# Banus/pano360

Hardware: AMD Instinct MI355X
Metric: blended megapixels/sec (multiband) (higher is better)
Workload: dtype f32; 1 GPU; cfg3: 32 synthetic 3840x2160 frames per image set, spherical warp + multiband blend L=5, native resolution (MAX_RESOLUTION uncapped); frames=32

## Files before the change

### include/pano360.h

```cpp
#ifndef PANO360_H
#define PANO360_H

#include <stddef.h>
#include <stdint.h>

#ifdef __cplusplus
extern "C" {
#endif

#define PANO_OK 0
#define PANO_EINVAL (-1)
#define PANO_EHIP (-2)
#define PANO_ELIMIT (-3)
#define PANO_ESOLVE (-4)

#define PANO_MAX_TAPS 129
#define PANO_MAX_LEVELS 8
#define PANO_TAP_LEAD 7
#define PANO_TAP_PAD 40
#ifndef PANO_INTERIOR_BLOCK
#define PANO_INTERIOR_BLOCK 4
#endif

typedef struct pano_patch {
    float *planes;
    uint8_t *mask;
    float *blurred;
    float *scratch;
    int32_t y0, x0, h, w;
    int32_t vy0, vx0, vh, vw;
    int32_t ay0, ax0, ah, aw;
    int32_t vpitch, apitch;
    int32_t index;
    int32_t tiles_off;
} pano_patch;

typedef struct pano_layout {
    int64_t planes_floats;
    int64_t blurred_floats;
    int64_t scratch_floats;
    int32_t n_records, n_tiles;
    int32_t max_vw, max_vh, max_aw, max_ah;
    int32_t missing;
} pano_layout;

typedef struct pano_camera {
    double proj[9];
    const uint8_t *frame;
    const double *hat_x;
    const double *hat_y;
    int32_t sh, sw;
    int32_t y0, x0, h, w;
} pano_camera;

typedef struct pano_pair {
    double minv[9];
    int32_t i, j;
} pano_pair;

typedef struct pano_sift_keypoint {
    float x, y;
    float size;
    float angle;
    float response;
    int32_t octave;
    int32_t r, c;
} pano_sift_keypoint;


const char *pano_version(void);
const char *pano_last_error(void);
int pano_device_count(void);
int pano_pitch(int w);
int pano_interior_block(void);

typedef struct pano_ctx pano_ctx;
#define PANO_OPT_BLUR_KERNEL 0
#define PANO_OPT_OWN_PRUNE 1
#define PANO_OPT_BLUR_SEGMENTS 2
#define PANO_OPT_BLUR_LEAN 3
#define PANO_OPT_STITCH_STREAMS 4
#define PANO_OPT_STITCH_ASYNC 5
#define PANO_OPT_BLUR_SEG_LEN 6
#define PANO_OPT_SIFT_GRAPH 7
#define PANO_OPT_LEVEL_CLASSES 8
#define PANO_OPT_COUNT 9
#define PANO_BLUR_MFMA 0
#define PANO_BLUR_VALU 1
int pano_ctx_create(int device, void *stream, pano_ctx **out);
int pano_ctx_destroy(pano_ctx *ctx);
int pano_ctx_set_stream(pano_ctx *ctx, void *stream);
int pano_ctx_set_option(pano_ctx *ctx, int option, int value);
int pano_ctx_get_option(const pano_ctx *ctx, int option, int *value);

int pano_timing_enable(pano_ctx *ctx, int on);
int pano_kernel_count(void);
const char *pano_kernel_name(int kid);
int pano_timing_read(pano_ctx *ctx, int kid, double *total_ms, int *launches);

int pano_add_weights(pano_ctx *ctx, const uint8_t *frame, int h, int w,
                     const float *lut255, const double *hat_x, const double *hat_y,
                     float *rgba);

int pano_warp_spherical(pano_ctx *ctx, const uint8_t *frame, int sh, int sw,
                        const double *proj, const double *sin_t, const double *cos_t,
                        const double *tan_p, const float *lut255, const double *hat_x,
                        const double *hat_y, int gx0, int gy0, int pw, int ph,
                        float *planes, uint8_t *mask, float *map_x, float *map_y);

int pano_warp_windows(pano_ctx *ctx, const pano_camera *cams, const pano_patch *patches,
                      int n, int max_vw, int max_vh, const double *sin_t,
                      const double *cos_t, const double *tan_p, const float *lut,
                      int lut_stride, const uint8_t *need);

int pano_ownership(pano_ctx *ctx, const pano_patch *patches, int n, int H, int W,
                   int16_t *owner, uint8_t *valid);

int pano_ownership_cameras(pano_ctx *ctx, const pano_camera *cams, int n, int H, int W,
                           int xs0, int xs1, const double *sin_t, const double *cos_t,
                           const double *tan_p, int16_t *owner, uint8_t *valid);

int pano_owned_regions(pano_ctx *ctx, const int16_t *owner, int H, int W, int xs0, int xs1,
                       int n, int min_gap, int max_spans, uint8_t *marks,
                       int32_t *regions);

int pano_ownership_regions(pano_ctx *ctx, const pano_camera *cams, int n, int H, int W,
                           int xs0, int xs1, const double *sin_t, const double *cos_t,
                           const double *tan_p, int16_t *owner, uint8_t *valid,
                           int min_gap, int max_spans, uint8_t *marks, int32_t *regions);

int pano_blur_tile_grid(const pano_ctx *ctx);
int pano_blur_tiles(pano_ctx *ctx, const pano_patch *patches, int n, int max_aw,
                    int max_ah, int W, int radius, const uint8_t *interior,
                    uint8_t *tile_flags, uint8_t *warp_need);
int pano_multiband_blur_prepare(pano_ctx *ctx, const pano_patch *patches, int n,
                                int max_aw, int max_ah, int W, const uint8_t *interior,
                                uint8_t *tile_flags);
int pano_multiband_blur(pano_ctx *ctx, const pano_patch *patches, int n, int max_aw,
                        int max_vh, int max_ah, const int16_t *owner, int W,
                        const float *taps, const int *ntaps, int n_blur,
                        const uint8_t *interior, uint8_t *tile_flags);

int pano_interior_map(pano_ctx *ctx, const int16_t *owner, int H, int W, int xs0, int xs1,
                      int radius, int16_t *block_owner, uint8_t *interior);
int pano_interior_classes(pano_ctx *ctx, const int16_t *owner, int H, int W, int xs0, int xs1,
                          const int *radii, int n_radii, int16_t *block_owner, uint8_t *interior,
                          uint8_t *classes);

int pano_layout_windows(int tile_grid, const int32_t *regions, int n, int max_spans,
                        const int32_t *rects, const uint8_t *have, int radius,
                        int xs0, int xs1, int n_blur, pano_patch *records, int cap,
                        pano_layout *out);
int pano_layout_place(pano_patch *records, int n_records, void *planes, void *blurred,
                      void *scratch);

int pano_multiband_compose(pano_ctx *ctx, const pano_patch *patches, int n, int H, int W,
                           int xs0, int xs1, int n_levels, const int16_t *owner,
                           const uint8_t *valid, const uint8_t *interior,
                           const uint8_t *classes, const pano_camera *cams,
                           const double *sin_t, const double *cos_t, const double *tan_p,
                           const float *lut, int lut_stride, uint8_t *mosaic,
                           float *mosaic_f32);

int pano_blend_cameras(pano_ctx *ctx, const pano_camera *cams, int n, int H, int W,
                       int xs0, int xs1, int linear, const double *sin_t,
                       const double *cos_t, const double *tan_p, const float *lut,
                       int lut_stride, uint8_t *mosaic, uint8_t *valid);

int pano_overlap_blocks(int h, int w);
int pano_overlap_stats(pano_ctx *ctx, const pano_camera *cams, const pano_pair *pairs,
                       int n_pairs, int h, int w, int bw0, const float *lut255,
                       double *partials, double *stats);

int pano_linear_blend(pano_ctx *ctx, const pano_patch *patches, int n, int H, int W,
                      uint8_t *mosaic);

int pano_no_blend(pano_ctx *ctx, const pano_patch *patches, int n, int H, int W,
                  uint8_t *mosaic);

int pano_crop_rect(pano_ctx *ctx, const uint8_t *valid, int H, int W, int32_t *heights,
                   int64_t *result);

int pano_blur_plane(pano_ctx *ctx, const float *src, float *dst, float *tmp, int h, int w,
                    int pitch, const float *taps, int ntaps);

int pano_pyr_down(pano_ctx *ctx, const float *src, int h, int w, float *dst);

int pano_gray_u8(pano_ctx *ctx, const uint8_t *bgr, int h, int w, float *out);
int pano_scale_step(pano_ctx *ctx, const float *src, int h, int w, const float *taps, int ntaps,
                    float *dst, float *dog);
int pano_scale_space(pano_ctx *ctx, const uint8_t *frame, int h, int w, int n_octaves,
                     int n_layers, const float *taps, const int *ntaps, float *const *gauss,
                     float *const *dog, float *work);
int pano_resize_up2(pano_ctx *ctx, const float *src, int h, int w, float *dst);
int pano_decimate2(pano_ctx *ctx, const float *src, int h, int w, float *dst);
int pano_subtract(pano_ctx *ctx, const float *a, const float *b, size_t n, float *out);

int pano_pyr_down_image(pano_ctx *ctx, const void *src, int h, int w, int c, int is_f64,
                        void *dst);
int pano_pyr_up_image(pano_ctx *ctx, const void *src, int sh, int sw, int c, int is_f64,
                      const void *other, int mode, void *dst, int oh, int ow);
int pano_u8_to_f32(pano_ctx *ctx, const uint8_t *src, size_t n, float *dst);
int pano_laplacian_mix(pano_ctx *ctx, const float *la, const float *lb, const void *gm, size_t n,
                       int is_f64, void *out);
int pano_clip_u8(pano_ctx *ctx, const void *src, size_t n, int is_f64, uint8_t *dst);

#define PANO_POISSON_CHUNK 32
int pano_poisson_blend(pano_ctx *ctx, const uint8_t *src, uint8_t *tgt, const uint8_t *mask,
                       int h, int w, int c, double rtol, int max_iters, double *solution,
                       int32_t *iters, double *resid);

#define PANO_SEAM_U8 0
#define PANO_SEAM_I16 1
#define PANO_SEAM_I32 2
#define PANO_SEAM_F32 3
#define PANO_SEAM_F64 4
#define PANO_SEAM_RESIDENT_CELLS 81408
#define PANO_SEAM_BATCH 64
int pano_seam_levels(pano_ctx *ctx, const void *img1, const void *img2, int dtype, int h, int w,
                     int c, int shrink, int16_t *level, int32_t *bad);
int pano_seam_flood(pano_ctx *ctx, const int16_t *level, int rows, int cols, int border,
                    int path, int8_t *labels, int32_t *stats);
int pano_seam_mask(pano_ctx *ctx, const int8_t *labels, int rows, int cols,
                   const int32_t *xtab, const int32_t *ytab, uint8_t *mask, int h, int w);
int pano_alpha_blend(pano_ctx *ctx, const void *img1, const void *img2, int dtype,
                     const void *mask, int mask_f64, int64_t mask_sy, int64_t mask_sx,
                     int64_t mask_sc, int h, int w, int c, uint8_t *out);

int pano_resize_u8(pano_ctx *ctx, const uint8_t *src, int sh, int sw, int c,
                   const int32_t *xtab, const int32_t *ytab, uint8_t *dst, int oh, int ow);

int pano_sift_extrema(pano_ctx *ctx, const float *dog, int rows, int cols, int octave,
                      int n_layers, float contrast_thr, float edge_thr, float sigma,
                      pano_sift_keypoint *cands, int *count, int max_cands);
int pano_sift_orient(pano_ctx *ctx, const float *const *gauss, const int *dims,
                     int n_layers, const pano_sift_keypoint *cands, const int *n_cands,
                     int max_cands, pano_sift_keypoint *kpts, int *count, int max_kpts);
int pano_sift_describe(pano_ctx *ctx, const float *const *gauss, const int *dims,
                       int first_octave, const pano_sift_keypoint *kpts, int n,
                       const int *n_dev, float *desc);
size_t pano_sift_sort_work_bytes(int n);
int pano_sift_sort_unique(pano_ctx *ctx, const pano_sift_keypoint *kpts, int n, const int *n_dev,
                          int first_octave, void *work, pano_sift_keypoint *out, int *n_out);

typedef struct pano_sift_args {
    const uint8_t *frame;
    uint8_t *frame_copy;
    int32_t h, w, n_octaves, n_layers;
    const float *taps;
    const int32_t *ntaps;
    float *const *gauss;
    float *const *dog;
    float *work;
    int32_t detect;
    float contrast_thr, edge_thr, sigma;
    int32_t first_octave, max_keypoints;
    const float *const *gauss_dev;
    const int32_t *dims_dev;
    pano_sift_keypoint *cands, *kpts;
    int32_t *counts;
    void *sort_work;
    float *desc;
} pano_sift_args;
int pano_sift_detect(pano_ctx *ctx, const pano_sift_args *args);
int pano_sift_detect_replaying(const pano_ctx *ctx);

size_t pano_knn2_work_bytes(int nq, int nt, int d);
int pano_knn2(pano_ctx *ctx, const float *query, int nq, const float *train, int nt, int d,
              float scale, void *work, int32_t *idx, float *dist, int *rescans);

int pano_match_pack(pano_ctx *ctx, const int32_t *idx, const float *dist, int nq, double ratio,
                    const float *kp_query, const float *kp_train, int nt, float *pts,
                    int32_t *match, int32_t *count);

size_t pano_hom_ransac_work_bytes(int n_pairs, int max_iters);
int pano_hom_ransac(pano_ctx *ctx, const float *pts, const int32_t *offsets, const int32_t *counts,
                    int n_pairs, int max_iters, float thresh, uint64_t seed, void *work,
                    double *hom, uint8_t *mask, int32_t *n_inliers, int32_t *hyp_inliers);

size_t pano_ba_work_bytes(int n_pairs);
int pano_ba_residuals(pano_ctx *ctx, const double *rows, const int32_t *pairs, int n_pairs,
                      const double *hom, double *ssq);
int pano_ba_normal(pano_ctx *ctx, const double *rows, const int32_t *pairs, int n_pairs,
                   const int32_t *slot, int n_active, const double *jtab, const double *hom_r,
                   double lambda, void *work, double *jtj, double *jtr);

#define PANO_JPEG_FIELDS 32
#define PANO_JPEG_CHUNK 1024
#define PANO_JPEG_SUBSEQ 1024
#define PANO_JPEG_HUFF_BYTES 1424
enum {
    PANO_JD_W, PANO_JD_H, PANO_JD_NC, PANO_JD_HMAX, PANO_JD_VMAX, PANO_JD_MCUX, PANO_JD_MCUY,
    PANO_JD_RI,
    PANO_JD_NINT,
    PANO_JD_BPM,
    PANO_JD_ORIENT, PANO_JD_DATA_OFF, PANO_JD_DATA_LEN, PANO_JD_TAB_OFF,
    PANO_JD_CHUNK0,
    PANO_JD_INT0,
    PANO_JD_SUB0,
    PANO_JD_BLK0, PANO_JD_PIX0,
    PANO_JD_DST_OFF,
    PANO_JD_PLANE0, PANO_JD_PLANE1, PANO_JD_PLANE2,
    PANO_JD_PITCH0, PANO_JD_PITCH1, PANO_JD_PITCH2,
    PANO_JD_OUT_OFF,
    PANO_JD_COMP_U,
    PANO_JD_SAMP,
    PANO_JD_TABSEL
};
enum {
    PANO_JB_N, PANO_JB_CHUNKS, PANO_JB_INTS, PANO_JB_SUBS, PANO_JB_BLOCKS, PANO_JB_PIXELS,
    PANO_JB_OUT_BYTES, PANO_JB_W_KEPT, PANO_JB_W_RST, PANO_JB_W_KEPTX, PANO_JB_W_RSTX,
    PANO_JB_W_DSTLEN, PANO_JB_W_ISTART, PANO_JB_W_IEND, PANO_JB_W_INSUB, PANO_JB_W_ISUBX,
    PANO_JB_W_STATE0, PANO_JB_W_STATE1, PANO_JB_W_CNTX, PANO_JB_W_FLAG, PANO_JB_W_COEF,
    PANO_JB_WORK_BYTES, PANO_JB_PACKED_BYTES
};
int pano_jpeg_decode(pano_ctx *ctx, const int64_t *desc, int n, const uint8_t *packed,
                     int64_t packed_bytes, void *work, int64_t work_bytes, uint8_t *out,
                     int64_t out_bytes);

#define PANO_JPEG_MAX_SIDE 65500
#define PANO_JPEG_BGR 1
size_t pano_jpeg_encode_work_bytes(int h, int w, int subsampling);
int pano_jpeg_encode(pano_ctx *ctx, const uint8_t *img, int h, int w, int64_t pitch, int flags,
                     int subsampling, const uint8_t *qt, void *work, int64_t work_bytes,
                     const uint8_t **stream, int64_t *stream_bytes);

#define PANO_EGROW 1
typedef struct pano_stitch_args {
    const pano_camera *cams;
    const int32_t *rects;
    const uint8_t *have;
    const double *sin_t, *cos_t, *tan_p;
    const float *lut;
    const float *taps;
    const int32_t *ntaps;
    int16_t *owner;
    uint8_t *valid;
    uint8_t *marks;
    int32_t *regions;
    int32_t *regions_host;
    int16_t *block_owner;
    uint8_t *interior;
    pano_patch *records_host;
    pano_patch *table;
    float *planes, *blurred, *scratch;
    uint8_t *tile_flags, *need;
    uint8_t *mosaic;
    float *mosaic_f32;
    int64_t planes_floats, blurred_floats, scratch_floats;
    int32_t n, H, W, xs0, xs1, own0, own1;
    int32_t lut_stride, n_levels, radius, shortcut, warp_need, max_spans, min_gap;
    int32_t cap_records, cap_tiles;
    int32_t used_need;
    int32_t trust_layout;
    uint8_t *classes;
    pano_layout layout;
} pano_stitch_args;
int pano_stitch_multiband(pano_ctx *ctx, pano_stitch_args *args, int resume);
int pano_stitch_verify(pano_ctx *ctx);
int pano_stitch_counts(const pano_ctx *ctx, int *device_layouts, int *fallbacks);

#ifdef __cplusplus
}
#endif
#endif
```

### pano360_amd/_lib.py

```python
import ctypes as C
import os
import subprocess

_HERE = os.path.dirname(os.path.abspath(__file__))
LIB_PATH = os.environ.get("PANO_LIB") or os.path.join(_HERE, "libpano360_hip.so")

MAX_TAPS = 129
MAX_LEVELS = 8
TAP_LEAD = 7
TAP_PAD = 40
OPT_BLUR_KERNEL, OPT_OWN_PRUNE, OPT_BLUR_SEGMENTS, OPT_BLUR_LEAN, OPT_STITCH_STREAMS = 0, 1, 2, 3, 4
OPT_STITCH_ASYNC = 5
OPT_BLUR_SEG_LEN = 6
OPT_SIFT_GRAPH = 7
OPT_LEVEL_CLASSES = 8
BLUR_MFMA, BLUR_VALU = 0, 1


class PanoError(RuntimeError):
    """A C-ABI call returned a negative status."""


class Patch(C.Structure):
    _fields_ = [("planes", C.c_void_p), ("mask", C.c_void_p),
                ("blurred", C.c_void_p), ("scratch", C.c_void_p),
                ("y0", C.c_int32), ("x0", C.c_int32), ("h", C.c_int32), ("w", C.c_int32),
                ("vy0", C.c_int32), ("vx0", C.c_int32), ("vh", C.c_int32), ("vw", C.c_int32),
                ("ay0", C.c_int32), ("ax0", C.c_int32), ("ah", C.c_int32), ("aw", C.c_int32),
                ("vpitch", C.c_int32), ("apitch", C.c_int32),
                ("index", C.c_int32), ("tiles_off", C.c_int32)]


class Layout(C.Structure):
    _fields_ = [("planes_floats", C.c_int64), ("blurred_floats", C.c_int64),
                ("scratch_floats", C.c_int64), ("n_records", C.c_int32), ("n_tiles", C.c_int32),
                ("max_vw", C.c_int32), ("max_vh", C.c_int32), ("max_aw", C.c_int32),
                ("max_ah", C.c_int32), ("missing", C.c_int32)]


class SiftArgs(C.Structure):
    _fields_ = [("frame", C.c_void_p), ("frame_copy", C.c_void_p),
                ("h", C.c_int32), ("w", C.c_int32), ("n_octaves", C.c_int32), ("n_layers", C.c_int32),
                ("taps", C.c_void_p), ("ntaps", C.c_void_p), ("gauss", C.c_void_p),
                ("dog", C.c_void_p), ("work", C.c_void_p), ("detect", C.c_int32),
                ("contrast_thr", C.c_float), ("edge_thr", C.c_float), ("sigma", C.c_float),
                ("first_octave", C.c_int32), ("max_keypoints", C.c_int32),
                ("gauss_dev", C.c_void_p), ("dims_dev", C.c_void_p), ("cands", C.c_void_p),
                ("kpts", C.c_void_p), ("counts", C.c_void_p), ("sort_work", C.c_void_p),
                ("desc", C.c_void_p)]


class StitchArgs(C.Structure):
    _fields_ = ([(k, C.c_void_p) for k in (
        "cams", "rects", "have", "sin_t", "cos_t", "tan_p", "lut", "taps", "ntaps", "owner",
        "valid", "marks", "regions", "regions_host", "block_owner", "interior", "records_host",
        "table", "planes", "blurred", "scratch", "tile_flags", "need", "mosaic", "mosaic_f32")]
        + [(k, C.c_int64) for k in ("planes_floats", "blurred_floats", "scratch_floats")]
        + [(k, C.c_int32) for k in (
            "n", "H", "W", "xs0", "xs1", "own0", "own1", "lut_stride", "n_levels", "radius",
            "shortcut", "warp_need", "max_spans", "min_gap", "cap_records", "cap_tiles",
            "used_need", "trust_layout")]
        + [("classes", C.c_void_p), ("layout", Layout)])


EINVAL = -1
ESOLVE = -4
SEAM_DTYPES = {"uint8": 0, "int16": 1, "int32": 2, "float32": 3, "float64": 4}
SEAM_RESIDENT_CELLS = 81408
EGROW = 1


class Pair(C.Structure):
    _fields_ = [("minv", C.c_double * 9), ("i", C.c_int32), ("j", C.c_int32)]


class SiftKeypoint(C.Structure):
    _fields_ = [("x", C.c_float), ("y", C.c_float), ("size", C.c_float), ("angle", C.c_float),
                ("response", C.c_float), ("octave", C.c_int32), ("r", C.c_int32), ("c", C.c_int32)]


class Camera(C.Structure):
    _fields_ = [("proj", C.c_double * 9), ("frame", C.c_void_p),
                ("hat_x", C.c_void_p), ("hat_y", C.c_void_p),
                ("sh", C.c_int32), ("sw", C.c_int32),
                ("y0", C.c_int32), ("x0", C.c_int32), ("h", C.c_int32), ("w", C.c_int32)]


_vp, _i = C.c_void_p, C.c_int
_SIGNATURES = {
    "pano_version": (C.c_char_p, []),
    "pano_last_error": (C.c_char_p, []),
    "pano_device_count": (_i, []),
    "pano_pitch": (_i, [_i]),
    "pano_interior_block": (_i, []),
    "pano_ctx_create": (_i, [_i, _vp, C.POINTER(C.c_void_p)]),
    "pano_ctx_destroy": (_i, [_vp]),
    "pano_ctx_set_stream": (_i, [_vp, _vp]),
    "pano_ctx_set_option": (_i, [_vp, _i, _i]),
    "pano_ctx_get_option": (_i, [_vp, _i, C.POINTER(C.c_int)]),
    "pano_timing_enable": (_i, [_vp, _i]),
    "pano_kernel_count": (_i, []),
    "pano_kernel_name": (C.c_char_p, [_i]),
    "pano_timing_read": (_i, [_vp, _i, C.POINTER(C.c_double), C.POINTER(C.c_int)]),
    "pano_add_weights": (_i, [_vp, _vp, _i, _i, _vp, _vp, _vp, _vp]),
    "pano_warp_spherical": (_i, [_vp, _vp, _i, _i, _vp, _vp, _vp, _vp, _vp, _vp, _vp, _i, _i, _i,
                                 _i, _vp, _vp, _vp, _vp]),
    "pano_warp_windows": (_i, [_vp, _vp, _vp, _i, _i, _i, _vp, _vp, _vp, _vp, _i, _vp]),
    "pano_blur_tiles": (_i, [_vp, _vp, _i, _i, _i, _i, _i, _vp, _vp, _vp]),
    "pano_ownership": (_i, [_vp, _vp, _i, _i, _i, _vp, _vp]),
    "pano_ownership_cameras": (_i, [_vp, _vp, _i, _i, _i, _i, _i, _vp, _vp, _vp, _vp, _vp]),
    "pano_owned_regions": (_i, [_vp, _vp, _i, _i, _i, _i, _i, _i, _i, _vp, _vp]),
    "pano_ownership_regions": (_i, [_vp, _vp, _i, _i, _i, _i, _i, _vp, _vp, _vp, _vp, _vp,
                                    _i, _i, _vp, _vp]),
    "pano_multiband_blur": (_i, [_vp, _vp, _i, _i, _i, _i, _vp, _i, _vp, C.POINTER(C.c_int), _i,
                                 _vp, _vp]),
    "pano_multiband_blur_prepare": (_i, [_vp, _vp, _i, _i, _i, _i, _vp, _vp]),
    "pano_layout_windows": (_i, [_i, _vp, _i, _i, _vp, _vp, _i, _i, _i, _i, _vp, _i, _vp]),
    "pano_layout_place": (_i, [_vp, _i, _vp, _vp, _vp]),
    "pano_interior_map": (_i, [_vp, _vp, _i, _i, _i, _i, _i, _vp, _vp]),
    "pano_interior_classes": (_i, [_vp, _vp, _i, _i, _i, _i, _vp, _i, _vp, _vp, _vp]),
    "pano_multiband_compose": (_i, [_vp, _vp, _i, _i, _i, _i, _i, _i, _vp, _vp, _vp, _vp, _vp, _vp,
                                    _vp, _vp, _vp, _i, _vp, _vp]),
    "pano_blend_cameras": (_i, [_vp, _vp, _i, _i, _i, _i, _i, _i, _vp, _vp, _vp, _vp, _i, _vp,
                                _vp]),
    "pano_blur_tile_grid": (_i, [_vp]),
    "pano_overlap_blocks": (_i, [_i, _i]),
    "pano_overlap_stats": (_i, [_vp, _vp, _vp, _i, _i, _i, _i, _vp, _vp, _vp]),
    "pano_linear_blend": (_i, [_vp, _vp, _i, _i, _i, _vp]),
    "pano_no_blend": (_i, [_vp, _vp, _i, _i, _i, _vp]),
    "pano_crop_rect": (_i, [_vp, _vp, _i, _i, _vp, _vp]),
    "pano_blur_plane": (_i, [_vp, _vp, _vp, _vp, _i, _i, _i, _vp, _i]),
    "pano_pyr_down": (_i, [_vp, _vp, _i, _i, _vp]),
    "pano_gray_u8": (_i, [_vp, _vp, _i, _i, _vp]),
    "pano_scale_step": (_i, [_vp, _vp, _i, _i, _vp, _i, _vp, _vp]),
    "pano_scale_space": (_i, [_vp, _vp, _i, _i, _i, _i, _vp, _vp, _vp, _vp, _vp]),
    "pano_resize_up2": (_i, [_vp, _vp, _i, _i, _vp]),
    "pano_decimate2": (_i, [_vp, _vp, _i, _i, _vp]),
    "pano_subtract": (_i, [_vp, _vp, _vp, C.c_size_t, _vp]),
    "pano_pyr_down_image": (_i, [_vp, _vp, _i, _i, _i, _i, _vp]),
    "pano_pyr_up_image": (_i, [_vp, _vp, _i, _i, _i, _i, _vp, _i, _vp, _i, _i]),
    "pano_u8_to_f32": (_i, [_vp, _vp, C.c_size_t, _vp]),
    "pano_laplacian_mix": (_i, [_vp, _vp, _vp, _vp, C.c_size_t, _i, _vp]),
    "pano_clip_u8": (_i, [_vp, _vp, C.c_size_t, _i, _vp]),
    "pano_poisson_blend": (_i, [_vp, _vp, _vp, _vp, _i, _i, _i, C.c_double, _i, _vp, _vp, _vp]),
    "pano_seam_levels": (_i, [_vp, _vp, _vp, _i, _i, _i, _i, _i, _vp, _vp]),
    "pano_seam_flood": (_i, [_vp, _vp, _i, _i, _i, _i, _vp, _vp]),
    "pano_seam_mask": (_i, [_vp, _vp, _i, _i, _vp, _vp, _vp, _i, _i]),
    "pano_alpha_blend": (_i, [_vp, _vp, _vp, _i, _vp, _i, C.c_int64, C.c_int64, C.c_int64, _i, _i,
                              _i, _vp]),
    "pano_resize_u8": (_i, [_vp, _vp, _i, _i, _i, _vp, _vp, _vp, _i, _i]),
    "pano_sift_extrema": (_i, [_vp, _vp, _i, _i, _i, _i, C.c_float, C.c_float, C.c_float, _vp,
                               _vp, _i]),
    "pano_sift_orient": (_i, [_vp, _vp, _vp, _i, _vp, _vp, _i, _vp, _vp, _i]),
    "pano_sift_describe": (_i, [_vp, _vp, _vp, _i, _vp, _i, _vp, _vp]),
    "pano_sift_sort_work_bytes": (C.c_size_t, [_i]),
    "pano_sift_sort_unique": (_i, [_vp, _vp, _i, _vp, _i, _vp, _vp, _vp]),
    "pano_knn2_work_bytes": (C.c_size_t, [_i, _i, _i]),
    "pano_knn2": (_i, [_vp, _vp, _i, _vp, _i, _i, C.c_float, _vp, _vp, _vp, _vp]),
    "pano_hom_ransac_work_bytes": (C.c_size_t, [_i, _i]),
    "pano_hom_ransac": (_i, [_vp, _vp, _vp, _vp, _i, _i, C.c_float, C.c_uint64, _vp, _vp, _vp, _vp,
                             _vp]),
    "pano_match_pack": (_i, [_vp, _vp, _vp, _i, C.c_double, _vp, _vp, _i, _vp, _vp, _vp]),
    "pano_ba_work_bytes": (C.c_size_t, [_i]),
    "pano_ba_residuals": (_i, [_vp, _vp, _vp, _i, _vp, _vp]),
    "pano_ba_normal": (_i, [_vp, _vp, _vp, _i, _vp, _i, _vp, _vp, C.c_double, _vp, _vp, _vp]),
    "pano_jpeg_decode": (_i, [_vp, _vp, _i, _vp, C.c_int64, _vp, C.c_int64, _vp, C.c_int64]),
    "pano_jpeg_encode_work_bytes": (C.c_size_t, [_i, _i, _i]),
    "pano_jpeg_encode": (_i, [_vp, _vp, _i, _i, C.c_int64, _i, _i, _vp, _vp, C.c_int64,
                             C.POINTER(C.c_void_p), C.POINTER(C.c_int64)]),
    "pano_sift_detect": (_i, [_vp, _vp]),
    "pano_sift_detect_replaying": (_i, [_vp]),
    "pano_stitch_multiband": (_i, [_vp, _vp, _i]),
    "pano_stitch_counts": (_i, [_vp, _vp, _vp]),
    "pano_stitch_verify": (_i, [_vp]),
}
EXPORTS = tuple(_SIGNATURES)


def sources_digest():
    import hashlib
    src = os.path.join(_HERE, "csrc")
    files = sorted(os.path.join(src, f) for f in os.listdir(src)
                   if f.endswith((".hip", ".h", ".inc")) or f == "Makefile")
    files.append(os.path.join(os.path.dirname(_HERE), "include", "pano360.h"))
    h = hashlib.sha256()
    for path in files:
        if not os.path.exists(path):
            continue
        h.update(os.path.basename(path).encode() + b"\0")
        with open(path, "rb") as fid:
            h.update(fid.read())
    return h.hexdigest()


BUILD_RECORD = os.path.join(_HERE, "csrc", ".build_stamp")


def build(force=False):
    import json
    src = os.path.join(_HERE, "csrc")
    digest = sources_digest()
    have = None
    try:
        with open(BUILD_RECORD) as fid:
            have = json.load(fid).get("sources_sha256")
    except (OSError, ValueError):
        pass
    full = force or have != digest or not os.path.exists(LIB_PATH)
    before = os.path.getmtime(LIB_PATH) if os.path.exists(LIB_PATH) else None
    cmd = ["make", "-C", src, "-s", "-j4"] + (["-B"] if full else [])
    subprocess.check_call(cmd)
    after = os.path.getmtime(LIB_PATH)
    mode = "full" if full else ("incremental" if after != before else "up to date")
    with open(BUILD_RECORD, "w") as fid:
        json.dump({"sources_sha256": digest, "mode": mode}, fid)
    return LIB_PATH


_lib = None


def lib():
    global _lib
    if _lib is None:
        if not os.path.exists(LIB_PATH):
            raise PanoError(
                f"{LIB_PATH} is missing: build it with "
                "`python -c 'import __graft_entry__ as g; g.build()'` "
                "(there is no CPU fallback)")
        import torch
        handle = C.CDLL(LIB_PATH)
        for name, (res, args) in _SIGNATURES.items():
            fn = getattr(handle, name)
            fn.restype, fn.argtypes = res, args
        _lib = handle
    return _lib


def check(status, what):
    if status != 0:
        msg = lib().pano_last_error().decode("utf-8", "replace")
        raise PanoError(f"{what} failed ({status}): {msg}")
```

### pano360_amd/csrc/api.hip

```cpp
#include <stdarg.h>
#include <stdio.h>
#include <stdlib.h>
#include <string.h>

#include <vector>

#include "common.h"
#include "layout.h"

static thread_local char g_error[512] = "";

void pano_set_error(const char *fmt, ...) {
    va_list ap;
    va_start(ap, fmt);
    vsnprintf(g_error, sizeof(g_error), fmt, ap);
    va_end(ap);
}

extern "C" const char *pano_version(void) { return "pano360_hip 0.1 (gfx950)"; }

extern "C" const char *pano_last_error(void) { return g_error; }

extern "C" int pano_device_count(void) {
    int n = 0;
    if (hipGetDeviceCount(&n) != hipSuccess) {
        (void)hipGetLastError();
        return 0;
    }
    return n;
}

extern "C" int pano_pitch(int w) { return pano_pitch_of(w); }

extern "C" int pano_interior_block(void) { return PANO_INTERIOR_BLOCK; }

extern "C" int pano_ctx_create(int device, void *stream, pano_ctx **out) {
    PANO_REQUIRE(out, "pano_ctx_create: null output");
    *out = nullptr;
    PANO_REQUIRE(device >= 0 && device < pano_device_count(), "pano_ctx_create: no device %d",
                 device);
    PANO_HIP(hipSetDevice(device));
    if (int rc = pano_blur_mfma_opt_in()) return rc;
    if (int rc = pano_blur_valu_opt_in()) return rc;
    pano_ctx *ctx = new pano_ctx();
    ctx->device = device;
    ctx->stream = (hipStream_t)stream;
    ctx->opt[PANO_OPT_BLUR_KERNEL] = PANO_BLUR_MFMA;
    ctx->opt[PANO_OPT_OWN_PRUNE] = 1;
    ctx->opt[PANO_OPT_BLUR_SEGMENTS] = 1;
    ctx->opt[PANO_OPT_BLUR_LEAN] = 1;
    ctx->opt[PANO_OPT_STITCH_STREAMS] = 1;
    ctx->opt[PANO_OPT_STITCH_ASYNC] = 0;
    ctx->opt[PANO_OPT_BLUR_SEG_LEN] = 0;
    ctx->opt[PANO_OPT_SIFT_GRAPH] = 1;
    ctx->opt[PANO_OPT_LEVEL_CLASSES] = 0;
    *out = ctx;
    return PANO_OK;
}

int pano_ctx_enter(pano_ctx *ctx) {
    if (!ctx->in_stitch) ctx->geom_valid = false;
    PANO_HIP(hipSetDevice(ctx->device));
    return PANO_OK;
}

static void timing_clear(pano_ctx *ctx) {
    for (int k = 0; k < PK_COUNT; ++k) {
        for (hipEvent_t e : ctx->t_begin[k]) (void)hipEventDestroy(e);
        for (hipEvent_t e : ctx->t_end[k]) (void)hipEventDestroy(e);
        ctx->t_begin[k].clear();
        ctx->t_end[k].clear();
    }
}

static void tap_set_free(PanoTapSet &ts) {
    if (ts.taps) (void)hipFree(ts.taps);
    if (ts.tables) (void)hipFree(ts.tables);
    if (ts.ready) (void)hipEventDestroy(ts.ready);
    free(ts.host);
    ts.taps = nullptr;
    ts.tables = nullptr;
    ts.ready = nullptr;
    ts.host = nullptr;
}

extern "C" int pano_ctx_destroy(pano_ctx *ctx) {
    if (!ctx) return PANO_OK;
    PANO_HIP(hipSetDevice(ctx->device));
    if (hipStreamSynchronize(ctx->stream) != hipSuccess) {
        (void)hipGetLastError();
        (void)hipDeviceSynchronize();
    }
    timing_clear(ctx);
    for (PanoTapSet &ts : ctx->tap_sets) tap_set_free(ts);
    if (ctx->item_buf) (void)hipFree(ctx->item_buf);
    if (ctx->item_counter) (void)hipFree(ctx->item_counter);
    if (ctx->sift_raw) (void)hipFree(ctx->sift_raw);
    if (ctx->enc_dev) (void)hipFree(ctx->enc_dev);
    if (ctx->enc_out) (void)hipFree(ctx->enc_out);
    if (ctx->enc_host) (void)hipHostFree(ctx->enc_host);
    if (ctx->poisson_dev) (void)hipFree(ctx->poisson_dev);
    if (ctx->poisson_host) (void)hipHostFree(ctx->poisson_host);
    if (ctx->seam_dev) (void)hipFree(ctx->seam_dev);
    if (ctx->seam_host) (void)hipHostFree(ctx->seam_host);
    pano_sift_graphs_free(ctx);
    if (ctx->lay_sum_host) (void)hipHostFree(ctx->lay_sum_host);
    if (ctx->lay_rects_dev) (void)hipFree(ctx->lay_rects_dev);
    if (ctx->lay_have_dev) (void)hipFree(ctx->lay_have_dev);
    if (ctx->side) {
        (void)hipStreamSynchronize(ctx->side);
        (void)hipStreamDestroy(ctx->side);
    }
    if (ctx->ev_fork) (void)hipEventDestroy(ctx->ev_fork);
    if (ctx->ev_join) (void)hipEventDestroy(ctx->ev_join);
    if (ctx->ev_regions) (void)hipEventDestroy(ctx->ev_regions);
    if (ctx->ev_upload) (void)hipEventDestroy(ctx->ev_upload);
    if (ctx->ev_copy) (void)hipEventDestroy(ctx->ev_copy);
    delete ctx;
    return PANO_OK;
}

int pano_ctx_side_stream(pano_ctx *ctx) {
    if (!ctx->ev_regions) PANO_HIP(hipEventCreateWithFlags(&ctx->ev_regions, hipEventDisableTiming));
    if (!ctx->ev_upload) PANO_HIP(hipEventCreateWithFlags(&ctx->ev_upload, hipEventDisableTiming));
    if (!ctx->ev_fork) PANO_HIP(hipEventCreateWithFlags(&ctx->ev_fork, hipEventDisableTiming));
    if (!ctx->ev_join) PANO_HIP(hipEventCreateWithFlags(&ctx->ev_join, hipEventDisableTiming));
    if (!ctx->ev_copy) PANO_HIP(hipEventCreateWithFlags(&ctx->ev_copy, hipEventDisableTiming));
    if (!ctx->side) PANO_HIP(hipStreamCreateWithFlags(&ctx->side, hipStreamNonBlocking));
    return PANO_OK;
}

extern "C" int pano_ctx_set_stream(pano_ctx *ctx, void *stream) {
    PANO_REQUIRE(ctx, "pano_ctx_set_stream: null context");
    if ((hipStream_t)stream != ctx->stream) ctx->geom_valid = false;
    ctx->stream = (hipStream_t)stream;
    return PANO_OK;
}

extern "C" int pano_ctx_set_option(pano_ctx *ctx, int option, int value) {
    PANO_REQUIRE(ctx, "pano_ctx_set_option: null context");
    PANO_REQUIRE(option >= 0 && option < PANO_OPT_COUNT, "pano_ctx_set_option: option %d", option);
    if (option == PANO_OPT_BLUR_KERNEL)
        PANO_REQUIRE(value == PANO_BLUR_MFMA || value == PANO_BLUR_VALU,
                     "pano_ctx_set_option: blur kernel %d", value);
    else if (option == PANO_OPT_STITCH_ASYNC)
        PANO_REQUIRE(value >= 0 && value <= 2, "pano_ctx_set_option: option %d takes 0, 1 or 2", option);
    else if (option == PANO_OPT_OWN_PRUNE)
        PANO_REQUIRE(value >= 0 && value <= 3, "pano_ctx_set_option: option %d takes 0 .. 3", option);
    else if (option == PANO_OPT_BLUR_SEG_LEN)
        PANO_REQUIRE(value == -1 || value == 0 || (value >= 4 && value <= 2047),
                     "pano_ctx_set_option: option %d takes -1, 0 or 4 .. 2047", option);
    else
        PANO_REQUIRE(value == 0 || value == 1, "pano_ctx_set_option: option %d takes 0 or 1", option);
    const bool changed = ctx->opt[option] != value;
    ctx->opt[option] = value;
    ctx->prepared_table = ctx->flags_table = ctx->list_table = nullptr;
    ctx->geom_valid = false;
    if (changed && option == PANO_OPT_BLUR_KERNEL)
        ctx->lay_prev_valid = ctx->lay_prev_verified = false;
    return PANO_OK;
}

extern "C" int pano_ctx_get_option(const pano_ctx *ctx, int option, int *value) {
    PANO_REQUIRE(ctx && value, "pano_ctx_get_option: null pointer");
    PANO_REQUIRE(option >= 0 && option < PANO_OPT_COUNT, "pano_ctx_get_option: option %d", option);
    *value = ctx->opt[option];
    return PANO_OK;
}

static uint64_t tap_hash(const float *taps, const int *ntaps, int n, size_t floats) {
    uint64_t h = 1469598103934665603ull;
    auto eat = [&](const void *p, size_t bytes) {
        const unsigned char *b = (const unsigned char *)p;
        for (size_t i = 0; i < bytes; ++i) h = (h ^ b[i]) * 1099511628211ull;
    };
    eat(&n, sizeof(n));
    eat(ntaps, n * sizeof(int));
    eat(taps, floats * sizeof(float));
    return h;
}

#define PANO_TAP_SETS_MAX 64
int pano_ctx_tap_set(pano_ctx *ctx, const float *taps, const int *ntaps, int n, size_t table_bytes,
                     PanoTapSet **out, bool *fresh) {
    size_t floats = 0;
    for (int k = 0; k < n; ++k) floats += (size_t)ntaps[k] + PANO_TAP_PAD;
    const uint64_t key = tap_hash(taps, ntaps, n, floats);
    *fresh = false;
    for (PanoTapSet &ts : ctx->tap_sets)
        if (ts.key == key && ts.n == n && !memcmp(ts.ntaps, ntaps, n * sizeof(int)) &&
            ts.floats == floats && !memcmp(ts.host, taps, floats * sizeof(float))) {
            ts.used = ++ctx->tick;
            if (ctx->stream != ts.built_on) PANO_HIP(hipStreamWaitEvent(ctx->stream, ts.ready, 0));
            if (table_bytes && !ts.tables) {
                PANO_HIP(hipMalloc((void **)&ts.tables, table_bytes));
                *fresh = true;
            }
            *out = &ts;
            return PANO_OK;
        }
    if (ctx->tap_sets.size() >= PANO_TAP_SETS_MAX) {
        size_t old = 0;
        for (size_t i = 1; i < ctx->tap_sets.size(); ++i)
            if (ctx->tap_sets[i].used < ctx->tap_sets[old].used) old = i;
        PANO_HIP(hipDeviceSynchronize());
        tap_set_free(ctx->tap_sets[old]);
        ctx->tap_sets.erase(ctx->tap_sets.begin() + old);
    }
    PanoTapSet ts = {};
    ts.key = key;
    ts.n = n;
    memcpy(ts.ntaps, ntaps, n * sizeof(int));
    ts.floats = floats;
    ts.host = (float *)malloc(floats * sizeof(float));
    PANO_REQUIRE(ts.host, "pano_ctx_tap_set: out of host memory");
    memcpy(ts.host, taps, floats * sizeof(float));
    PANO_HIP(hipMalloc((void **)&ts.taps, floats * sizeof(float)));
    PANO_HIP(hipMemcpyAsync(ts.taps, taps, floats * sizeof(float), hipMemcpyHostToDevice,
                            ctx->stream));
    PANO_HIP(hipEventCreateWithFlags(&ts.ready, hipEventDisableTiming));
    PANO_HIP(hipEventRecord(ts.ready, ctx->stream));
    ts.built_on = ctx->stream;
    if (table_bytes) {
        PANO_HIP(hipMalloc((void **)&ts.tables, table_bytes));
        *fresh = true;
    }
    ts.used = ++ctx->tick;
    ctx->tap_sets.push_back(ts);
    *out = &ctx->tap_sets.back();
    return PANO_OK;
}

int pano_ctx_tap_set_built(pano_ctx *ctx, PanoTapSet *set) {
    PANO_HIP(hipEventRecord(set->ready, ctx->stream));
    set->built_on = ctx->stream;
    return PANO_OK;
}

static const char *const g_kernel_names[] = {
    "add_weights_kernel", "warp_spherical_kernel", "ownership_kernel", "blur_rows_kernel",
    "blur_cols_kernel",   "multiband_compose_kernel", "linear_blend_kernel",
    "no_blend_kernel",    "crop_heights_kernel", "crop_rows_kernel", "pyr_down_kernel",
    "ownership_cameras_kernel", "owned_boxes_kernel", "warp_windows_kernel",
    "blend_cameras_kernel", "owned_spans_kernel",
    "block_owner_kernel", "tile_flags_kernel", "overlap_stats_kernel",
    "blur_mfma_kernel", "sift_extrema_kernel", "sift_orient_kernel", "sift_describe_kernel",
    "scale_step_kernel", "knn2_kernel", "blur_lean_kernel", "blur_lean5_kernel",
    "ransac_score_kernel", "ransac_finish_kernel", "match_pack_kernel",
    "ba_residual_kernel", "ba_pair_kernel", "ba_assemble_kernel",
    "jpeg_destuff_kernel", "jpeg_scan_kernel", "jpeg_intervals_kernel", "jpeg_huff_sync_kernel",
    "jpeg_huff_write_kernel", "jpeg_dc_kernel", "jpeg_idct_kernel", "jpeg_pixels_kernel",
    "jpeg_enc_blocks_kernel", "jpeg_enc_count_kernel", "jpeg_enc_scan_kernel", "jpeg_enc_emit_kernel",
    "jpeg_enc_stuff_kernel"};
static_assert(sizeof(g_kernel_names) / sizeof(g_kernel_names[0]) == PK_COUNT,
              "one name per PanoKernelId, in enum order");

void pano_timing_edge(pano_ctx *ctx, int kid, hipStream_t stream, bool begin) {
    hipEvent_t ev;
    if (hipEventCreate(&ev) != hipSuccess) return;
    (void)hipEventRecord(ev, stream);
    (begin ? ctx->t_begin : ctx->t_end)[kid].push_back(ev);
}

extern "C" int pano_timing_enable(pano_ctx *ctx, int on) {
    PANO_REQUIRE(ctx, "pano_timing_enable: null context");
    timing_clear(ctx);
    ctx->timing_on = on != 0;
    return PANO_OK;
}

extern "C" int pano_kernel_count(void) { return PK_COUNT; }

extern "C" const char *pano_kernel_name(int kid) {
    return kid >= 0 && kid < PK_COUNT ? g_kernel_names[kid] : "";
}

extern "C" int pano_timing_read(pano_ctx *ctx, int kid, double *total_ms, int *launches) {
    PANO_REQUIRE(ctx && kid >= 0 && kid < PK_COUNT && total_ms && launches,
                 "pano_timing_read: bad argument");
    double sum = 0.0;
    const size_t nb = ctx->t_begin[kid].size(), ne = ctx->t_end[kid].size();
    const size_t n = ne < nb ? ne : nb;
    for (size_t i = 0; i < n; ++i) {
        PANO_HIP(hipEventSynchronize(ctx->t_end[kid][i]));
        float ms = 0.f;
        PANO_HIP(hipEventElapsedTime(&ms, ctx->t_begin[kid][i], ctx->t_end[kid][i]));
        sum += ms;
    }
    *total_ms = sum;
    *launches = (int)n;
    return PANO_OK;
}

extern "C" int pano_layout_windows(int tile_grid, const int32_t *regions, int n, int max_spans,
                                   const int32_t *rects, const uint8_t *have, int radius,
                                   int xs0, int xs1, int n_blur, pano_patch *records, int cap,
                                   pano_layout *out) {
    PANO_REQUIRE(regions && rects && records && out, "pano_layout_windows: null pointer");
    PANO_REQUIRE(tile_grid == 0 || tile_grid == 32, "pano_layout_windows: tile grid %d", tile_grid);
    PANO_REQUIRE(n >= 0 && max_spans >= 1 && radius >= 0 && n_blur >= 0 && cap >= 0,
                 "pano_layout_windows: bad argument");
    const bool grid32 = tile_grid == 32;
    const int stride = 5 + 2 * max_spans;
    pano_layout lay = {};
    lay.missing = 0;
    long planes = 0, blurred = 0, scratch = 0, tiles = 0;
    int k = 0;
    for (int i = 0; i < n; ++i) {
        const int32_t *rg = regions + (size_t)i * stride;
        const int spans = rg[4] < max_spans ? rg[4] : max_spans;
        for (int sp = 0; sp < spans; ++sp) {
            pano_patch rec;
            LayoutSizes sz;
            if (!layout_record(rg, sp, rects + 4 * i, i, radius, xs0, xs1, n_blur, grid32, rec, sz))
                continue;
            PANO_REQUIRE(k < cap, "pano_layout_windows: more than %d records", cap);
            if (have && !have[i]) ++lay.missing;
            pano_patch &r = records[k++];
            r = rec;
            PANO_REQUIRE(layout_record_fits(r),
                         "pano_layout_windows: a plane of record %d exceeds 2 GiB", k - 1);
            r.planes = (float *)(uintptr_t)planes;
            r.blurred = (float *)(uintptr_t)(blurred + sz.lead);
            r.scratch = (float *)(uintptr_t)scratch;
            PANO_REQUIRE(tiles < (1l << 31), "pano_layout_windows: tile count overflow");
            r.tiles_off = (int)tiles;
            planes += sz.planes;
            blurred += sz.blurred;
            scratch += sz.scratch;
            tiles += sz.tiles;
            lay.max_vw = r.vw > lay.max_vw ? r.vw : lay.max_vw;
            lay.max_vh = r.vh > lay.max_vh ? r.vh : lay.max_vh;
            lay.max_aw = r.aw > lay.max_aw ? r.aw : lay.max_aw;
            lay.max_ah = r.ah > lay.max_ah ? r.ah : lay.max_ah;
        }
    }
    lay.n_records = k;
    lay.n_tiles = (int)tiles;
    lay.planes_floats = planes;
    lay.blurred_floats = blurred + 32;
    lay.scratch_floats = scratch;
    *out = lay;
    return PANO_OK;
}

extern "C" int pano_layout_place(pano_patch *records, int n_records, void *planes, void *blurred,
                                 void *scratch) {
    PANO_REQUIRE(records || n_records == 0, "pano_layout_place: null pointer");
    uintptr_t bbase = (uintptr_t)blurred;
    bbase += (uintptr_t)(-(intptr_t)bbase) % 128;
    for (int k = 0; k < n_records; ++k) {
        pano_patch &r = records[k];
        r.planes = (float *)planes + (uintptr_t)r.planes;
        r.blurred = blurred ? (float *)bbase + (uintptr_t)r.blurred : nullptr;
        r.scratch = scratch ? (float *)scratch + (uintptr_t)r.scratch : nullptr;
    }
    return PANO_OK;
}
```

### pano360_amd/csrc/blend.hip

```cpp
#include <stdlib.h>

#include "geom.h"

__global__ __launch_bounds__(256) void ownership_kernel(
    const pano_patch *__restrict__ patches, int n, int H, int W,
    int16_t *__restrict__ owner, uint8_t *__restrict__ valid) {
    const int x = blockIdx.x * 64 + threadIdx.x, y = blockIdx.y * 4 + threadIdx.y;
    if (x >= W || y >= H) return;
    float best = 0.0f;
    int who = -1;
    bool any = false;
    for (int i = 0; i < n; ++i) {
        const pano_patch p = patches[i];
        const int px = x - p.x0, py = y - p.y0;
        if ((unsigned)px >= (unsigned)p.w || (unsigned)py >= (unsigned)p.h) continue;
        const float a = p.planes[3 * (size_t)p.vh * p.vpitch + (size_t)py * p.vpitch + px];
        if (a > best) {
            best = a;
            who = i;
        }
        any |= p.mask[(size_t)py * p.w + px] == 0;
    }
    owner[(size_t)y * W + x] = (int16_t)who;
    valid[(size_t)y * W + x] = any ? 1 : 0;
// ... 384 lines not shown
        }
        __syncthreads();
        const int tid = wave * 64 + lane;
        const bool keep = tid < listed && alpha_bound(cams + sh.list[tid], s_rng).hi >= 0.0f;
        const unsigned long long bal = __ballot(keep);
        if (lane == 0) s_kept[wave] = __popcll(bal);
        __syncthreads();
        int off = 0;
        for (int w = 0; w < wave; ++w) off += s_kept[w];
        off += __popcll(bal & ((1ull << lane) - 1ull));
        if (keep) s_keep[off] = sh.list[tid];
        ncand = s_kept[0] + s_kept[1] + s_kept[2] + s_kept[3];
        list = s_keep;
        __syncthreads();
    }

    const int x = bx0 + threadIdx.x, y = by0 + threadIdx.y;
    if (x >= xs1 || y >= H) return;
    const double s = sin_t[x], c = cos_t[x], t = tan_p[y];
    float acc[3] = {0.0f, 0.0f, 0.0f}, wsum = 0.0f;
    uint8_t last[3] = {0, 0, 0};
    bool any = false;
    for (int kk = 0; kk < ncand; ++kk) {
        const int k = LINEAR ? kk : ncand - 1 - kk;
        const int i = listed < 0 ? k : __builtin_amdgcn_readfirstlane(list[k]);
        const pano_camera *cam = cams + i;
        const int px = x - cam->x0, py = y - cam->y0;
        if ((unsigned)px >= (unsigned)cam->w || (unsigned)py >= (unsigned)cam->h) continue;
        float fx, fy;
        const int sw = cam->sw, sh_ = cam->sh;
        if (map_pixel(cam->proj, s, c, t, sw, sh_, fx, fy)) continue;
        any = true;
        const Taps tp = make_taps_unmasked(fx, fy, sw, sh_);
        const TapBytes tb = load_taps(cam->frame, sw, tp);
        float rgb[3];
        const float *__restrict__ gl = lut + (size_t)i * 256;
#pragma unroll
        for (int ch = 0; ch < 3; ++ch)
            rgb[ch] = PERCAM ? lerp4(lut_at(gl, tb.v[0][ch]), lut_at(gl, tb.v[1][ch]), lut_at(gl, tb.v[2][ch]),
                                     lut_at(gl, tb.v[3][ch]), tp)
                             : lerp4(lut_at(s_lut, tb.v[0][ch]), lut_at(s_lut, tb.v[1][ch]), lut_at(s_lut, tb.v[2][ch]),
                                     lut_at(s_lut, tb.v[3][ch]), tp);
        if (LINEAR) {
            const float a = alpha_at(cam->hat_x, cam->hat_y, tp);
#pragma unroll
            for (int ch = 0; ch < 3; ++ch) acc[ch] = acc[ch] + rgb[ch] * a;
            wsum = wsum + a;
        } else {
#pragma unroll
            for (int ch = 0; ch < 3; ++ch) last[ch] = (uint8_t)(int)(255.0f * rgb[ch]);
            break;
        }
    }
    const size_t g = ((size_t)y * W + x) * 3;
    if (LINEAR) {
        const float ws = wsum == 0.0f ? 1.0f : wsum;
#pragma unroll
        for (int ch = 0; ch < 3; ++ch)
            mosaic[g + ch] = (uint8_t)(int)(255.0f * __fdiv_rn(acc[ch], ws));
    } else {
        mosaic[g] = last[0];
        mosaic[g + 1] = last[1];
        mosaic[g + 2] = last[2];
    }
    if (valid) valid[(size_t)y * W + x] = any ? 1 : 0;
}

typedef short own8 __attribute__((ext_vector_type(8), aligned(2)));

__device__ __forceinline__ void owned_box_pixel(int o, int x, int y, bool up, bool down, bool left,
                                                bool right, int W, int32_t *__restrict__ boxes,
                                                int stride, uint8_t *__restrict__ marks) {
    if (o < 0) return;
    if (up && marks) marks[(size_t)o * W + x] = 1;
    if (!left && !right) return;
    if (left && up) {
        atomicMin(&boxes[(size_t)stride * o + 0], y);
        atomicMin(&boxes[(size_t)stride * o + 2], x);
    }
    if (left && down) atomicMax(&boxes[(size_t)stride * o + 1], y);
    if (right && up) atomicMax(&boxes[(size_t)stride * o + 3], x);
}

__global__ __launch_bounds__(256) void owned_boxes_kernel(const int16_t *__restrict__ owner,
                                                          int H, int W, int xs0, int xs1,
                                                          int32_t *__restrict__ boxes, int stride,
                                                          uint8_t *__restrict__ marks) {
    const int x8 = xs0 + (blockIdx.x * 64 + threadIdx.x) * 8, y = blockIdx.y * 4 + threadIdx.y;
    if (x8 >= xs1 || y >= H) return;
    const int16_t *row = owner + (size_t)y * W;
    const bool top = y == 0, bottom = y == H - 1;
    if (x8 + 8 <= xs1) {
        const own8 cur = *(const own8 *)(row + x8);
        const own8 upv = top ? cur : *(const own8 *)(row - W + x8);
        const own8 dnv = bottom ? cur : *(const own8 *)(row + W + x8);
        const int before = x8 == xs0 ? -32768 : row[x8 - 1];
        const int after = x8 + 8 == xs1 ? -32768 : row[x8 + 8];
#pragma unroll
        for (int j = 0; j < 8; ++j) {
            const int o = cur[j];
            const int l = j == 0 ? before : cur[j - 1], r = j == 7 ? after : cur[j + 1];
            owned_box_pixel(o, x8 + j, y, top || upv[j] != o, bottom || dnv[j] != o, l != o, r != o,
                            W, boxes, stride, marks);
        }
        return;
    }
    for (int x = x8; x < xs1; ++x) {
        const int o = row[x];
        owned_box_pixel(o, x, y, top || row[x - W] != o, bottom || row[x + W] != o,
                        x == xs0 || row[x - 1] != o, x == xs1 - 1 || row[x + 1] != o, W, boxes,
                        stride, marks);
    }
}

__device__ __forceinline__ uint8_t quant255(float v) { return (uint8_t)(int)(255.0f * v); }

#define IB PANO_INTERIOR_BLOCK

__global__ __launch_bounds__(256) void block_owner_kernel(const int16_t *__restrict__ owner,
                                                          int H, int W, int xs0, int xs1,
                                                          int H8, int W8, int blo, int bhi,
                                                          int16_t *__restrict__ bown) {
    const int bx = blo + blockIdx.x * 64 + threadIdx.x, by = blockIdx.y * 4 + threadIdx.y;
    if (bx >= bhi || by >= H8) return;
    const int x0 = bx * IB, y0 = by * IB;
    int o = -2;
    if (x0 >= xs0 && (x0 + IB < W ? x0 + IB : W) <= xs1) {
        o = owner[(size_t)y0 * W + x0];
        const bool whole = x0 + IB <= W && (W & 1) == 0;
        if (x0 + IB <= W && y0 + IB <= H) {
            static_assert(IB == 4, "one 8-byte load per block row");
            typedef uint64_t u64_any __attribute__((aligned(2)));
            const uint64_t o16 = (uint16_t)o;
            const uint64_t all = o16 | o16 << 16 | o16 << 32 | o16 << 48;
            uint64_t diff = 0;
#pragma unroll
            for (int dy = 0; dy < IB; ++dy)
                diff |= *(const u64_any *)(owner + (size_t)(y0 + dy) * W + x0) ^ all;
            if (diff) o = -2;
        } else
        for (int dy = 0; dy < IB && o != -2; ++dy) {
            const int y = y0 + dy;
            if (y >= H) break;
            if (whole) {
                const uint32_t *q = (const uint32_t *)(owner + (size_t)y * W + x0);
                const uint32_t both = ((uint32_t)(uint16_t)o << 16) | (uint16_t)o;
                uint32_t diff = 0;
#pragma unroll
                for (int k = 0; k < IB / 2; ++k) diff |= q[k] ^ both;
                if (diff) o = -2;
            } else {
                for (int dx = 0; dx < IB; ++dx) {
                    const int x = x0 + dx;
                    if (x >= W) break;
                    if (owner[(size_t)y * W + x] != o) {
                        o = -2;
                        break;
                    }
                }
            }
        }
    }
    bown[(size_t)by * W8 + bx] = (int16_t)o;
}

#define IT_W 64
#define IT_H 16
#define IT_REACH_MAX 20
__device__ __forceinline__ bool agree(int a, int b) { return a == b || a == -3 || b == -3; }

struct LevelReaches {
    int n;
    int reach[PANO_MAX_LEVELS];
};

__global__ __launch_bounds__(256) void interior_tile_kernel(const int16_t *__restrict__ bown,
                                                            int H8, int W8, int reach, int blo,
                                                            int bhi, int ilo, int ihi,
                                                            uint8_t *__restrict__ interior,
                                                            LevelReaches lv,
                                                            uint8_t *__restrict__ classes) {
    __shared__ int16_t s_own[(IT_H + 2 * IT_REACH_MAX) * (IT_W + 2 * IT_REACH_MAX)];
    __shared__ int16_t s_col[IT_H * (IT_W + 2 * IT_REACH_MAX)];
    __shared__ unsigned long long s_vmask[IT_W + 2 * IT_REACH_MAX];
    const int tid = threadIdx.x, lane = tid & 63, wave = tid >> 6;
    const int bx0 = ilo + blockIdx.x * IT_W, by0 = blockIdx.y * IT_H;
    const int tw = IT_W + 2 * reach, th = IT_H + 2 * reach;
    for (int ty = wave; ty < th; ty += 4) {
        const int y = by0 - reach + ty;
        const bool row_in = y >= 0 && y < H8;
        for (int tx = lane; tx < tw; tx += 64) {
            const int x = bx0 - reach + tx;
            s_own[ty * tw + tx] = (row_in && x >= 0 && x < W8)
                                      ? (x >= blo && x < bhi ? bown[(size_t)y * W8 + x] : (int16_t)-2)
                                      : (int16_t)-3;
        }
    }
    __syncthreads();
    for (int tx = tid; tx < tw; tx += 256) {
        unsigned long long m = 0;
        int prev = s_own[tx];
#pragma unroll 8
        for (int ty = 0; ty + 1 < th; ++ty) {
            const int cur = s_own[(ty + 1) * tw + tx];
            m |= (unsigned long long)agree(prev, cur) << ty;
            prev = cur;
        }
        s_vmask[tx] = m;
    }
    __syncthreads();
    int cls[IT_H / 4];
#pragma unroll
    for (int r = 0; r < IT_H / 4; ++r) cls[r] = 0;
    const int nlv = classes ? lv.n : 1;
    for (int q = 0; q < nlv; ++q) {
        const int rq = classes ? lv.reach[q] : reach, off = reach - rq;
        const unsigned long long full = (1ull << (2 * rq)) - 1ull;
        for (int ry = wave; ry < IT_H; ry += 4)
            for (int tx = lane; tx < tw; tx += 64) {
                const int o = s_own[(ry + reach) * tw + tx];
                const bool same = ((s_vmask[tx] >> (ry + off)) & full) == full;
                s_col[ry * tw + tx] = (int16_t)(o >= 0 && !same ? -2 : o);
            }
        __syncthreads();
#pragma unroll
        for (int r = 0; r < IT_H / 4; ++r) {
            const int ry = wave + 4 * r;
            const int16_t *row = s_col + ry * tw;
            const int a0 = row[lane], a1 = row[min(lane + 1, tw - 1)];
            const int b0 = row[min(lane + 64, tw - 1)], b1 = row[min(lane + 65, tw - 1)];
            const unsigned long long lo = __ballot(lane + 1 < tw && agree(a0, a1));
            const unsigned long long hi = __ballot(lane + 65 < tw && agree(b0, b1));
            const int sh = lane + off;
            const unsigned long long win = sh == 0 ? lo
                                           : sh < 64 ? (lo >> sh) | (hi << (64 - sh))
                                                     : hi >> (sh - 64);
            const int o = row[lane + reach];
            if (o >= 0 && (win & full) == full && cls[r] == q) cls[r] = q + 1;
        }
        __syncthreads();
    }
#pragma unroll
    for (int r = 0; r < IT_H / 4; ++r) {
        const int y = by0 + wave + 4 * r, x = bx0 + lane;
        if (y >= H8 || x >= ihi) continue;
        interior[(size_t)y * W8 + x] = cls[r] == nlv ? 1 : 0;
        if (classes) classes[(size_t)y * W8 + x] = (uint8_t)cls[r];
    }
}

struct InteriorArgs {
    const uint8_t *interior;
    int W8;
    const pano_camera *cams;
    const double *sin_t, *cos_t, *tan_p;
    const float *lut;
    const uint8_t *classes;
};

enum { LUT_LDS = 0, LUT_GLOBAL = 1 };

template <int LUT>
__device__ __forceinline__ void shade_interior(const pano_camera *cam, const float *__restrict__ table,
                                               const InteriorArgs &ia, int x, int y, int W,
                                               uint8_t *__restrict__ mosaic,
                                               float *__restrict__ mosaic_f32) {
    if (!cam->frame) return;
    const int sw = cam->sw, sh = cam->sh;
    float fx, fy;
    map_pixel(cam->proj, table_f64(ia.sin_t, x), table_f64(ia.cos_t, x), table_f64(ia.tan_p, y), sw, sh, fx, fy);
    Taps tp = tap_base(fx, fy);
    TapBytes tb;
    if (__ballot(!taps_interior(tp, sw, sh)) == 0ull) {
        tb = load_taps_interior(cam->frame, sw, tp);
    } else {
        tp.x1 = min(tp.x1, sw - 1);
        tp.y1 = min(tp.y1, sh - 1);
        tb = load_taps(cam->frame, sw, tp);
    }
    const size_t g = ((size_t)y * W + x) * 3;
#pragma unroll
    for (int c = 0; c < 3; ++c) {
        float v = lerp4(lut_at(table, tb.v[0][c]), lut_at(table, tb.v[1][c]),
                        lut_at(table, tb.v[2][c]), lut_at(table, tb.v[3][c]), tp);
        v = v < 0.0f ? 0.0f : (v > 1.0f ? 1.0f : v);
        if (mosaic_f32) mosaic_f32[g + c] = v;
        mosaic[g + c] = (uint8_t)(int)(255.0f * v);
    }
}

template <int LUT>
__device__ __forceinline__ void shade_interior_of(int own, const float *__restrict__ table, int stride,
                                                  const InteriorArgs &ia, int x, int y, int W,
                                                  uint8_t *__restrict__ mosaic,
                                                  float *__restrict__ mosaic_f32) {
    const int own_u = __builtin_amdgcn_readfirstlane(own);
    if (__ballot(own != own_u) == 0)
        shade_interior<LUT>(ia.cams + own_u, table + (size_t)own_u * stride, ia, x, y, W, mosaic, mosaic_f32);
    else
        shade_interior<LUT>(ia.cams + own, table + (size_t)own * stride, ia, x, y, W, mosaic, mosaic_f32);
}

#define COMPOSE_MASKS 4
template <int L, bool PERCAM, bool CLS>
__global__ __launch_bounds__(256) void multiband_compose_kernel(
    const pano_patch *__restrict__ patches, int n, int H, int W, int xs0, int xs1,
    const int16_t *__restrict__ owner, const uint8_t *__restrict__ valid,
    uint8_t *__restrict__ mosaic, float *__restrict__ mosaic_f32, InteriorArgs ia) {
    __shared__ float s_lut[256];
    if (ia.interior && !PERCAM) {
        s_lut[threadIdx.y * 64 + threadIdx.x] = ia.lut[threadIdx.y * 64 + threadIdx.x];
        __syncthreads();
    }
    const int x = xs0 + blockIdx.x * 64 + threadIdx.x, y = blockIdx.y * 4 + threadIdx.y;
    const bool inside = x < xs1 && y < H;
    const bool is_interior = inside && ia.interior && ia.interior[(size_t)(y / IB) * ia.W8 + x / IB];
    unsigned long long cand[COMPOSE_MASKS] = {};
    const bool masked = n <= 64 * COMPOSE_MASKS && __ballot(inside && !is_interior) != 0;
    if (masked) {
        const int wx0 = xs0 + blockIdx.x * 64, wx1 = min(wx0 + 64, xs1);
#pragma unroll
        for (int m = 0; m < COMPOSE_MASKS; ++m) {
            const int i = 64 * m + (int)threadIdx.x;
            bool hit = false;
            if (i < n) {
                const pano_patch *q = patches + i;
                const int ax = q->x0 + q->ax0, ay = q->y0 + q->ay0;
                hit = ax < wx1 && ax + q->aw > wx0 && ay <= y && y < ay + q->ah;
            }
            cand[m] = __ballot(hit);
        }
    }
    if (!inside) return;
    if (is_interior) {
        const int own = owner[(size_t)y * W + x];
        if (PERCAM)
            shade_interior_of<LUT_GLOBAL>(own, ia.lut, 256, ia, x, y, W, mosaic, mosaic_f32);
        else
            shade_interior_of<LUT_LDS>(own, s_lut, 0, ia, x, y, W, mosaic, mosaic_f32);
        return;
    }
    float layer[L][3], wsum[L];
#pragma unroll
    for (int k = 0; k < L; ++k) layer[k][0] = layer[k][1] = layer[k][2] = wsum[k] = 0.0f;
    const int j = CLS && L > 1 ? (int)ia.classes[(size_t)(y / IB) * ia.W8 + x / IB] : 0;
    const int own_px = CLS && j > 0 ? (int)owner[(size_t)y * W + x] : -1;
    float base[3] = {0.0f, 0.0f, 0.0f};

    int m = 0;
    unsigned long long bits = masked ? cand[0] : 0ull;
    for (int i = 0;; ++i) {
        if (masked) {
            while (bits == 0ull && ++m < COMPOSE_MASKS) bits = cand[m];
            if (bits == 0ull) break;
            i = 64 * m + __ffsll((long long)bits) - 1;
            bits &= bits - 1ull;
        } else if (i >= n) {
            break;
        }
        const pano_patch p = patches[i];
        const int ax = x - p.x0 - p.ax0, ay = y - p.y0 - p.ay0;
        if ((unsigned)ax >= (unsigned)p.aw || (unsigned)ay >= (unsigned)p.ah) continue;
        const size_t vplane = (size_t)p.vh * p.vpitch;
        const size_t vo = (size_t)(ay + p.ay0 - p.vy0) * p.vpitch + (ax + p.ax0 - p.vx0);
        const size_t aplane = (size_t)p.ah * p.apitch, ao = (size_t)ay * p.apitch + ax;
        float hi[3], ha = 0.0f;
        if (!CLS || j == 0) {
#pragma unroll
            for (int c = 0; c < 3; ++c) hi[c] = p.planes[c * vplane + vo];
        } else {
            const float *b = p.blurred + (size_t)(j - 1) * 4 * aplane + ao;
#pragma unroll
            for (int c = 0; c < 3; ++c) hi[c] = b[c * aplane];
            if (p.index == own_px) {
#pragma unroll
                for (int c = 0; c < 3; ++c) base[c] = p.planes[c * vplane + vo] - hi[c];
            }
        }
        if (L == 1) ha = owner[(size_t)y * W + x] == p.index ? 1.0f : 0.0f;
#pragma unroll
        for (int k = 0; k < L; ++k) {
            if (CLS && k < j) continue;
            float rgb[3], a;
            if (k < L - 1) {
                const float *b = p.blurred + (size_t)k * 4 * aplane + ao;
                a = b[3 * aplane];
#pragma unroll
                for (int c = 0; c < 3; ++c) {
                    const float g = b[c * aplane];
                    rgb[c] = hi[c] - g;
                    hi[c] = g;
                }
                ha = a;
            } else {
                a = ha;
#pragma unroll
                for (int c = 0; c < 3; ++c) rgb[c] = hi[c];
            }
#pragma unroll
            for (int c = 0; c < 3; ++c) layer[k][c] = layer[k][c] + rgb[c] * a;
            wsum[k] = wsum[k] + a;
        }
    }
    const bool ok = valid[(size_t)y * W + x] != 0;
    float out[3] = {CLS && ok ? base[0] : 0.0f, CLS && ok ? base[1] : 0.0f, CLS && ok ? base[2] : 0.0f};
#pragma unroll
    for (int k = 0; k < L; ++k) {
        if (CLS && k < j) continue;
        const float ws = wsum[k] == 0.0f ? 1.0f : wsum[k];
#pragma unroll
        for (int c = 0; c < 3; ++c)
            out[c] = out[c] + __fdiv_rn(ok ? layer[k][c] : 0.0f, ws);
    }
    const size_t g = ((size_t)y * W + x) * 3;
#pragma unroll
    for (int c = 0; c < 3; ++c) {
        float v = out[c];
        v = v < 0.0f ? 0.0f : (v > 1.0f ? 1.0f : v);
        if (mosaic_f32) mosaic_f32[g + c] = v;
        mosaic[g + c] = quant255(v);
    }
}

__global__ __launch_bounds__(256) void linear_blend_kernel(
    const pano_patch *__restrict__ patches, int n, int H, int W,
    uint8_t *__restrict__ mosaic) {
    const int x = blockIdx.x * 64 + threadIdx.x, y = blockIdx.y * 4 + threadIdx.y;
    if (x >= W || y >= H) return;
    float acc[3] = {0.0f, 0.0f, 0.0f}, wsum = 0.0f;
    for (int i = 0; i < n; ++i) {
        const pano_patch p = patches[i];
        const int px = x - p.x0, py = y - p.y0;
        if ((unsigned)px >= (unsigned)p.w || (unsigned)py >= (unsigned)p.h) continue;
        const size_t plane = (size_t)p.vh * p.vpitch, o = (size_t)py * p.vpitch + px;
        const bool m = p.mask[(size_t)py * p.w + px] != 0;
        const float a = p.planes[3 * plane + o];
#pragma unroll
        for (int c = 0; c < 3; ++c) {
            const float t = m ? 0.0f : p.planes[c * plane + o];
            acc[c] = acc[c] + t * a;
        }
        wsum = wsum + a;
    }
    const float ws = wsum == 0.0f ? 1.0f : wsum;
    const size_t g = ((size_t)y * W + x) * 3;
#pragma unroll
    for (int c = 0; c < 3; ++c) mosaic[g + c] = quant255(__fdiv_rn(acc[c], ws));
}

__global__ __launch_bounds__(256) void no_blend_kernel(
    const pano_patch *__restrict__ patches, int n, int H, int W,
    uint8_t *__restrict__ mosaic) {
    const int x = blockIdx.x * 64 + threadIdx.x, y = blockIdx.y * 4 + threadIdx.y;
    if (x >= W || y >= H) return;
    uint8_t out[3] = {0, 0, 0};
    for (int i = 0; i < n; ++i) {
        const pano_patch p = patches[i];
        const int px = x - p.x0, py = y - p.y0;
        if ((unsigned)px >= (unsigned)p.w || (unsigned)py >= (unsigned)p.h) continue;
        if (p.mask[(size_t)py * p.w + px]) continue;
        const size_t plane = (size_t)p.vh * p.vpitch, o = (size_t)py * p.vpitch + px;
#pragma unroll
        for (int c = 0; c < 3; ++c) out[c] = quant255(p.planes[c * plane + o]);
    }
    const size_t g = ((size_t)y * W + x) * 3;
    mosaic[g] = out[0];
    mosaic[g + 1] = out[1];
    mosaic[g + 2] = out[2];
}

static int check_table(const void *table, int n, int H, int W, const char *who) {
    PANO_REQUIRE(table, "%s: null table", who);
    PANO_REQUIRE(n >= 0 && n <= 32767, "%s: %d patches (int16 owner map holds 32767)", who, n);
    PANO_REQUIRE(H > 0 && W > 0, "%s: bad mosaic shape %dx%d", who, H, W);
    return PANO_OK;
}

#define MOSAIC_GRID dim3 block(64, 4), grid(ceil_div(W, 64), ceil_div(H, 4))

extern "C" int pano_ownership(pano_ctx *ctx, const pano_patch *patches, int n, int H, int W,
                              int16_t *owner, uint8_t *valid) {
    PANO_ENTER(ctx, "pano_ownership");
    if (int rc = check_table(patches, n, H, W, "pano_ownership")) return rc;
    PANO_REQUIRE(owner && valid, "pano_ownership: null output");
    MOSAIC_GRID;
    PANO_TIMED(PK_OWNERSHIP, (hipStream_t)stream,
               hipLaunchKernelGGL(ownership_kernel, grid, block, 0, (hipStream_t)stream,
                                  patches, n, H, W, owner, valid));
    PANO_LAUNCH_CHECK("ownership_kernel");
    return PANO_OK;
}

extern "C" int pano_ownership_cameras(pano_ctx *ctx, const pano_camera *cams, int n, int H, int W,
                                      int xs0, int xs1, const double *sin_t, const double *cos_t,
                                      const double *tan_p, int16_t *owner, uint8_t *valid) {
    PANO_ENTER(ctx, "pano_ownership_cameras");
    if (int rc = check_table(cams, n, H, W, "pano_ownership_cameras")) return rc;
    PANO_REQUIRE(sin_t && cos_t && tan_p && owner && valid, "pano_ownership_cameras: null pointer");
    PANO_REQUIRE(xs0 >= 0 && xs1 <= W && xs0 <= xs1, "pano_ownership_cameras: bad strip [%d, %d)", xs0, xs1);
    if (xs0 == xs1) return PANO_OK;
    const int prune = ctx->opt[PANO_OPT_OWN_PRUNE];
    dim3 block(64, 4), grid(ceil_div(xs1 - xs0, 64), ceil_div(H, (prune & 2) ? OWN_TILE_ROWS : OW_TH_TALL));
    PANO_TIMED(PK_OWNERSHIP_CAMS, (hipStream_t)stream,
               hipLaunchKernelGGL((prune & 2) ? ownership_cameras_l1_kernel : ownership_cameras_kernel,
                                  grid, block, (prune & 2) ? 0 : own_shared_bytes(n),
                                  (hipStream_t)stream, cams, n, H, W, xs0, xs1, sin_t, cos_t,
                                  tan_p, owner, valid, prune & 1, (int32_t *)nullptr, 0,
                                  (uint8_t *)nullptr));
    PANO_LAUNCH_CHECK("ownership_cameras_kernel");
    return PANO_OK;
}

extern "C" int pano_blend_cameras(pano_ctx *ctx, const pano_camera *cams, int n, int H, int W,
                                  int xs0, int xs1, int linear, const double *sin_t,
                                  const double *cos_t, const double *tan_p, const float *lut,
                                  int lut_stride, uint8_t *mosaic, uint8_t *valid) {
    PANO_ENTER(ctx, "pano_blend_cameras");
    if (int rc = check_table(cams, n, H, W, "pano_blend_cameras")) return rc;
    PANO_REQUIRE(sin_t && cos_t && tan_p && lut && mosaic, "pano_blend_cameras: null pointer");
    PANO_REQUIRE(lut_stride == 0 || lut_stride == 256,
                 "pano_blend_cameras: lut_stride %d (0 = shared table, 256 = per camera)", lut_stride);
    PANO_REQUIRE(xs0 >= 0 && xs1 <= W && xs0 <= xs1, "pano_blend_cameras: bad strip [%d, %d)", xs0, xs1);
    if (xs0 == xs1) return PANO_OK;
    dim3 block(64, 4), grid(ceil_div(xs1 - xs0, 64), ceil_div(H, 4));
    hipStream_t s = (hipStream_t)stream;
#define BLEND(LIN, PC)                                                                        \
    PANO_TIMED(PK_BLEND_CAMERAS, s,                                                           \
               hipLaunchKernelGGL((blend_cameras_kernel<LIN, PC>), grid, block, 0, s, cams, n, \
                                  H, W, xs0, xs1, sin_t, cos_t, tan_p, lut, mosaic, valid))
    if (linear && lut_stride) BLEND(true, true);
    else if (linear) BLEND(true, false);
    else if (lut_stride) BLEND(false, true);
    else BLEND(false, false);
#undef BLEND
    PANO_LAUNCH_CHECK("blend_cameras_kernel");
    return PANO_OK;
}

#define SPAN_WORDS 1024
__global__ __launch_bounds__(256) void owned_spans_kernel(const uint8_t *__restrict__ marks,
                                                          int W, int xs0, int xs1, int min_gap,
                                                          int max_spans, int stride,
                                                          int32_t *__restrict__ regions) {
    __shared__ unsigned long long s_bits[SPAN_WORDS];
    const int lane = threadIdx.x & 63, wave = threadIdx.x >> 6;
    const uint8_t *row = marks + (size_t)blockIdx.x * W;
    int32_t *out = regions + (size_t)blockIdx.x * stride + 5;
    int cnt = 0, last = 0;
    const int32_t *box = regions + (size_t)blockIdx.x * stride;
    xs0 = max(xs0, box[2]);
    xs1 = min(xs1, box[3] + 1);
    for (int chunk0 = xs0; chunk0 < xs1; chunk0 += 64 * SPAN_WORDS) {
        const int words = min(SPAN_WORDS, (xs1 - chunk0 + 63) >> 6);
        for (int w = wave; w < words; w += 4) {
            const int x = chunk0 + 64 * w + lane;
            const unsigned long long bal = __ballot(x < xs1 && row[x] != 0);
            if (lane == 0) s_bits[w] = bal;
        }
        __syncthreads();
        if (wave == 0) {
            for (int w = 0; w < words; ++w) {
                const int base = chunk0 + 64 * w;
                unsigned long long bal = s_bits[w];
                while (bal) {
                    const int s = __ffsll((long long)bal) - 1;
                    const unsigned long long rest = ~(bal >> s);
                    const int len = rest ? __ffsll((long long)rest) - 1 : 64 - s;
                    const int xa = base + s, xb = xa + len - 1;
                    if (cnt && (xa - last - 1 < min_gap || cnt == max_spans)) {
                        if (lane == 0) out[2 * (cnt - 1) + 1] = xb;
                    } else {
                        if (lane == 0) {
                            out[2 * cnt] = xa;
                            out[2 * cnt + 1] = xb;
                        }
                        ++cnt;
                    }
                    last = xb;
                    bal = s + len >= 64 ? 0ull : bal & ~((1ull << (s + len)) - 1ull);
                }
            }
        }
        __syncthreads();
    }
    if (threadIdx.x == 0) regions[(size_t)blockIdx.x * stride + 4] = cnt;
}

__global__ __launch_bounds__(256) void init_regions_kernel(int32_t *regions, int n, int stride,
                                                           uint8_t *marks, size_t mark_bytes) {
    const size_t i = (size_t)blockIdx.x * 256 + threadIdx.x;
    if (i < (size_t)n) {
        int32_t *r = regions + i * stride;
        r[0] = 0x7fffffff;
        r[1] = -1;
        r[2] = 0x7fffffff;
        r[3] = -1;
        r[4] = 0;
    }
    const size_t words = mark_bytes / 16, step = (size_t)gridDim.x * 256;
    uint4 *m16 = (uint4 *)marks;
    for (size_t k = i; k < words; k += step) m16[k] = make_uint4(0u, 0u, 0u, 0u);
    if (i < mark_bytes - words * 16) marks[words * 16 + i] = 0;
}

static int launch_init_regions(hipStream_t s, int32_t *regions, int n, int stride, uint8_t *marks,
                               int W) {
    size_t bytes = (size_t)n * W;
    if ((uintptr_t)marks & 15) {
        PANO_HIP(hipMemsetAsync(marks, 0, bytes, s));
        bytes = 0;
    }
    const size_t want = bytes / 16 / 256 + 1;
    const int blocks = (int)(want < 2048 ? (want > (size_t)ceil_div(n, 256) ? want : ceil_div(n, 256))
                                         : 2048);
    hipLaunchKernelGGL(init_regions_kernel, dim3(blocks), dim3(256), 0, s, regions, n, stride, marks,
                       bytes);
    PANO_LAUNCH_CHECK("init_regions_kernel");
    return PANO_OK;
}

extern "C" int pano_owned_regions(pano_ctx *ctx, const int16_t *owner, int H, int W, int xs0,
                                  int xs1, int n, int min_gap, int max_spans, uint8_t *marks,
                                  int32_t *regions) {
    PANO_ENTER(ctx, "pano_owned_regions");
    PANO_REQUIRE(owner && marks && regions, "pano_owned_regions: null pointer");
    PANO_REQUIRE(H > 0 && W > 0 && n >= 0 && n <= 32767 && max_spans >= 1 && min_gap >= 0,
                 "pano_owned_regions: bad argument");
    PANO_REQUIRE(xs0 >= 0 && xs1 <= W && xs0 <= xs1, "pano_owned_regions: bad strip [%d, %d)", xs0, xs1);
    if (n == 0) return PANO_OK;
    hipStream_t s = (hipStream_t)stream;
    const int stride = 5 + 2 * max_spans;
    if (int rc = launch_init_regions(s, regions, n, stride, marks, W)) return rc;
    if (xs0 == xs1) return PANO_OK;
    dim3 block(64, 4), grid(ceil_div(xs1 - xs0, 512), ceil_div(H, 4));
    PANO_TIMED(PK_OWNED_BOXES, s,
               hipLaunchKernelGGL(owned_boxes_kernel, grid, block, 0, s, owner, H, W, xs0, xs1,
                                  regions, stride, marks));
    PANO_LAUNCH_CHECK("owned_boxes_kernel");
    PANO_TIMED(PK_OWNED_SPANS, s,
               hipLaunchKernelGGL(owned_spans_kernel, dim3(n), dim3(256), 0, s, marks, W, xs0, xs1,
                                  min_gap, max_spans, stride, regions));
    PANO_LAUNCH_CHECK("owned_spans_kernel");
    return PANO_OK;
}

extern "C" int pano_ownership_regions(pano_ctx *ctx, const pano_camera *cams, int n, int H, int W,
                                      int xs0, int xs1, const double *sin_t, const double *cos_t,
                                      const double *tan_p, int16_t *owner, uint8_t *valid,
                                      int min_gap, int max_spans, uint8_t *marks,
                                      int32_t *regions) {
    PANO_ENTER(ctx, "pano_ownership_regions");
    if (int rc = check_table(cams, n, H, W, "pano_ownership_regions")) return rc;
    PANO_REQUIRE(sin_t && cos_t && tan_p && owner && valid && marks && regions,
                 "pano_ownership_regions: null pointer");
    PANO_REQUIRE(xs0 >= 0 && xs1 <= W && xs0 <= xs1, "pano_ownership_regions: bad strip [%d, %d)", xs0, xs1);
    PANO_REQUIRE(max_spans >= 1 && min_gap >= 0, "pano_ownership_regions: bad argument");
    if (n == 0) return PANO_OK;
    hipStream_t s = (hipStream_t)stream;
    const int stride = 5 + 2 * max_spans;
    if (int rc = launch_init_regions(s, regions, n, stride, marks, W)) return rc;
    if (xs0 == xs1) return PANO_OK;
    const int prune = ctx->opt[PANO_OPT_OWN_PRUNE];
    dim3 block(64, 4), grid(ceil_div(xs1 - xs0, 64), ceil_div(H, (prune & 2) ? OWN_TILE_ROWS : OW_TH_TALL));
    PANO_TIMED(PK_OWNERSHIP_CAMS, s,
               hipLaunchKernelGGL((prune & 2) ? ownership_cameras_l1_kernel : ownership_cameras_kernel,
                                  grid, block, (prune & 2) ? 0 : own_shared_bytes(n), s, cams, n, H, W, xs0,
                                  xs1, sin_t, cos_t, tan_p, owner, valid, prune & 1, regions, stride,
                                  marks));
    PANO_LAUNCH_CHECK("ownership_cameras_kernel");
    PANO_TIMED(PK_OWNED_SPANS, s,
               hipLaunchKernelGGL(owned_spans_kernel, dim3(n), dim3(256), 0, s, marks, W, xs0, xs1,
                                  min_gap, max_spans, stride, regions));
    PANO_LAUNCH_CHECK("owned_spans_kernel");
    return PANO_OK;
}

static int interior_map_launch(pano_ctx *ctx, const int16_t *owner, int H, int W, int xs0, int xs1,
                               const int *radii, int n_radii, int16_t *block_owner,
                               uint8_t *interior, uint8_t *classes, const char *who) {
    void *const stream = (void *)ctx->stream;
    PANO_REQUIRE(owner && block_owner && interior && radii, "%s: null pointer", who);
    PANO_REQUIRE(H > 0 && W > 0 && n_radii >= 1 && n_radii < PANO_MAX_LEVELS, "%s: bad argument", who);
    PANO_REQUIRE(xs0 >= 0 && xs1 <= W && xs0 <= xs1, "%s: bad strip [%d, %d)", who, xs0, xs1);
    LevelReaches lv = {};
    lv.n = n_radii;
    for (int k = 0; k < n_radii; ++k) {
        PANO_REQUIRE(radii[k] >= 0 && (k == 0 || radii[k] >= radii[k - 1]),
                     "%s: radii must ascend (level %d: %d)", who, k, radii[k]);
        lv.reach[k] = ceil_div(radii[k] + IB - 1, IB);
    }
    const int radius = radii[n_radii - 1];
    const int H8 = ceil_div(H, IB), W8 = ceil_div(W, IB), reach = lv.reach[n_radii - 1];
    if (xs0 == xs1) return PANO_OK;
    const int ilo = xs0 / IB, ihi = ceil_div(xs1, IB);
    const int blo = ilo - reach > 0 ? ilo - reach : 0, bhi = ihi + reach < W8 ? ihi + reach : W8;
    dim3 block(64, 4), grid(ceil_div(bhi - blo, 64), ceil_div(H8, 4));
    hipStream_t s = (hipStream_t)stream;
    PANO_TIMED(PK_INTERIOR, s,
               hipLaunchKernelGGL(block_owner_kernel, grid, block, 0, s, owner, H, W, xs0, xs1,
                                  H8, W8, blo, bhi, block_owner));
    PANO_LAUNCH_CHECK("block_owner_kernel");
    PANO_REQUIRE(reach <= IT_REACH_MAX, "%s: radius %d reaches %d blocks (at most %d)", who, radius,
                 reach, IT_REACH_MAX);
    hipLaunchKernelGGL(interior_tile_kernel, dim3(ceil_div(ihi - ilo, IT_W), ceil_div(H8, IT_H)),
                       dim3(256), 0, s, block_owner, H8, W8, reach, blo, bhi, ilo, ihi, interior, lv,
                       classes);
    PANO_LAUNCH_CHECK("interior_tile_kernel");
    return PANO_OK;
}

extern "C" int pano_interior_map(pano_ctx *ctx, const int16_t *owner, int H, int W, int xs0,
                                 int xs1, int radius, int16_t *block_owner, uint8_t *interior) {
    PANO_ENTER(ctx, "pano_interior_map");
    return interior_map_launch(ctx, owner, H, W, xs0, xs1, &radius, 1, block_owner, interior, nullptr,
                               "pano_interior_map");
}

extern "C" int pano_interior_classes(pano_ctx *ctx, const int16_t *owner, int H, int W, int xs0,
                                     int xs1, const int *radii, int n_radii, int16_t *block_owner,
                                     uint8_t *interior, uint8_t *classes) {
    PANO_ENTER(ctx, "pano_interior_classes");
    PANO_REQUIRE(classes, "pano_interior_classes: null pointer");
    return interior_map_launch(ctx, owner, H, W, xs0, xs1, radii, n_radii, block_owner, interior,
                               classes, "pano_interior_classes");
}

extern "C" int pano_multiband_compose(pano_ctx *ctx, const pano_patch *patches, int n, int H,
                                      int W, int xs0, int xs1, int n_levels, const int16_t *owner,
                                      const uint8_t *valid, const uint8_t *interior,
                                      const uint8_t *classes, const pano_camera *cams,
                                      const double *sin_t,
                                      const double *cos_t, const double *tan_p, const float *lut,
                                      int lut_stride, uint8_t *mosaic, float *mosaic_f32) {
    PANO_ENTER(ctx, "pano_multiband_compose");
    if (int rc = check_table(patches, n, H, W, "pano_multiband_compose")) return rc;
    PANO_REQUIRE(H > 0 && W > 0, "pano_multiband_compose: bad mosaic shape %dx%d", H, W);
    PANO_REQUIRE(owner && mosaic && valid, "pano_multiband_compose: null pointer");
    PANO_REQUIRE(n_levels >= 1 && n_levels <= PANO_MAX_LEVELS,
                 "pano_multiband_compose: n_levels %d outside [1, %d]", n_levels, PANO_MAX_LEVELS);
    PANO_REQUIRE(xs0 >= 0 && xs1 <= W && xs0 <= xs1,
                 "pano_multiband_compose: bad strip [%d, %d)", xs0, xs1);
    PANO_REQUIRE(!interior || (cams && sin_t && cos_t && tan_p && lut),
                 "pano_multiband_compose: the interior map needs cameras, tables and LUT");
    PANO_REQUIRE(lut_stride == 0 || lut_stride == 256,
                 "pano_multiband_compose: lut_stride %d (0 = shared table, 256 = per camera)",
                 lut_stride);
    if (xs0 == xs1) return PANO_OK;
    PANO_REQUIRE(!classes || interior, "pano_multiband_compose: level classes without the interior map");
    InteriorArgs ia = {interior, ceil_div(W, IB), cams, sin_t, cos_t, tan_p, lut,
                       ctx->opt[PANO_OPT_LEVEL_CLASSES] ? classes : nullptr};
    const bool percam = interior && lut_stride != 0;
    dim3 block(64, 4), grid(ceil_div(xs1 - xs0, 64), ceil_div(H, 4));
    hipStream_t s = (hipStream_t)stream;
#define COMPOSE_AS(L, PC, CL)                                                            \
    PANO_TIMED(PK_COMPOSE, s,                                                           \
               hipLaunchKernelGGL((multiband_compose_kernel<L, PC, CL>), grid, block, 0, s, \
                                  patches, n, H, W, xs0, xs1, owner, valid, mosaic,     \
                                  mosaic_f32, ia))
#define COMPOSE(L)                                                                      \
    case L:                                                                             \
        if (ia.classes && L > 1) {                                                      \
            if (percam) COMPOSE_AS(L, true, true); else COMPOSE_AS(L, false, true);     \
        } else {                                                                        \
            if (percam) COMPOSE_AS(L, true, false); else COMPOSE_AS(L, false, false);   \
        }                                                                               \
        break;
    switch (n_levels) {
        COMPOSE(1) COMPOSE(2) COMPOSE(3) COMPOSE(4) COMPOSE(5) COMPOSE(6) COMPOSE(7) COMPOSE(8)
    }
#undef COMPOSE_AS
#undef COMPOSE
    PANO_LAUNCH_CHECK("multiband_compose_kernel");
    return PANO_OK;
}

extern "C" int pano_linear_blend(pano_ctx *ctx, const pano_patch *patches, int n, int H, int W,
                                 uint8_t *mosaic) {
    PANO_ENTER(ctx, "pano_linear_blend");
    if (int rc = check_table(patches, n, H, W, "pano_linear_blend")) return rc;
    PANO_REQUIRE(mosaic, "pano_linear_blend: null output");
    MOSAIC_GRID;
    PANO_TIMED(PK_LINEAR, (hipStream_t)stream,
               hipLaunchKernelGGL(linear_blend_kernel, grid, block, 0, (hipStream_t)stream,
                                  patches, n, H, W, mosaic));
    PANO_LAUNCH_CHECK("linear_blend_kernel");
    return PANO_OK;
}

extern "C" int pano_no_blend(pano_ctx *ctx, const pano_patch *patches, int n, int H, int W,
                             uint8_t *mosaic) {
    PANO_ENTER(ctx, "pano_no_blend");
    if (int rc = check_table(patches, n, H, W, "pano_no_blend")) return rc;
    PANO_REQUIRE(mosaic, "pano_no_blend: null output");
    MOSAIC_GRID;
    PANO_TIMED(PK_NOBLEND, (hipStream_t)stream,
               hipLaunchKernelGGL(no_blend_kernel, grid, block, 0, (hipStream_t)stream,
                                  patches, n, H, W, mosaic));
    PANO_LAUNCH_CHECK("no_blend_kernel");
    return PANO_OK;
}
```

### pano360_amd/csrc/common.h

```cpp
#pragma once
#include <hip/hip_runtime.h>
#include <stdint.h>

#include <vector>

#include "../../include/pano360.h"

void pano_set_error(const char *fmt, ...);

#define PANO_REQUIRE(cond, ...)          \
    do {                                 \
        if (!(cond)) {                   \
            pano_set_error(__VA_ARGS__); \
            return PANO_EINVAL;          \
        }                                \
    } while (0)

#define PANO_HIP(call)                                                         \
    do {                                                                       \
        hipError_t e_ = (call);                                                \
        if (e_ != hipSuccess) {                                                \
            pano_set_error("%s failed: %s", #call, hipGetErrorString(e_));     \
            return PANO_EHIP;                                                  \
        }                                                                      \
    } while (0)

#define PANO_LAUNCH_CHECK(name)                                                \
    do {                                                                       \
        hipError_t e_ = hipGetLastError();                                     \
        if (e_ != hipSuccess) {                                                \
            pano_set_error("launch of %s failed: %s", name,                    \
                           hipGetErrorString(e_));                             \
            return PANO_EHIP;                                                  \
        }                                                                      \
    } while (0)

enum PanoKernelId {
    PK_ADD_WEIGHTS = 0,
    PK_WARP,
    PK_OWNERSHIP,
    PK_BLUR_ROWS,
    PK_BLUR_COLS,
    PK_COMPOSE,
    PK_LINEAR,
    PK_NOBLEND,
    PK_CROP_HEIGHTS,
    PK_CROP_ROWS,
    PK_PYR_DOWN,
    PK_OWNERSHIP_CAMS,
    PK_OWNED_BOXES,
    PK_WARP_WINDOWS,
    PK_BLEND_CAMERAS,
    PK_OWNED_SPANS,
    PK_INTERIOR,
    PK_TILE_FLAGS,
    PK_OVERLAP,
    PK_BLUR_MFMA,
    PK_SIFT_EXTREMA,
    PK_SIFT_ORIENT,
    PK_SIFT_DESCRIBE,
    PK_SCALE_STEP,
    PK_KNN2,
    PK_BLUR_LEAN,
    PK_BLUR_LEAN5,
    PK_RANSAC_SCORE,
    PK_RANSAC_FINISH,
    PK_MATCH_PACK,
    PK_BA_RESIDUAL,
    PK_BA_PAIRS,
    PK_BA_ASSEMBLE,
    PK_JPEG_DESTUFF,
    PK_JPEG_SCAN,
    PK_JPEG_INTERVALS,
    PK_JPEG_HUFF_SYNC,
    PK_JPEG_HUFF_WRITE,
    PK_JPEG_DC,
    PK_JPEG_IDCT,
    PK_JPEG_PIXELS,
    PK_JPEG_ENC_BLOCKS,
    PK_JPEG_ENC_COUNT,
    PK_JPEG_ENC_SCAN,
    PK_JPEG_ENC_EMIT,
    PK_JPEG_ENC_STUFF,
    PK_COUNT
};
struct PanoTapSet {
    uint64_t key;
    int n, ntaps[PANO_MAX_LEVELS];
    float *taps;
    unsigned char *tables;
    uint64_t used;
    float *host;
    size_t floats;
    hipEvent_t ready;
    hipStream_t built_on;
};

struct LayoutSummary;
struct PanoSiftGraph {
    uint64_t key;
    hipGraphExec_t exec;
    int seen;
    uint64_t used;
};

#define GEOM_BUFS 11
#define STITCH_SIG 13
struct pano_ctx {
    int device;
    hipStream_t stream;
    int opt[PANO_OPT_COUNT];
    bool timing_on;
    std::vector<hipEvent_t> t_begin[PK_COUNT], t_end[PK_COUNT];
    int2 *item_buf;
    int *item_counter;
    int blur_cm;
    int item_cap;
    const pano_patch *prepared_table, *flags_table;
    int prepared_n, flags_n;
    const pano_patch *list_table;
    int list_n;
    std::vector<PanoTapSet> tap_sets;
    uint64_t tick;
    hipEvent_t ev_regions, ev_upload, ev_fork, ev_join, ev_copy;
    hipStream_t side;
    bool upload_pending;
    LayoutSummary *lay_sum_host;
    int32_t *lay_rects_dev;
    uint8_t *lay_have_dev;
    int lay_cap_n;
    std::vector<int32_t> lay_rects_host;
    std::vector<uint8_t> lay_have_host;
    pano_layout lay_prev;
    int lay_prev_sig[STITCH_SIG];
    bool lay_prev_valid;
    bool lay_prev_verified;
    bool trusted_pending;
    int lay_prev_used_need;
    bool geom_valid, in_stitch;
    const void *geom_bufs[GEOM_BUFS];
    int lay_count[2];
    uint32_t *sift_raw;
    size_t sift_raw_cap;
    bool sift_capturing;
    std::vector<PanoSiftGraph> sift_graphs;
    uint8_t *enc_dev, *enc_out, *enc_host;
    size_t enc_dev_cap, enc_out_cap, enc_host_cap;
    uint8_t *poisson_dev, *poisson_host;
    size_t poisson_cap;
    uint8_t *seam_dev, *seam_host;
};

int pano_ctx_enter(pano_ctx *ctx);
void pano_sift_graphs_free(pano_ctx *ctx);
int pano_sift_raw_reserve(pano_ctx *ctx, int rows, int cols);
int pano_zero_i32(hipStream_t s, int *p, int n);
int pano_ctx_side_stream(pano_ctx *ctx);
int pano_ctx_tap_set(pano_ctx *ctx, const float *taps, const int *ntaps, int n, size_t table_bytes,
                     PanoTapSet **out, bool *fresh);
int pano_ctx_tap_set_built(pano_ctx *ctx, PanoTapSet *set);

#define PANO_ENTER(ctx, who)                                       \
    PANO_REQUIRE((ctx) != nullptr, "%s: null context", who);       \
    if (int rc_ = pano_ctx_enter(ctx)) return rc_;                 \
    void *const stream = (void *)(ctx)->stream;                    \
    (void)stream

#define PANO_ENTER_READONLY(ctx, who)                              \
    const bool geom_keep_ = (ctx) != nullptr && (ctx)->geom_valid; \
    PANO_ENTER(ctx, who);                                          \
    (ctx)->geom_valid = geom_keep_

void pano_timing_edge(pano_ctx *ctx, int kid, hipStream_t stream, bool begin);

#define PANO_TIMED(kid, stream, ...)                                        \
    do {                                                                    \
        if (ctx->timing_on) pano_timing_edge(ctx, kid, stream, true);       \
        __VA_ARGS__;                                                        \
        if (ctx->timing_on) pano_timing_edge(ctx, kid, stream, false);      \
    } while (0)

static inline int pano_pitch_of(int w) { return (w + 3) & ~3; }

int pano_launch_blur_mfma(pano_ctx *ctx, const pano_patch *table, int n, int max_aw, int max_ah,
                          const int16_t *owner, int W, const float *taps, const int *ntaps,
                          int n_blur, const uint8_t *interior, uint8_t *tile_flags);
int pano_prepare_blur_mfma(pano_ctx *ctx, const pano_patch *table, int n, int max_aw, int max_ah,
                           int W, const uint8_t *interior, uint8_t *tile_flags);
int pano_tiles_blur_mfma(pano_ctx *ctx, const pano_patch *table, int n, int max_aw, int max_ah,
                         int W, int radius, const uint8_t *interior, uint8_t *tile_flags,
                         uint8_t *warp_need);
int pano_blur_mfma_opt_in(void);
int pano_blur_valu_opt_in(void);
static inline bool pano_blur_uses_mfma(const pano_ctx *ctx) {
    return ctx->opt[PANO_OPT_BLUR_KERNEL] == PANO_BLUR_MFMA;
}
static inline int ceil_div(int a, int b) { return (a + b - 1) / b; }

typedef const __attribute__((address_space(4))) float *kptr_f32;

__device__ __forceinline__ int reflect_edge(int p, int len) {
    if ((unsigned)p < (unsigned)len) return p;
    int per = 2 * len;
    int m = p % per;
    if (m < 0) m += per;
    return m < len ? m : per - 1 - m;
}

__device__ __forceinline__ int reflect_101(int p, int len) {
    if ((unsigned)p < (unsigned)len) return p;
    if (len == 1) return 0;
    int per = 2 * len - 2;
    int m = p % per;
    if (m < 0) m += per;
    return m < len ? m : per - m;
}

__device__ __forceinline__ int cv_round(float v) {
    const float r = rintf(v);
    return fabsf(r) < 2147483648.0f ? (int)r : (int)0x80000000;
}

__device__ __forceinline__ int sat16(int v) {
    return v < -32768 ? -32768 : (v > 32767 ? 32767 : v);
}
```

### pano360_amd/csrc/stitch.hip

```cpp
#include <string.h>

#include "common.h"
#include "layout.h"


#define LAY_THREADS 512
__global__ __launch_bounds__(LAY_THREADS) void layout_windows_kernel(
    const int32_t *__restrict__ regions, const int32_t *__restrict__ rects,
    const uint8_t *__restrict__ have, int n, int max_spans, int radius, int xs0, int xs1,
    int n_blur, int grid32, float *planes, float *blurred, float *scratch, long cap_planes,
    long cap_blurred, long cap_scratch, int cap_tiles, int want_tiles, int b_nr, int b_vw,
    int b_vh, int b_aw, int b_ah, pano_patch *__restrict__ table,
    LayoutSummary *__restrict__ summary, LayoutSummary expect, int check_expect,
    int *__restrict__ sticky) {
    __shared__ long s_planes[LAY_THREADS], s_blurred[LAY_THREADS], s_scratch[LAY_THREADS];
    __shared__ int s_tiles[LAY_THREADS], s_slot[LAY_THREADS];
    __shared__ long s_run[4];
    __shared__ int s_count, s_max[4], s_missing, s_bad;
    const int tid = threadIdx.x, stride = 5 + 2 * max_spans;
    if (tid == 0) {
        s_run[0] = s_run[1] = s_run[2] = s_run[3] = 0;
        s_count = s_missing = s_bad = 0;
        s_max[0] = s_max[1] = s_max[2] = s_max[3] = 0;
    }
    __syncthreads();
    const int total = n * max_spans;
    for (int base = 0; base < total; base += LAY_THREADS) {
        const int c = base + tid, i = c / max_spans, sp = c - i * max_spans;
        pano_patch rec = pano_patch{};
        LayoutSizes sz = LayoutSizes{};
        bool ok = false;
        if (c < total) {
            const int32_t *rg = regions + (size_t)i * stride;
            const int spans = rg[4] < max_spans ? rg[4] : max_spans;
            if (sp < spans)
                ok = layout_record(rg, sp, rects + 4 * i, i, radius, xs0, xs1, n_blur, grid32 != 0,
                                   rec, sz);
        }
        s_slot[tid] = ok ? 1 : 0;
        s_planes[tid] = sz.planes;
        s_blurred[tid] = sz.blurred;
        s_scratch[tid] = sz.scratch;
        s_tiles[tid] = (int)(sz.tiles < (1l << 30) ? sz.tiles : (1l << 30));
        if (ok) {
            atomicMax(&s_max[0], rec.vw);
            atomicMax(&s_max[1], rec.vh);
            atomicMax(&s_max[2], rec.aw);
            atomicMax(&s_max[3], rec.ah);
            if (have && !have[i]) atomicAdd(&s_missing, 1);
            if (!layout_record_fits(rec)) atomicOr(&s_bad, 8);
        }
        __syncthreads();
        if (tid < 64) {
            long pl = s_run[0], bl = s_run[1], sc = s_run[2], tl = s_run[3];
            int k = s_count;
            const int cnt = min(LAY_THREADS, total - base);
            for (int t0 = 0; t0 < cnt; t0 += 64) {
                const int t = t0 + tid;
                const int has = s_slot[t];
                long v[4] = {has ? s_planes[t] : 0, has ? s_blurred[t] : 0, has ? s_scratch[t] : 0,
                             has ? (long)s_tiles[t] : 0};
                int one = has;
                const long own[4] = {v[0], v[1], v[2], v[3]};
#pragma unroll
                for (int off = 1; off < 64; off <<= 1) {
                    const int o1 = __shfl_up(one, off, 64);
                    long o[4];
#pragma unroll
                    for (int q = 0; q < 4; ++q) o[q] = __shfl_up(v[q], off, 64);
                    if (tid >= off) {
                        one += o1;
#pragma unroll
                        for (int q = 0; q < 4; ++q) v[q] += o[q];
                    }
                }
                s_slot[t] = has ? k + one - 1 : -1;
                s_planes[t] = pl + v[0] - own[0];
                s_blurred[t] = bl + v[1] - own[1];
                s_scratch[t] = sc + v[2] - own[2];
                const long toff = tl + v[3] - own[3];
                s_tiles[t] = (int)(toff < (1l << 30) ? toff : (1l << 30));
                k += __shfl(one, 63, 64);
                pl += __shfl(v[0], 63, 64);
                bl += __shfl(v[1], 63, 64);
                sc += __shfl(v[2], 63, 64);
                tl += __shfl(v[3], 63, 64);
            }
            for (int t = cnt + tid; t < LAY_THREADS; t += 64) s_slot[t] = -1;
            if (tid == 0) {
                s_run[0] = pl, s_run[1] = bl, s_run[2] = sc, s_run[3] = tl;
                s_count = k;
            }
        }
        __syncthreads();
        const int k = s_slot[tid];
        if (k >= 0 && k < b_nr) {
            rec.planes = planes + s_planes[tid];
            rec.blurred = blurred ? blurred + s_blurred[tid] + sz.lead : nullptr;
            rec.scratch = scratch ? scratch + s_scratch[tid] : nullptr;
            rec.tiles_off = s_tiles[tid];
            table[k] = rec;
        }
        __syncthreads();
    }
    const int nr = s_count;
    const long need_planes = s_run[0], need_blurred = s_run[1] + 32, need_scratch = s_run[2];
    int why = s_bad;
    if (need_planes > cap_planes || (n_blur > 0 && nr > 0 && (need_blurred > cap_blurred ||
                                                              need_scratch > cap_scratch)) ||
        (want_tiles && s_run[3] > cap_tiles))
        why |= 1;
    if (s_max[0] > b_vw || s_max[1] > b_vh || s_max[2] > b_aw || s_max[3] > b_ah) why |= 2;
    if (nr > b_nr) why |= 4;
    if (s_missing) why |= 16;
    for (int k = (why ? 0 : nr) + tid; k < b_nr; k += LAY_THREADS) table[k] = pano_patch{};
    if (tid == 0) {
        LayoutSummary out;
        out.planes_floats = need_planes;
        out.blurred_floats = need_blurred;
        out.scratch_floats = need_scratch;
        out.n_records = nr;
        out.n_tiles = (int)(s_run[3] < (1l << 30) ? s_run[3] : (1l << 30));
        out.max_vw = s_max[0], out.max_vh = s_max[1], out.max_aw = s_max[2], out.max_ah = s_max[3];
        out.missing = s_missing;
        out.ok = why == 0;
        out.why = why;
        out.pad = 0;
        *summary = out;
        if (check_expect &&
            !(out.ok && out.planes_floats == expect.planes_floats &&
              out.blurred_floats == expect.blurred_floats && out.scratch_floats == expect.scratch_floats &&
              out.n_records == expect.n_records && out.n_tiles == expect.n_tiles &&
              out.max_vw == expect.max_vw && out.max_vh == expect.max_vh && out.max_aw == expect.max_aw &&
              out.max_ah == expect.max_ah && out.missing == 0))
            *(volatile int *)sticky = 1;
    }
}

static int ensure_layout_buffers(pano_ctx *ctx, int n) {
    if (!ctx->lay_sum_host) {
        PANO_HIP(hipHostMalloc((void **)&ctx->lay_sum_host, sizeof(LayoutSummary) + 64, hipHostMallocDefault));
        memset(ctx->lay_sum_host, 0, sizeof(LayoutSummary) + 64);
    }
    if (n > ctx->lay_cap_n) {
        PANO_HIP(hipStreamSynchronize(ctx->stream));
        if (ctx->lay_rects_dev) PANO_HIP(hipFree(ctx->lay_rects_dev));
        if (ctx->lay_have_dev) PANO_HIP(hipFree(ctx->lay_have_dev));
        ctx->lay_rects_dev = nullptr;
        ctx->lay_have_dev = nullptr;
        PANO_HIP(hipMalloc((void **)&ctx->lay_rects_dev, (size_t)n * 4 * sizeof(int32_t)));
        PANO_HIP(hipMalloc((void **)&ctx->lay_have_dev, (size_t)n));
        ctx->lay_cap_n = n;
        ctx->lay_rects_host.clear();
        ctx->lay_have_host.clear();
    }
    return PANO_OK;
}

static LayoutSummary layout_expectation(const pano_layout &v) {
    LayoutSummary e = {};
    e.planes_floats = v.planes_floats, e.blurred_floats = v.blurred_floats;
    e.scratch_floats = v.scratch_floats;
    e.n_records = v.n_records, e.n_tiles = v.n_tiles;
    e.max_vw = v.max_vw, e.max_vh = v.max_vh, e.max_aw = v.max_aw, e.max_ah = v.max_ah;
    return e;
}
static int *layout_sticky(pano_ctx *ctx) {
    return (int *)((unsigned char *)ctx->lay_sum_host + sizeof(LayoutSummary));
}

static void stitch_signature(const pano_stitch_args *a, int tile_grid, int *sig) {
    const int v[STITCH_SIG] = {a->n, a->H, a->W, a->xs0, a->xs1, a->own0, a->own1, a->n_levels,
                               a->radius, a->max_spans, a->shortcut, a->min_gap, tile_grid};
    for (int k = 0; k < STITCH_SIG; ++k) sig[k] = v[k];
}

static int stitch_interior_map(pano_ctx *ctx, const pano_stitch_args *a, int n_blur) {
    if (a->classes && n_blur > 0 && ctx->opt[PANO_OPT_LEVEL_CLASSES]) {
        int radii[PANO_MAX_LEVELS];
        bool ascending = true;
        for (int k = 0; k < n_blur; ++k) {
            radii[k] = a->ntaps[k] / 2;
            if (k && radii[k] < radii[k - 1]) ascending = false;
        }
        if (ascending && radii[n_blur - 1] == a->radius)
            return pano_interior_classes(ctx, a->owner, a->H, a->W, a->own0, a->own1, radii, n_blur,
                                         a->block_owner, a->interior, a->classes);
    }
    return pano_interior_map(ctx, a->owner, a->H, a->W, a->own0, a->own1, a->radius, a->block_owner,
                             a->interior);
}

static bool stitch_has_classes(const pano_ctx *ctx, const pano_stitch_args *a, int n_blur) {
    if (!a->classes || n_blur <= 0 || !ctx->opt[PANO_OPT_LEVEL_CLASSES]) return false;
    for (int k = 0; k < n_blur; ++k)
        if (k && a->ntaps[k] / 2 < a->ntaps[k - 1] / 2) return false;
    return a->ntaps[n_blur - 1] / 2 == a->radius;
}

#define ON_SIDE(ctx, call)                  \
    do {                                    \
        const hipStream_t main_ = (ctx)->stream; \
        (ctx)->stream = (ctx)->side;        \
        const int rc_side_ = (call);        \
        (ctx)->stream = main_;              \
        if (rc_side_) return rc_side_;      \
    } while (0)

static int queue_tail(pano_ctx *ctx, pano_stitch_args *a, const pano_layout &lay, bool device_table,
                      int need_choice, bool two_streams, bool interior, int n_blur, int tile_grid,
                      bool kept = false) {
    const hipStream_t s = ctx->stream;
    const bool use_blur = n_blur > 0 && lay.n_records > 0;
    const int nr = lay.n_records;
    if (!device_table) {
        if (lay.planes_floats > a->planes_floats || (use_blur && lay.blurred_floats > a->blurred_floats) ||
            (use_blur && lay.scratch_floats > a->scratch_floats) ||
            (interior && lay.n_tiles > a->cap_tiles))
            return PANO_EGROW;
        PANO_REQUIRE(lay.planes_floats == 0 || a->planes, "pano_stitch_multiband: no plane arena");
        if (int rc = pano_layout_place(a->records_host, lay.n_records, a->planes, a->blurred, a->scratch))
            return rc;
        if (nr) {
            PANO_HIP(hipMemcpyAsync(a->table, a->records_host, (size_t)nr * sizeof(pano_patch),
                                    hipMemcpyHostToDevice, s));
            PANO_HIP(hipEventRecord(ctx->ev_upload, s));
            ctx->upload_pending = true;
        }
    }
    a->used_need = 0;
    if (kept) {
        a->used_need = need_choice == 1;
        two_streams = false;
    } else if (interior && tile_grid == 32 && nr && a->tile_flags && a->need) {
        bool on = need_choice == 1;
        if (need_choice < 0) {
            double sum = 0.0;
            for (int k = 0; k < nr; ++k) sum += a->records_host[k].aw;
            on = sum / nr >= 768.0;
        }
        if (on) {
            if (two_streams) {
                PANO_HIP(hipEventRecord(ctx->ev_join, ctx->side));
                PANO_HIP(hipStreamWaitEvent(s, ctx->ev_join, 0));
            }
            if (int rc = pano_blur_tiles(ctx, a->table, nr, lay.max_aw, lay.max_ah, a->W, a->radius,
                                         a->interior, a->tile_flags, a->need))
                return rc;
            a->used_need = 1;
        }
    }
    const bool fork2 = two_streams && interior && n_blur && nr &&
                       !a->used_need && tile_grid == 32 && a->tile_flags;
    if (fork2) {
        if (device_table) {
            PANO_HIP(hipEventRecord(ctx->ev_upload, s));
        }
        PANO_HIP(hipStreamWaitEvent(ctx->side, ctx->ev_upload, 0));
        ON_SIDE(ctx, pano_multiband_blur_prepare(ctx, a->table, nr, lay.max_aw, lay.max_ah, a->W,
                                                 a->interior, a->tile_flags));
        PANO_HIP(hipEventRecord(ctx->ev_join, ctx->side));
    } else if (two_streams && interior) {
        PANO_HIP(hipEventRecord(ctx->ev_join, ctx->side));
    }
    if (int rc = pano_warp_windows(ctx, a->cams, a->table, nr, lay.max_vw, lay.max_vh, a->sin_t,
                                   a->cos_t, a->tan_p, a->lut, a->lut_stride,
                                   a->used_need ? a->need : nullptr))
        return rc;
    if (two_streams && interior) PANO_HIP(hipStreamWaitEvent(s, ctx->ev_join, 0));
    if (kept && use_blur) {
        ctx->prepared_table = a->table;
        ctx->prepared_n = nr;
    }
    if (n_blur)
        if (int rc = pano_multiband_blur(ctx, a->table, nr, lay.max_aw, lay.max_vh, lay.max_ah,
                                         a->owner, a->W, a->taps, (const int *)a->ntaps, n_blur,
                                         interior ? a->interior : nullptr,
                                         interior ? a->tile_flags : nullptr))
            return rc;
    return pano_multiband_compose(ctx, a->table, nr, a->H, a->W, a->xs0, a->xs1, a->n_levels,
                                  a->owner, a->valid, interior ? a->interior : nullptr,
                                  interior && stitch_has_classes(ctx, a, n_blur) ? a->classes : nullptr,
                                  interior ? a->cams : nullptr, interior ? a->sin_t : nullptr,
                                  interior ? a->cos_t : nullptr, interior ? a->tan_p : nullptr,
                                  a->lut, a->lut_stride, a->mosaic, a->mosaic_f32);
}

static void geometry_buffers(const pano_stitch_args *a, const void *out[GEOM_BUFS]) {
    const void *v[GEOM_BUFS] = {a->owner, a->valid, a->table, a->interior, a->tile_flags, a->need,
                                a->planes, a->blurred, a->scratch, a->sin_t, a->classes};
    for (int k = 0; k < GEOM_BUFS; ++k) out[k] = v[k];
}
static void geometry_left(pano_ctx *ctx, const pano_stitch_args *a) {
    geometry_buffers(a, ctx->geom_bufs);
    ctx->geom_valid = true;
}

namespace {
struct StitchScope {
    pano_ctx *ctx;
    explicit StitchScope(pano_ctx *c) : ctx(c) { ctx->in_stitch = true; }
    ~StitchScope() { ctx->in_stitch = false; }
};
}

extern "C" int pano_stitch_multiband(pano_ctx *ctx, pano_stitch_args *a, int resume) {
    const bool geom_was_valid = ctx && ctx->geom_valid;
    PANO_ENTER(ctx, "pano_stitch_multiband");
    ctx->geom_valid = false;
    StitchScope scope(ctx);
    PANO_REQUIRE(a, "pano_stitch_multiband: null arguments");
    PANO_REQUIRE(a->cams && a->rects && a->sin_t && a->cos_t && a->tan_p && a->lut && a->owner &&
                     a->valid && a->marks && a->regions && a->regions_host && a->records_host &&
                     a->table && a->mosaic,
                 "pano_stitch_multiband: null pointer");
    PANO_REQUIRE(a->n > 0 && a->n <= 32767 && a->H > 0 && a->W > 0 && a->max_spans >= 1,
                 "pano_stitch_multiband: bad argument");
    PANO_REQUIRE(a->n_levels >= 1 && a->n_levels <= PANO_MAX_LEVELS,
                 "pano_stitch_multiband: n_levels %d outside [1, %d]", a->n_levels, PANO_MAX_LEVELS);
    PANO_REQUIRE(a->own0 <= a->xs0 && a->xs1 <= a->own1 && a->own0 >= 0 && a->own1 <= a->W,
                 "pano_stitch_multiband: strip [%d, %d) outside the ownership columns [%d, %d)",
                 a->xs0, a->xs1, a->own0, a->own1);
    PANO_REQUIRE(a->cap_records >= a->n * a->max_spans,
                 "pano_stitch_multiband: %d record slots for %d cameras x %d spans", a->cap_records,
                 a->n, a->max_spans);
    const int n_blur = a->n_levels - 1;
    PANO_REQUIRE(n_blur == 0 || (a->taps && a->ntaps), "pano_stitch_multiband: no tap tables");
    const bool interior = a->shortcut && n_blur > 0;
    PANO_REQUIRE(!interior || (a->block_owner && a->interior),
                 "pano_stitch_multiband: interior map without its buffers");
    const hipStream_t s = (hipStream_t)stream;
    if (int rc = pano_ctx_side_stream(ctx)) return rc;
    const bool big = (long long)a->H * (a->own1 - a->own0) >= (1ll << 24);
    const bool two_streams = ctx->opt[PANO_OPT_STITCH_STREAMS] != 0 && big;
    const int tile_grid = pano_blur_tile_grid(ctx);
    const int stride = 5 + 2 * a->max_spans;
    int sig[STITCH_SIG];
    stitch_signature(a, tile_grid, sig);

    if (!resume) {
        bool spec = ctx->opt[PANO_OPT_STITCH_ASYNC] != 0 && interior && tile_grid == 32 &&
                    ctx->lay_prev_valid && memcmp(sig, ctx->lay_prev_sig, sizeof(sig)) == 0 &&
                    ctx->lay_prev.n_records > 0 && a->planes && a->blurred && a->tile_flags;
        pano_layout bound = ctx->lay_prev;
        const bool want_keep = a->trust_layout == 3;
        const bool want_trust = a->trust_layout == 1 || want_keep;
        a->trust_layout = 0;
        if (ctx->trusted_pending && !(want_trust && spec))
            if (int rc = pano_stitch_verify(ctx)) return rc;
        const bool trusted = want_trust && spec && ctx->lay_prev_verified &&
                             ctx->opt[PANO_OPT_STITCH_ASYNC] == 1;
        const bool list_kept = n_blur == 0 || ctx->lay_prev.n_records == 0 ||
                               (ctx->item_buf && ctx->list_table == a->table &&
                                ctx->list_n == ctx->lay_prev.n_records);
        if (want_keep && trusted && geom_was_valid && tile_grid == 32 && list_kept) {
            const void *bufs[GEOM_BUFS];
            geometry_buffers(a, bufs);
            if (memcmp(bufs, ctx->geom_bufs, sizeof(bufs)) == 0) {
                if (int rc = queue_tail(ctx, a, ctx->lay_prev, true, ctx->lay_prev_used_need, false,
                                        interior, n_blur, tile_grid, true))
                    return rc;
                a->layout = ctx->lay_prev;
                a->trust_layout = 4;
                ctx->geom_valid = true;
                ++ctx->lay_count[0];
                return PANO_OK;
            }
        }
        if (spec) {
            if (int rc = ensure_layout_buffers(ctx, a->n)) return rc;
            const size_t nrect = (size_t)a->n * 4;
            if (ctx->lay_rects_host.size() != nrect ||
                memcmp(ctx->lay_rects_host.data(), a->rects, nrect * sizeof(int32_t)) != 0) {
                ctx->lay_rects_host.assign(a->rects, a->rects + nrect);
                PANO_HIP(hipMemcpyAsync(ctx->lay_rects_dev, ctx->lay_rects_host.data(),
                                        nrect * sizeof(int32_t), hipMemcpyHostToDevice, s));
            }
            std::vector<uint8_t> have(a->n, 1);
            if (a->have) have.assign(a->have, a->have + a->n);
            if (ctx->lay_have_host != have) {
                ctx->lay_have_host = have;
                PANO_HIP(hipMemcpyAsync(ctx->lay_have_dev, ctx->lay_have_host.data(), (size_t)a->n,
                                        hipMemcpyHostToDevice, s));
            }
            if (!trusted) {
                bound.n_records = bound.n_records + 2 < a->cap_records ? bound.n_records + 2 : a->cap_records;
                bound.max_vw += 64, bound.max_vh += 64, bound.max_aw += 64, bound.max_ah += 64;
            }
            if (ctx->opt[PANO_OPT_STITCH_ASYNC] == 2) {
                bound.n_records = ctx->lay_prev.n_records > 1 ? ctx->lay_prev.n_records - 1 : 1;
                bound.max_vw = ctx->lay_prev.max_vw - 1;
            }
        }
        if (int rc = pano_ownership_regions(ctx, a->cams, a->n, a->H, a->W, a->own0, a->own1,
                                            a->sin_t, a->cos_t, a->tan_p, a->owner, a->valid,
                                            a->min_gap, a->max_spans, a->marks, a->regions))
            return rc;
        const bool forked = two_streams;
        if (forked && interior) {
            PANO_HIP(hipEventRecord(ctx->ev_fork, s));
            PANO_HIP(hipStreamWaitEvent(ctx->side, ctx->ev_fork, 0));
            ON_SIDE(ctx, stitch_interior_map(ctx, a, n_blur));
        }
        bool interior_queued = forked && interior;
        if (spec) {
            if (ctx->upload_pending) {
                PANO_HIP(hipEventSynchronize(ctx->ev_upload));
                ctx->upload_pending = false;
            }
            uintptr_t bbase = (uintptr_t)a->blurred;
            bbase += (uintptr_t)(-(intptr_t)bbase) % 128;
            hipLaunchKernelGGL(layout_windows_kernel, dim3(1), dim3(LAY_THREADS), 0, s, a->regions,
                               ctx->lay_rects_dev, ctx->lay_have_dev, a->n, a->max_spans, a->radius,
                               a->xs0, a->xs1, n_blur, 1, a->planes, (float *)bbase, a->scratch,
                               (long)a->planes_floats, (long)a->blurred_floats,
                               (long)a->scratch_floats, a->cap_tiles, 1, bound.n_records,
                               bound.max_vw, bound.max_vh, bound.max_aw, bound.max_ah, a->table,
                               ctx->lay_sum_host, layout_expectation(ctx->lay_prev), trusted ? 1 : 0,
                               layout_sticky(ctx));
            PANO_LAUNCH_CHECK("layout_windows_kernel");
            PANO_HIP(hipEventRecord(ctx->ev_regions, s));
            if (!trusted) {
                PANO_HIP(hipStreamWaitEvent(ctx->side, ctx->ev_regions, 0));
                PANO_HIP(hipMemcpyAsync(a->records_host, a->table,
                                        (size_t)bound.n_records * sizeof(pano_patch),
                                        hipMemcpyDeviceToHost, ctx->side));
                PANO_HIP(hipEventRecord(ctx->ev_copy, ctx->side));
            }
            if (interior && !interior_queued) {
                if (int rc = stitch_interior_map(ctx, a, n_blur)) return rc;
                interior_queued = true;
            }
            if (int rc = queue_tail(ctx, a, bound, true, ctx->lay_prev_used_need, two_streams, interior,
                                    n_blur, tile_grid))
                return rc;
            if (trusted) {
                a->layout = ctx->lay_prev;
                a->used_need = ctx->lay_prev_used_need;
                a->trust_layout = 2;
                ctx->trusted_pending = true;
                geometry_left(ctx, a);
                ++ctx->lay_count[0];
                return PANO_OK;
            }
            PANO_HIP(hipEventSynchronize(ctx->ev_regions));
            PANO_HIP(hipEventSynchronize(ctx->ev_copy));
            const LayoutSummary sum = *ctx->lay_sum_host;
            a->layout.planes_floats = sum.planes_floats;
            a->layout.blurred_floats = sum.blurred_floats;
            a->layout.scratch_floats = sum.scratch_floats;
            a->layout.n_records = sum.n_records, a->layout.n_tiles = sum.n_tiles;
            a->layout.max_vw = sum.max_vw, a->layout.max_vh = sum.max_vh;
            a->layout.max_aw = sum.max_aw, a->layout.max_ah = sum.max_ah;
            a->layout.missing = sum.missing;
            if (sum.ok) {
                ctx->lay_prev = a->layout;
                ctx->lay_prev_used_need = a->used_need;
                ctx->lay_prev_verified = true;
                geometry_left(ctx, a);
                ++ctx->lay_count[0];
                return PANO_OK;
            }
            ++ctx->lay_count[1];
            ctx->lay_prev_valid = false;
            ctx->lay_prev_verified = false;
        }
        PANO_HIP(hipMemcpyAsync(a->regions_host, a->regions, (size_t)a->n * stride * sizeof(int32_t),
                                hipMemcpyDeviceToHost, s));
        PANO_HIP(hipEventRecord(ctx->ev_regions, s));
        if (interior && !interior_queued)
            if (int rc = stitch_interior_map(ctx, a, n_blur)) return rc;
        PANO_HIP(hipEventSynchronize(ctx->ev_regions));
        if (ctx->upload_pending) {
            PANO_HIP(hipEventSynchronize(ctx->ev_upload));
            ctx->upload_pending = false;
        }
        a->layout = pano_layout{};
        if (int rc = pano_layout_windows(tile_grid, a->regions_host, a->n, a->max_spans, a->rects,
                                         a->have, a->radius, a->xs0, a->xs1, n_blur,
                                         a->records_host, a->cap_records, &a->layout))
            return rc;
        if (a->layout.missing) {
            pano_set_error("pano_stitch_multiband: %d records of cameras whose frames are not "
                           "resident reach columns [%d, %d)", a->layout.missing, a->xs0, a->xs1);
            return PANO_EINVAL;
        }
    }
    const int rc = queue_tail(ctx, a, a->layout, false, a->warp_need, two_streams, interior, n_blur,
                              tile_grid);
    if (rc == PANO_OK) {
        ctx->lay_prev = a->layout;
        memcpy(ctx->lay_prev_sig, sig, sizeof(sig));
        ctx->lay_prev_used_need = a->used_need;
        ctx->lay_prev_valid = true;
        ctx->lay_prev_verified = true;
        geometry_left(ctx, a);
    }
    return rc;
}

extern "C" int pano_stitch_verify(pano_ctx *ctx) {
    PANO_REQUIRE(ctx, "pano_stitch_verify: null context");
    if (!ctx->trusted_pending) return PANO_OK;
    PANO_HIP(hipSetDevice(ctx->device));
    PANO_HIP(hipEventSynchronize(ctx->ev_regions));
    ctx->trusted_pending = false;
    const LayoutSummary sum = *ctx->lay_sum_host;
    const pano_layout &v = ctx->lay_prev;
    const int sticky = __atomic_exchange_n(layout_sticky(ctx), 0, __ATOMIC_SEQ_CST);
    const bool same = !sticky && sum.ok && sum.planes_floats == v.planes_floats &&
                      sum.blurred_floats == v.blurred_floats && sum.scratch_floats == v.scratch_floats &&
                      sum.n_records == v.n_records && sum.n_tiles == v.n_tiles &&
                      sum.max_vw == v.max_vw && sum.max_vh == v.max_vh && sum.max_aw == v.max_aw &&
                      sum.max_ah == v.max_ah && sum.missing == 0;
    if (!same) {
        ctx->lay_prev_valid = ctx->lay_prev_verified = false;
        ctx->geom_valid = false;
        pano_set_error("pano_stitch_verify: a trusted stitch laid out %d records (ok %d, why %d, an "
                       "earlier one differed: %d) where the verified layout has %d: the cameras were "
                       "not those of the verified stitch",
                       sum.n_records, sum.ok, sum.why, sticky, v.n_records);
        return PANO_EINVAL;
    }
    return PANO_OK;
}

extern "C" int pano_stitch_counts(const pano_ctx *ctx, int *device_layouts, int *fallbacks) {
    PANO_REQUIRE(ctx && device_layouts && fallbacks, "pano_stitch_counts: null pointer");
    *device_layouts = ctx->lay_count[0];
    *fallbacks = ctx->lay_count[1];
    return PANO_OK;
}
```

### pano360_amd/csrc/warp.hip

```cpp
#include "geom.h"

struct ProjK {
    double p[9];
};

template <bool FULL>
__global__ __launch_bounds__(256) void warp_spherical_kernel(
    const uint8_t *__restrict__ frame, int sh, int sw, ProjK K,
    const double *__restrict__ sin_t, const double *__restrict__ cos_t,
    const double *__restrict__ tan_p, const float *__restrict__ lut255,
    const double *__restrict__ hat_x, const double *__restrict__ hat_y,
    int gx0, int gy0, int pw, int ph, int pitch, float *__restrict__ planes,
    uint8_t *__restrict__ mask, float *__restrict__ map_x,
    float *__restrict__ map_y) {
    __shared__ float s_lut[256];
    s_lut[threadIdx.y * 64 + threadIdx.x] = lut255[threadIdx.y * 64 + threadIdx.x];
    __syncthreads();

    const int x = blockIdx.x * 64 + threadIdx.x;
    const int y = blockIdx.y * 4 + threadIdx.y;
    if (x >= pw || y >= ph) return;

    float px, py;
    const bool m = map_pixel(K.p, sin_t[gx0 + x], cos_t[gx0 + x], tan_p[gy0 + y], sw, sh,
                             px, py);
    const Taps tp = make_taps(px, py, sw, sh);
    const uint8_t *r0 = frame + (size_t)tp.y0 * sw * 3;
    const uint8_t *r1 = frame + (size_t)tp.y1 * sw * 3;
    const uint8_t *p00 = r0 + tp.x0 * 3, *p01 = r0 + tp.x1 * 3;
    const uint8_t *p10 = r1 + tp.x0 * 3, *p11 = r1 + tp.x1 * 3;
    const size_t plane = (size_t)ph * pitch;
    const size_t o = (size_t)y * pitch + x;
#pragma unroll
    for (int k = 0; k < 3; ++k)
        planes[k * plane + o] =
            lerp4(s_lut[p00[k]], s_lut[p01[k]], s_lut[p10[k]], s_lut[p11[k]], tp);
    if (FULL) {
        float a = alpha_at(hat_x, hat_y, tp);
        a = a * (m ? 0.0f : 1.0f);
        planes[3 * plane + o] = a;
        mask[(size_t)y * pw + x] = m ? 1 : 0;
        if (map_x) {
            map_x[(size_t)y * pw + x] = px;
            map_y[(size_t)y * pw + x] = py;
        }
    }
}

#define WARP_ROWS 4
__global__ __launch_bounds__(256) void warp_windows_kernel(
    const pano_camera *__restrict__ cams, const pano_patch *__restrict__ patches,
    const double *__restrict__ sin_t, const double *__restrict__ cos_t,
    const double *__restrict__ tan_p, const float *__restrict__ lut, int lut_stride,
    const uint8_t *__restrict__ need) {
    __shared__ float s_lut[256];
    const pano_patch p = patches[blockIdx.z];
    constexpr int BH = 4 * WARP_ROWS;
    if ((int)blockIdx.x * 64 >= p.vw || (int)blockIdx.y * BH >= p.vh) return;
    if (need) {
        const int ntx = ((p.ax0 + p.aw - 1) >> 5) - (p.ax0 >> 5) + 1;
        const int nty = ((p.ay0 + p.ah - 1) >> 5) - (p.ay0 >> 5) + 1;
        const int px0 = p.vx0 + (int)blockIdx.x * 64, py0 = p.vy0 + (int)blockIdx.y * BH;
        const int ty0 = min(max((py0 >> 5) - (p.ay0 >> 5), 0), nty - 1);
        const int ty1 = min(max(((py0 + BH - 1) >> 5) - (p.ay0 >> 5), 0), nty - 1);
        const int tx0 = min(max((px0 >> 5) - (p.ax0 >> 5), 0), ntx - 1);
        const int tx1 = min(max(((px0 + 63) >> 5) - (p.ax0 >> 5), 0), ntx - 1);
        bool any = false;
        for (int ty = ty0; ty <= ty1; ++ty)
            for (int tx = tx0; tx <= tx1; ++tx) any |= need[p.tiles_off + ty * ntx + tx] != 0;
        if (!any) return;
    }
    s_lut[threadIdx.y * 64 + threadIdx.x] =
        lut[(size_t)p.index * lut_stride + threadIdx.y * 64 + threadIdx.x];
    __syncthreads();

    const int x = blockIdx.x * 64 + threadIdx.x;
    const int y0 = blockIdx.y * BH + threadIdx.y;
    if (x >= p.vw || y0 >= p.vh) return;
    const pano_camera *cam = cams + p.index;
    const int sw = cam->sw, sh = cam->sh;
    const int gx = p.x0 + p.vx0 + x;
    const double s = table_f64(sin_t, gx), c = table_f64(cos_t, gx);
    double t[WARP_ROWS];
#pragma unroll
    for (int j = 0; j < WARP_ROWS; ++j)
        t[j] = table_f64(tan_p, p.y0 + p.vy0 + min(y0 + 4 * j, p.vh - 1));
    Taps tp[WARP_ROWS];
    TapBytes tb[WARP_ROWS];
    bool inner = true;
#pragma unroll
    for (int j = 0; j < WARP_ROWS; ++j) {
        float px, py;
        map_pixel(cam->proj, s, c, t[j], sw, sh, px, py);
        tp[j] = tap_base(px, py);
        inner &= taps_interior(tp[j], sw, sh);
    }
    if (__ballot(!inner) == 0ull) {
#pragma unroll
        for (int j = 0; j < WARP_ROWS; ++j) tb[j] = load_taps_interior(cam->frame, sw, tp[j]);
    } else {
#pragma unroll
        for (int j = 0; j < WARP_ROWS; ++j) {
            reflect_taps(tp[j], sw, sh);
            tb[j] = load_taps(cam->frame, sw, tp[j]);
        }
    }
    typedef __attribute__((address_space(1))) float *plane_ptr;
    typedef __attribute__((address_space(1))) char *byte_ptr;
    const size_t plane = (size_t)p.vh * p.vpitch;
    const byte_ptr out[3] = {(byte_ptr)p.planes, (byte_ptr)(p.planes + plane),
                             (byte_ptr)(p.planes + 2 * plane)};
#pragma unroll
    for (int j = 0; j < WARP_ROWS; ++j) {
        const int y = y0 + 4 * j;
        if (y >= p.vh) break;
        const uint32_t o = ((uint32_t)y * (uint32_t)p.vpitch + (uint32_t)x) * 4u;
#pragma unroll
        for (int k = 0; k < 3; ++k) {
            *(plane_ptr)(out[k] + o) = lerp4(lut_at(s_lut, tb[j].v[0][k]), lut_at(s_lut, tb[j].v[1][k]),
                                             lut_at(s_lut, tb[j].v[2][k]), lut_at(s_lut, tb[j].v[3][k]), tp[j]);
        }
    }
}

__global__ __launch_bounds__(256) void add_weights_kernel(
    const uint8_t *__restrict__ frame, int h, int w,
    const float *__restrict__ lut255, const double *__restrict__ hat_x,
    const double *__restrict__ hat_y, float4 *__restrict__ rgba) {
    const int x = blockIdx.x * 64 + threadIdx.x;
    const int y = blockIdx.y * 4 + threadIdx.y;
    if (x >= w || y >= h) return;
    const uint8_t *s = frame + ((size_t)y * w + x) * 3;
    float4 v;
    v.x = lut255[s[0]];
    v.y = lut255[s[1]];
    v.z = lut255[s[2]];
    v.w = (float)(hat_y[y] * hat_x[x]);
    rgba[(size_t)y * w + x] = v;
}

extern "C" int pano_add_weights(pano_ctx *ctx, const uint8_t *frame, int h, int w,
                                const float *lut255, const double *hat_x, const double *hat_y,
                                float *rgba) {
    PANO_ENTER(ctx, "pano_add_weights");
    PANO_REQUIRE(frame && lut255 && hat_x && hat_y && rgba, "pano_add_weights: null pointer");
    PANO_REQUIRE(h > 0 && w > 0, "pano_add_weights: bad shape %dx%d", h, w);
    dim3 block(64, 4), grid(ceil_div(w, 64), ceil_div(h, 4));
    PANO_TIMED(PK_ADD_WEIGHTS, (hipStream_t)stream,
               hipLaunchKernelGGL(add_weights_kernel, grid, block, 0, (hipStream_t)stream,
                                  frame, h, w, lut255, hat_x, hat_y, (float4 *)rgba));
    PANO_LAUNCH_CHECK("add_weights_kernel");
    return PANO_OK;
}

static int check_frame(const char *who, int sh, int sw, int pw, int ph, int gx0, int gy0) {
    PANO_REQUIRE(sh > 0 && sw > 0 && sh < 32767 && sw < 32767,
                 "%s: frame %dx%d outside (0, 32767)", who, sh, sw);
    PANO_REQUIRE(pw > 0 && ph > 0 && gx0 >= 0 && gy0 >= 0, "%s: bad rectangle", who);
    return PANO_OK;
}

extern "C" int pano_warp_spherical(pano_ctx *ctx, const uint8_t *frame, int sh, int sw,
                                   const double *proj, const double *sin_t, const double *cos_t,
                                   const double *tan_p, const float *lut255, const double *hat_x,
                                   const double *hat_y, int gx0, int gy0, int pw, int ph,
                                   float *planes, uint8_t *mask, float *map_x, float *map_y) {
    PANO_ENTER(ctx, "pano_warp_spherical");
    PANO_REQUIRE(frame && proj && sin_t && cos_t && tan_p && lut255 && hat_x &&
                     hat_y && planes && mask,
                 "pano_warp_spherical: null pointer");
    PANO_REQUIRE((map_x == nullptr) == (map_y == nullptr),
                 "pano_warp_spherical: map_x and map_y must both be given or both be NULL");
    if (int rc = check_frame("pano_warp_spherical", sh, sw, pw, ph, gx0, gy0)) return rc;
    ProjK K;
    for (int i = 0; i < 9; ++i) K.p[i] = proj[i];
    dim3 block(64, 4), grid(ceil_div(pw, 64), ceil_div(ph, 4));
    PANO_TIMED(PK_WARP, (hipStream_t)stream,
               hipLaunchKernelGGL(warp_spherical_kernel<true>, grid, block, 0,
                                  (hipStream_t)stream, frame, sh, sw, K, sin_t, cos_t, tan_p,
                                  lut255, hat_x, hat_y, gx0, gy0, pw, ph, pano_pitch_of(pw),
                                  planes, mask, map_x, map_y));
    PANO_LAUNCH_CHECK("warp_spherical_kernel");
    return PANO_OK;
}

extern "C" int pano_warp_windows(pano_ctx *ctx, const pano_camera *cams, const pano_patch *patches,
                                 int n, int max_vw, int max_vh, const double *sin_t,
                                 const double *cos_t, const double *tan_p, const float *lut,
                                 int lut_stride, const uint8_t *need) {
    PANO_ENTER(ctx, "pano_warp_windows");
    PANO_REQUIRE(cams && patches && sin_t && cos_t && tan_p && lut && lut_stride >= 0,
                 "pano_warp_windows: null pointer");
    PANO_REQUIRE(n >= 0 && n <= 65535 && max_vw >= 0 && max_vh >= 0,
                 "pano_warp_windows: bad argument");
    if (n == 0 || max_vw == 0 || max_vh == 0) return PANO_OK;
    dim3 block(64, 4), grid(ceil_div(max_vw, 64), ceil_div(max_vh, 4 * WARP_ROWS), n);
    PANO_TIMED(PK_WARP_WINDOWS, (hipStream_t)stream,
               hipLaunchKernelGGL(warp_windows_kernel, grid, block, 0, (hipStream_t)stream,
                                  cams, patches, sin_t, cos_t, tan_p, lut, lut_stride, need));
    PANO_LAUNCH_CHECK("warp_windows_kernel");
    return PANO_OK;
}
```

### pano360_amd/engine.py

```python
import ctypes as C

import numpy as np

from . import _lib
from ._lib import Patch

BORDER_SAMPLES = 100
MULTIBAND_PAD = 10


class SphProj:

    @staticmethod
    def hom2proj(pts):
        pts = np.asarray(pts)
        xz = np.sqrt(pts[:, 0] ** 2 + pts[:, 2] ** 2)
        theta = np.arctan2(pts[:, 0], pts[:, 2])
        phi = np.arctan2(pts[:, 1], xz)
        return np.stack([theta, phi], axis=-1)

    @staticmethod
    def proj2hom(pts):
        pts = np.asarray(pts)
        return np.stack([np.sin(pts[:, 0]), np.tan(pts[:, 1]),
# ... 388 lines not shown
        return self

    def __init__(self, records, eng):
        self.host = np.array(records, dtype=PATCH_DTYPE).reshape(-1)
        self.n = len(self.host)
        aw, ah = self.host["aw"].astype(np.int64), self.host["ah"].astype(np.int64)
        if eng.tile_grid == 32:
            ax0, ay0 = self.host["ax0"].astype(np.int64), self.host["ay0"].astype(np.int64)
            tiles = (((ax0 + aw - 1) >> 5) - (ax0 >> 5) + 1) * (((ay0 + ah - 1) >> 5) - (ay0 >> 5) + 1)
            tiles = np.where((aw > 0) & (ah > 0), tiles, 0)
        else:
            tiles = ((aw + 63) // 64) * ((ah + 127) // 128)
        self.host["tiles_off"] = np.concatenate([[0], np.cumsum(tiles)[:-1]]) if self.n else 0
        self.n_tiles = int(tiles.sum())
        self.dev = eng.to_device(self.host)
        mx = lambda k: int(self.host[k].max()) if self.n else 0
        self.max_vw, self.max_vh, self.max_aw, self.max_ah = (mx("vw"), mx("vh"), mx("aw"),
                                                              mx("ah"))

    @property
    def ptr(self):
        return _ptr(self.dev)


def patch_table(patches, eng):
    return PatchTable([p.record(i) for i, p in enumerate(patches)], eng)


class WindowInfo:

    def __init__(self, area, window):
        self.area, self.window = area, window


class FusedPatches:

    @classmethod
    def from_regions(cls, raw, max_spans, rects, have, radius, strip, n_blur, eng, rec=None):
        lib = _lib.lib()
        n = len(rects)
        if rec is None:
            rec = np.zeros(n * max_spans, dtype=PATCH_DTYPE)
        lay = _lib.Layout()
        raw = np.ascontiguousarray(raw, np.int32)
        rects = np.ascontiguousarray(rects, np.int32)
        have = np.ascontiguousarray(have, np.uint8)
        _lib.check(lib.pano_layout_windows(
            eng.tile_grid, raw.ctypes.data, n, max_spans, rects.ctypes.data, have.ctypes.data,
            radius,
            strip[0], strip[1], n_blur, rec.ctypes.data, len(rec), C.byref(lay)),
            "pano_layout_windows")
        rec = rec[:lay.n_records]
        if lay.missing:
            missing = sorted({int(i) for i in rec["index"] if not have[int(i)]})
            raise _lib.PanoError(f"frames {missing} are needed for columns [{strip[0]}, "
                                 f"{strip[1]}) but are not resident on this device")
        self = cls.__new__(cls)
        self.planes = eng.arena("planes", int(lay.planes_floats))
        self.blurred = eng.arena("blurred", int(lay.blurred_floats))
        self.scratch = eng.arena("scratch", int(lay.scratch_floats))
        _lib.check(lib.pano_layout_place(rec.ctypes.data, len(rec), self.planes.data_ptr(),
                                         self.blurred.data_ptr(), self.scratch.data_ptr()),
                   "pano_layout_place")
        self._area = self._window = None
        self.table = PatchTable.from_layout(rec, lay, eng)
        return self

    @classmethod
    def from_records(cls, rec, lay, table_dev, arenas):
        self = cls.__new__(cls)
        self.planes, self.blurred, self.scratch = arenas
        self._area = self._window = None
        table = PatchTable.__new__(PatchTable)
        table.host, table.n, table.n_tiles, table.dev = rec, len(rec), int(lay.n_tiles), table_dev
        table.max_vw, table.max_vh, table.max_aw, table.max_ah = (
            int(lay.max_vw), int(lay.max_vh), int(lay.max_aw), int(lay.max_ah))
        self.table = table
        return self

    def _rectangles(self):
        if self._area is None:
            h = self.table.host
            i64 = lambda k: h[k].astype(np.int64)
            self._area = np.stack([i64("ay0"), i64("ay0") + i64("ah"), i64("ax0"),
                                   i64("ax0") + i64("aw")], axis=1)
            self._window = np.stack([i64("vy0"), i64("vy0") + i64("vh"), i64("vx0"),
                                     i64("vx0") + i64("vw")], axis=1)
        return self._area, self._window

    @property
    def info(self):
        return [WindowInfo(tuple(int(v) for v in a), tuple(int(v) for v in w))
                for a, w in zip(*self._rectangles())]

    def __iter__(self):
        return iter(self.info)

    def __len__(self):
        return self.table.n

    @property
    def warped_pixels(self):
        return int((self.table.host["vh"].astype(np.int64) * self.table.host["vw"]).sum())

    @property
    def blurred_pixels(self):
        return int((self.table.host["ah"].astype(np.int64) * self.table.host["aw"]).sum())


class Engine:

    def __init__(self, device=None, blur="mfma", own_prune=True):
        torch = _torch()
        self.lib = _lib.lib()
        if not torch.cuda.is_available() or self.lib.pano_device_count() < 1:
            raise _lib.PanoError("no MI355X visible: the HIP path has no CPU fallback")
        self.device = torch.device(device if device is not None
                                   else f"cuda:{torch.cuda.current_device()}")
        index = self.device.index if self.device.index is not None else torch.cuda.current_device()
        self.device = torch.device("cuda", index)
        self._device_index = index
        handle = C.c_void_p()
        self._ctx_stream = torch.cuda.current_stream(self.device).cuda_stream
        _lib.check(self.lib.pano_ctx_create(index, C.c_void_p(self._ctx_stream), C.byref(handle)),
                   "pano_ctx_create")
        self._ctx = handle
        if blur not in ("mfma", "valu"):
            raise ValueError(f"blur kernel {blur!r}: 'mfma' or 'valu'")
        self.set_option(_lib.OPT_BLUR_KERNEL, _lib.BLUR_VALU if blur == "valu" else _lib.BLUR_MFMA)
        self.set_option(_lib.OPT_OWN_PRUNE, 1 if own_prune else 0)
        self.tile_grid = int(self.lib.pano_blur_tile_grid(self._ctx))
        self.interior_block = int(self.lib.pano_interior_block())
        lut = np.arange(256, dtype=np.float32) / np.float32(255)
        self.lut255 = torch.from_numpy(lut).to(self.device)
        self._hats = {}
        self._taps = {}
        self._region_bufs = {}
        self._arenas = {}
        self._ring = None
        self.warp_need = "auto"
        self._cam_template = None
        self.native_stitch = True
        self._stitch_ws = {}
        self._plans = PlanMemo()
        self.trust_layout = False
        self.keep_geometry = False
        self.last_kept_geometry = False
        self._trusted = None

    def __del__(self):
        ctx, self._ctx = getattr(self, "_ctx", None), None
        if ctx is not None and ctx.value:
            try:
                self.lib.pano_ctx_destroy(ctx)
            except Exception:
                pass

    def ctx(self, stream=None):
        raw = (stream.cuda_stream if stream is not None
               else _torch()._C._cuda_getCurrentRawStream(self._device_index))
        if raw != self._ctx_stream:
            _lib.check(self.lib.pano_ctx_set_stream(self._ctx, C.c_void_p(raw)),
                       "pano_ctx_set_stream")
            self._ctx_stream = raw
        return self._ctx

    def set_option(self, option, value):
        _lib.check(self.lib.pano_ctx_set_option(self._ctx, option, int(value)),
                   "pano_ctx_set_option")
        if option == _lib.OPT_BLUR_KERNEL:
            self.tile_grid = int(self.lib.pano_blur_tile_grid(self._ctx))
        self._trusted = None

    def get_option(self, option):
        value = C.c_int(0)
        _lib.check(self.lib.pano_ctx_get_option(self._ctx, option, C.byref(value)),
                   "pano_ctx_get_option")
        return value.value

    def stitch_counts(self):
        ok, back = C.c_int(0), C.c_int(0)
        _lib.check(self.lib.pano_stitch_counts(self._ctx, C.byref(ok), C.byref(back)),
                   "pano_stitch_counts")
        return ok.value, back.value

    def timing(self, on):
        _lib.check(self.lib.pano_timing_enable(self._ctx, 1 if on else 0), "pano_timing_enable")

    def kernel_times(self):
        out = {}
        for kid in range(self.lib.pano_kernel_count()):
            ms, n = C.c_double(), C.c_int()
            _lib.check(self.lib.pano_timing_read(self._ctx, kid, C.byref(ms), C.byref(n)),
                       "pano_timing_read")
            if n.value:
                out[self.lib.pano_kernel_name(kid).decode()] = (ms.value, n.value)
        return out

    def arena(self, name, floats):
        torch = _torch()
        have = self._arenas.get(name)
        if have is None or have.numel() < floats:
            self._arenas[name] = None
            have = self._arenas[name] = torch.empty(int(floats * 1.125) + 4,
                                                    dtype=torch.float32, device=self.device)
        return have

    def to_device(self, array):
        if self._ring is None:
            self._ring = _PinnedRing(self.device)
        return self._ring.upload(array)

    def hat_tables(self, shape):
        torch = _torch()
        if shape not in self._hats:
            h, w = shape
            self._hats[shape] = (torch.from_numpy(hat(w)).to(self.device),
                                 torch.from_numpy(hat(h)).to(self.device))
        return self._hats[shape]

    def blur_tables(self, n_levels):
        if n_levels not in self._taps:
            sig = level_sigmas(n_levels)
            sizes = [gaussian_ksize(s) for s in sig]
            rmax = max([k // 2 for k in sizes], default=0)
            flat = np.concatenate([padded_taps(gaussian_taps(k, s), (rmax - k // 2) & 3)
                                   for k, s in zip(sizes, sig)]) if sig else np.zeros(1, np.float32)
            self._taps[n_levels] = (np.ascontiguousarray(flat, np.float32),
                                    (C.c_int * max(len(sizes), 1))(*sizes), len(sizes), rmax)
        return self._taps[n_levels]

    def upload_frames(self, imgs):
        torch = _torch()
        return [im.to(self.device) if isinstance(im, torch.Tensor) else
                torch.from_numpy(np.ascontiguousarray(im, np.uint8)).to(self.device)
                for im in imgs]

    def cached_plan(self, shapes, rots, intrs, padded, max_resolution, table_cols=None):
        return self._plans.get(shapes, rots, intrs, padded, max_resolution, table_cols,
                               make=lambda *a: self.upload_plan(Plan(*a)))

    def upload_plan(self, plan):
        torch = _torch()
        nx, ny = len(plan.sin_t), len(plan.tan_p)
        dev = self.to_device(np.concatenate([plan.sin_t, plan.cos_t, plan.tan_p])).view(
            torch.float64)
        plan.dev = (dev[:nx], dev[nx:2 * nx], dev[2 * nx:2 * nx + ny])
        return plan

    def add_weights(self, frame, lut=None):
        torch = _torch()
        h, w = frame.shape[:2]
        hx, hy = self.hat_tables((h, w))
        out = torch.empty((h, w, 4), dtype=torch.float32, device=self.device)
        lut = self.lut255 if lut is None else lut
        _lib.check(self.lib.pano_add_weights(self.ctx(), _ptr(frame), h, w, _ptr(lut), _ptr(hx),
                                             _ptr(hy), _ptr(out)),
                   "pano_add_weights")
        return out

    def warp(self, frame, plan, index, patch, want_maps=False, lut=None):
        torch = _torch()
        lut = self.lut255 if lut is None else lut
        sh, sw = frame.shape[:2]
        hx, hy = self.hat_tables((sh, sw))
        y0, _, x0, _ = plan.rects[index]
        mx = my = None
        if want_maps:
            mx = torch.empty((patch.h, patch.w), dtype=torch.float32, device=self.device)
            my = torch.empty_like(mx)
        proj = plan.projs[index]
        _lib.check(self.lib.pano_warp_spherical(
            self.ctx(), _ptr(frame), sh, sw, proj.ctypes.data_as(C.c_void_p), _ptr(plan.dev[0]),
            _ptr(plan.dev[1]), _ptr(plan.dev[2]), _ptr(lut), _ptr(hx), _ptr(hy),
            x0, y0, patch.w, patch.h, _ptr(patch.planes), _ptr(patch.mask), _ptr(mx),
            _ptr(my)), "pano_warp_spherical")
        return mx, my

    def warp_all(self, frames, plan, n_blur=0, want_maps=False, luts=None):
        patches, maps = [], []
        for i, frame in enumerate(frames):
            patch = DevicePatch(plan.rects[i], self.device, n_blur)
            maps.append(self.warp(frame, plan, i, patch, want_maps,
                                  None if luts is None else luts[i]))
            patches.append(patch)
        return patches, maps

    def ownership(self, table, shape):
        torch = _torch()
        H, W = shape
        owner = torch.empty((H, W), dtype=torch.int16, device=self.device)
        valid = torch.empty((H, W), dtype=torch.uint8, device=self.device)
        _lib.check(self.lib.pano_ownership(self.ctx(), table.ptr, table.n, H, W, _ptr(owner),
                                           _ptr(valid)), "pano_ownership")
        return owner, valid

    def multiband(self, patches, shape, n_levels, want_float=False, table=None):
        if table is None:
            table = patch_table(patches, self)
        owner, valid = self.ownership(table, shape)
        mosaic, fl = self.blur_and_compose(table, owner, valid, shape, n_levels, want_float)
        return mosaic, fl, owner, valid

    def interior_map(self, owner, radius, strip=None):
        torch = _torch()
        H, W = owner.shape
        c0, c1 = strip if strip is not None else (0, W)
        ib = self.interior_block
        shape8 = ((H + ib - 1) // ib, (W + ib - 1) // ib)
        bown = torch.empty((2,) + shape8, dtype=torch.int16, device=self.device)
        interior = torch.empty(shape8, dtype=torch.uint8, device=self.device)
        _lib.check(self.lib.pano_interior_map(self.ctx(), _ptr(owner), H, W, c0, c1, radius,
                                              _ptr(bown), _ptr(interior)), "pano_interior_map")
        return interior

    def interior_classes(self, owner, radii, strip=None):
        torch = _torch()
        H, W = owner.shape
        c0, c1 = strip if strip is not None else (0, W)
        ib = self.interior_block
        shape8 = ((H + ib - 1) // ib, (W + ib - 1) // ib)
        bown = torch.empty((2,) + shape8, dtype=torch.int16, device=self.device)
        interior = torch.empty(shape8, dtype=torch.uint8, device=self.device)
        classes = torch.empty(shape8, dtype=torch.uint8, device=self.device)
        arr = (C.c_int * len(radii))(*[int(r) for r in radii])
        _lib.check(self.lib.pano_interior_classes(self.ctx(), _ptr(owner), H, W, c0, c1, arr,
                                                  len(radii), _ptr(bown), _ptr(interior),
                                                  _ptr(classes)), "pano_interior_classes")
        return interior, classes

    def level_radii(self, n_levels):
        return [gaussian_ksize(s) // 2 for s in level_sigmas(n_levels)]

    COLUMN_COST_SHARES = (0.27, 0.25, 2.5)

    def column_costs(self, plan, n_levels, shortcut=True):
        torch = _torch()
        H, W = plan.shape
        if not hasattr(plan, "dev"):
            self.upload_plan(plan)
        n_blur, radius = self.blur_tables(n_levels)[2:]
        owner, valid = self.ownership_cameras(plan)
        a, b, g = self.COLUMN_COST_SHARES
        cost = np.full(W, a / W)
        per = valid.ne(0).sum(0, dtype=torch.int64).cpu().numpy().astype(np.float64)
        if per.sum() > 0:
            cost += b * per / per.sum()
        if n_blur and shortcut:
            interior = self.interior_map(owner, radius)
            near = interior.eq(0).sum(0, dtype=torch.int64).cpu().numpy().astype(np.float64)
            near = np.repeat(near, self.interior_block)[:W]
            if near.sum() > 0:
                cost += g * near / near.sum()
        elif per.sum() > 0:
            cost += g * per / per.sum()
        return cost

    def active_tile_pixels(self):
        table, flags = getattr(self, "last_tiles", (None, None))
        if table is None:
            return 0
        host = table.host
        if flags is None:
            return int((host["ah"].astype(np.int64) * host["aw"]).sum())
        if self.tile_grid == 32:
            return int(flags[:table.n_tiles].to(_torch().int64).sum().item()) * 1024
        on = flags.cpu().numpy()
        total = 0
        for rec in host:
            ntx, nty = (int(rec["aw"]) + 63) // 64, (int(rec["ah"]) + 127) // 128
            if ntx * nty == 0:
                continue
            grid = on[int(rec["tiles_off"]):int(rec["tiles_off"]) + ntx * nty].reshape(nty, ntx)
            wx = np.minimum(64, int(rec["aw"]) - 64 * np.arange(ntx))
            wy = np.minimum(128, int(rec["ah"]) - 128 * np.arange(nty))
            total += int((grid.astype(np.int64) * wy[:, None] * wx[None, :]).sum())
        return total

    def gather_bytes(self, shape, n_levels):
        torch = _torch()
        table, flags = getattr(self, "last_tiles", (None, None))
        classes = getattr(self, "last_classes", None)
        if table is None:
            return None
        H, W = shape
        nb = n_levels - 1
        host = table.host
        interior = getattr(self, "last_interior", None)
        if flags is None or (classes is None and interior is None):
            return float((host["ah"].astype(np.int64) * host["aw"]).sum()) * (12 + 16 * nb)
        if classes is None:
            classes = interior * nb
        ib = self.interior_block
        px = classes.repeat_interleave(ib, 0).repeat_interleave(ib, 1)[:H, :W]
        per_class = torch.tensor([12 + 16 * nb] + [12 + 16 * (nb - j) for j in range(1, nb)] + [0],
                                 dtype=torch.float64, device=self.device)
        total = torch.zeros((), dtype=torch.float64, device=self.device)
        for rec in host:
            aw, ah = int(rec["aw"]), int(rec["ah"])
            if aw <= 0 or ah <= 0:
                continue
            y0, x0 = int(rec["y0"]) + int(rec["ay0"]), int(rec["x0"]) + int(rec["ax0"])
            sub = px[max(y0, 0):min(y0 + ah, H), max(x0, 0):min(x0 + aw, W)]
            if sub.numel():
                counts = torch.bincount(sub.reshape(-1).long(), minlength=nb + 1)[:nb + 1]
                total += (counts.double() * per_class).sum()
        mid = ((px > 0) & (px < nb)).sum().double() * 12.0
        return float((total + mid).item())

    def blur_and_compose(self, table, owner, valid, shape, n_levels, want_float=False,
                         strip=None, interior=None, cams=None, plan=None, luts=None, flags=None,
                         mosaic_out=None, classes=None):
        torch = _torch()
        H, W = shape
        c0, c1 = strip if strip is not None else (0, W)
        taps, ntaps, n_blur, _ = self.blur_tables(n_levels)
        if n_blur:
            if flags is None and interior is not None:
                flags = torch.empty(max(table.n_tiles, 1), dtype=torch.uint8, device=self.device)
            _lib.check(self.lib.pano_multiband_blur(
                self.ctx(), table.ptr, table.n, table.max_aw, table.max_vh, table.max_ah,
                _ptr(owner), W, taps.ctypes.data, ntaps, n_blur, _ptr(interior), _ptr(flags)),
                "pano_multiband_blur")
            self.last_tiles = (table, flags)
        mosaic = (mosaic_out if mosaic_out is not None else
                  torch.empty((H, W, 3), dtype=torch.uint8, device=self.device))
        fl = (torch.empty((H, W, 3), dtype=torch.float32, device=self.device)
              if want_float else None)
        tabs = plan.dev if interior is not None else (None, None, None)
        _lib.check(self.lib.pano_multiband_compose(
            self.ctx(), table.ptr, table.n, H, W, c0, c1, n_levels, _ptr(owner), _ptr(valid),
            _ptr(interior), _ptr(classes) if interior is not None else None,
            _ptr(cams) if interior is not None else None, _ptr(tabs[0]),
            _ptr(tabs[1]), _ptr(tabs[2]), *self._lut_args(luts), _ptr(mosaic), _ptr(fl)),
            "pano_multiband_compose")
        return mosaic, fl

    def simple_blend(self, patches, shape, linear, table=None):
        torch = _torch()
        H, W = shape
        if table is None:
            table = patch_table(patches, self)
        mosaic = torch.empty((H, W, 3), dtype=torch.uint8, device=self.device)
        fn = self.lib.pano_linear_blend if linear else self.lib.pano_no_blend
        _lib.check(fn(self.ctx(), table.ptr, table.n, H, W, _ptr(mosaic)),
                   "pano_linear_blend" if linear else "pano_no_blend")
        return mosaic

    def _lut_args(self, luts):
        if luts is None:
            return _ptr(self.lut255), 0
        return _ptr(luts), 256

    def equalize_gains(self, frames, rots, intrs, chunk_bytes=256 << 20):
        torch = _torch()
        n = len(frames)
        h, w = (int(v) for v in frames[0].shape[:2])
        if any(tuple(f.shape[:2]) != (h, w) for f in frames):
            raise ValueError("equalize_gains: every overlap is sized by regions[0] "
                             "(stitcher.py:41); frames of different sizes cannot be indexed")
        pairs = overlap_pairs(rots, intrs, w, h)
        overlaps, sizes = np.zeros((n, n)), np.zeros((n, n))
        if len(pairs):
            hx, hy = self.hat_tables((h, w))
            rec = np.zeros(n, dtype=CAMERA_DTYPE)
            for k, frame in enumerate(frames):
                rec[k] = (np.zeros(9), frame.data_ptr(), hx.data_ptr(), hy.data_ptr(), h, w,
                          0, 0, 0, 0)
            cams = self.to_device(rec)
            nblk = int(self.lib.pano_overlap_blocks(h, w))
            bw0 = min(1024 // min(16, h), w)
            step = max(1, chunk_bytes // (nblk * 24))
            stats = torch.empty((len(pairs), 3), dtype=torch.float64, device=self.device)
            partials = torch.empty((min(step, len(pairs)), nblk, 3), dtype=torch.float64,
                                   device=self.device)
            for a in range(0, len(pairs), step):
                part = pairs[a:a + step]
                dev_pairs = torch.from_numpy(part.view(np.uint8).reshape(-1)).to(self.device)
                _lib.check(self.lib.pano_overlap_stats(
                    self.ctx(), _ptr(cams), _ptr(dev_pairs), len(part), h, w, bw0,
                    _ptr(self.lut255),
                    _ptr(partials), _ptr(stats[a:])), "pano_overlap_stats")
            host = stats.cpu().numpy()
            for (_, i, j), (count, sum_i, sum_j) in zip(pairs, host):
                sizes[i, j] = sizes[j, i] = count
                if count:
                    overlaps[i, j] = np.float32(sum_i / (3.0 * count))
                    overlaps[j, i] = np.float32(sum_j / (3.0 * count))
        gains = find_gains(overlaps, sizes)
        luts = torch.from_numpy(gain_tables(gains)).to(self.device)
        return overlaps, sizes, gains, luts

    def camera_table(self, plan, frames=None):
        key = (tuple(plan.shapes),
               tuple(sorted((i, f.data_ptr()) for i, f in frames.items())) if frames else ())
        kept = getattr(plan, "_cams", None)
        if kept is not None and kept[0] == key and kept[1] is self:
            return kept[2]
        if self._cam_template is None or self._cam_template[0] != key:
            rec = np.zeros(plan.n, dtype=CAMERA_DTYPE)
            for i in range(plan.n):
                sh, sw = plan.shapes[i]
                hx, hy = self.hat_tables((sh, sw))
                frame = frames.get(i) if frames else None
                rec[i] = (np.zeros(9), frame.data_ptr() if frame is not None else 0,
                          hx.data_ptr(), hy.data_ptr(), sh, sw, 0, 0, 0, 0)
            self._cam_template = (key, rec)
        rec = self._cam_template[1].copy()
        rec["proj"] = np.asarray(plan.projs, np.float64).reshape(plan.n, 9)
        rects = np.asarray(plan.rects, np.int32)
        rec["y0"], rec["x0"] = rects[:, 0], rects[:, 2]
        rec["h"], rec["w"] = rects[:, 1] - rects[:, 0], rects[:, 3] - rects[:, 2]
        dev = self.to_device(rec)
        plan._cams = (key, self, dev)
        return dev

    def ownership_cameras(self, plan, strip=None, out=None, cams=None):
        torch = _torch()
        H, W = plan.shape
        if out is None:
            owner = torch.empty((H, W), dtype=torch.int16, device=self.device)
            valid = torch.empty((H, W), dtype=torch.uint8, device=self.device)
        else:
            owner, valid = out
        xs0, xs1 = strip if strip is not None else (0, W)
        if cams is None:
            cams = self.camera_table(plan)
        _lib.check(self.lib.pano_ownership_cameras(
            self.ctx(), _ptr(cams), plan.n, H, W, xs0, xs1, _ptr(plan.dev[0]), _ptr(plan.dev[1]),
            _ptr(plan.dev[2]), _ptr(owner), _ptr(valid)),
            "pano_ownership_cameras")
        return owner, valid

    def ownership_regions(self, plan, strip=None, min_gap=0, max_spans=4, cams=None):
        torch = _torch()
        H, W = plan.shape
        owner = torch.empty((H, W), dtype=torch.int16, device=self.device)
        valid = torch.empty((H, W), dtype=torch.uint8, device=self.device)
        marks = torch.empty((plan.n, W), dtype=torch.uint8, device=self.device)
        regions = torch.empty((plan.n, 5 + 2 * max_spans), dtype=torch.int32, device=self.device)
        xs0, xs1 = strip if strip is not None else (0, W)
        if cams is None:
            cams = self.camera_table(plan)
        _lib.check(self.lib.pano_ownership_regions(
            self.ctx(), _ptr(cams), plan.n, H, W, xs0, xs1, _ptr(plan.dev[0]), _ptr(plan.dev[1]),
            _ptr(plan.dev[2]), _ptr(owner), _ptr(valid), min_gap, max_spans, _ptr(marks),
            _ptr(regions)), "pano_ownership_regions")
        return owner, valid, regions, marks

    def owned_regions_async(self, owner, n, strip=None, min_gap=0, max_spans=4):
        torch = _torch()
        H, W = owner.shape
        c0, c1 = strip if strip is not None else (0, W)
        marks = torch.empty((n, W), dtype=torch.uint8, device=self.device)
        regions = torch.empty((n, 5 + 2 * max_spans), dtype=torch.int32, device=self.device)
        _lib.check(self.lib.pano_owned_regions(
            self.ctx(), _ptr(owner), H, W, c0, c1, n, min_gap, max_spans,
                                               _ptr(marks), _ptr(regions)),
                   "pano_owned_regions")
        key = (n, max_spans)
        host_buf = self._region_bufs.get(key)
        if host_buf is None:
            host_buf = self._region_bufs[key] = torch.empty(
                (n, 5 + 2 * max_spans), dtype=torch.int32).pin_memory()
        host_buf.copy_(regions, non_blocking=True)
        done = torch.cuda.Event()
        done.record(torch.cuda.current_stream(self.device))

        def wait():
            done.synchronize()
            host = host_buf.numpy().copy()
            spans = [host[i, 5:5 + 2 * host[i, 4]].reshape(-1, 2) for i in range(n)]
            return host[:, :4], spans
        wait.raw = lambda: (done.synchronize(), host_buf.numpy())[1]
        wait.max_spans = max_spans
        return wait

    def owned_regions(self, owner, n, strip=None, min_gap=0, max_spans=4):
        return self.owned_regions_async(owner, n, strip, min_gap, max_spans)()

    def owned_boxes(self, owner, n, strip=None):
        return self.owned_regions(owner, n, strip)[0]

    def multiband_fused(self, frames, plan, n_levels, want_float=False, frame_ids=None,
                        strip=None, shortcut=True, luts=None, mosaic_out=None):
        H, W = plan.shape
        c0, c1 = strip if strip is not None else (0, W)
        taps, ntaps, n_blur, radius = self.blur_tables(n_levels)
        ib = self.interior_block
        margin = (max(radius, ib * ((radius + 2 * ib - 2) // ib) + ib - 1) if shortcut and n_blur
                  else radius)
        ext = (max(c0 - margin, 0), min(c1 + margin, W))
        ids = list(range(plan.n)) if frame_ids is None else list(frame_ids)
        have = dict(zip(ids, frames))
        cams = self.camera_table(plan, have)
        if self.native_stitch:
            return self._stitch_native(plan, cams, have, n_levels, want_float, (c0, c1), ext,
                                       shortcut, luts, mosaic_out)
        owner, valid = self.ownership_cameras(plan, strip=ext, cams=cams)
        regions = self.owned_regions_async(owner, plan.n, ext, 2 * radius + 2)
        interior = classes = None
        if shortcut and n_blur:
            if self.get_option(_lib.OPT_LEVEL_CLASSES):
                interior, classes = self.interior_classes(owner, self.level_radii(n_levels), ext)
            else:
                interior = self.interior_map(owner, radius, ext)
        resident = np.zeros(plan.n, np.uint8)
        resident[[i for i in have if 0 <= i < plan.n]] = 1
        rects32 = np.ascontiguousarray(plan.rects, np.int32)
        records = np.zeros(plan.n * regions.max_spans, dtype=PATCH_DTYPE)
        patches = FusedPatches.from_regions(regions.raw(), regions.max_spans, rects32,
                                            resident, radius, (c0, c1), n_blur, self, records)
        table = patches.table
        flags = need = None
        wide = table.n and float(np.mean(table.host["aw"])) >= 768.0
        choice = self.warp_need
        if (interior is not None and n_blur and self.tile_grid == 32
                and (choice is True or (choice == "auto" and wide))):
            torch = _torch()
            flags = torch.empty(max(table.n_tiles, 1), dtype=torch.uint8, device=self.device)
            need = torch.empty(max(table.n_tiles, 1), dtype=torch.uint8, device=self.device)
            _lib.check(self.lib.pano_blur_tiles(
                self.ctx(), table.ptr, table.n, table.max_aw, table.max_ah, plan.shape[1], radius,
                _ptr(interior), _ptr(flags), _ptr(need)), "pano_blur_tiles")
        _lib.check(self.lib.pano_warp_windows(
            self.ctx(), _ptr(cams), table.ptr, table.n, table.max_vw, table.max_vh,
            _ptr(plan.dev[0]),
            _ptr(plan.dev[1]), _ptr(plan.dev[2]), *self._lut_args(luts), _ptr(need)), "pano_warp_windows")
        mosaic, fl = self.blur_and_compose(table, owner, valid, plan.shape, n_levels,
                                           want_float, (c0, c1), interior, cams, plan, luts,
                                           flags=flags, mosaic_out=mosaic_out, classes=classes)
        self.last_classes, self.last_interior = classes, interior
        return mosaic, fl, valid, patches

    def _stitch_workspace(self, H, W, n, max_spans):
        torch = _torch()
        key = (H, W, n, max_spans)
        ws = self._stitch_ws.get(key)
        if ws is None:
            if len(self._stitch_ws) >= 4:
                self._stitch_ws.clear()
            ib = self.interior_block
            shape8 = ((H + ib - 1) // ib, (W + ib - 1) // ib)
            dev = self.device
            stride = 5 + 2 * max_spans
            cap = n * max_spans
            ws = dict(
                marks=torch.empty((n, W), dtype=torch.uint8, device=dev),
                regions=torch.empty((n, stride), dtype=torch.int32, device=dev),
                regions_host=torch.empty((n, stride), dtype=torch.int32).pin_memory(),
                bown=torch.empty((2,) + shape8, dtype=torch.int16, device=dev),
                interior=torch.zeros(shape8, dtype=torch.uint8, device=dev),
                classes=torch.zeros(shape8, dtype=torch.uint8, device=dev),
                records_host=torch.empty(cap * PATCH_DTYPE.itemsize, dtype=torch.uint8).pin_memory(),
                table=torch.empty(cap * PATCH_DTYPE.itemsize, dtype=torch.uint8, device=dev),
                cap=cap, tiles=None, need=None, cap_tiles=0, have=np.zeros(n, np.uint8),
                args=_lib.StitchArgs())
            self._stitch_ws[key] = ws
        return ws

    def _stitch_native(self, plan, cams, have, n_levels, want_float, strip, ext, shortcut, luts,
                       mosaic_out):
        torch = _torch()
        H, W = plan.shape
        taps, ntaps, n_blur, radius = self.blur_tables(n_levels)
        max_spans = 4
        ws = self._stitch_workspace(H, W, plan.n, max_spans)
        a = ws["args"]
        mosaic = (mosaic_out if mosaic_out is not None else
                  torch.empty((H, W, 3), dtype=torch.uint8, device=self.device))
        fl = (torch.empty((H, W, 3), dtype=torch.float32, device=self.device)
              if want_float else None)
        resident = ws["have"]
        resident[:] = 0
        resident[[i for i in have if 0 <= i < plan.n]] = 1
        rects32 = np.ascontiguousarray(plan.rects, np.int32)
        lut, lut_stride = self._lut_args(luts)
        ptr = lambda t: t.data_ptr() if t is not None else None
        a.cams, a.rects, a.have = ptr(cams), rects32.ctypes.data, resident.ctypes.data
        a.sin_t, a.cos_t, a.tan_p = (ptr(t) for t in plan.dev)
        a.lut, a.lut_stride = lut, lut_stride
        a.taps, a.ntaps = taps.ctypes.data, C.cast(ntaps, C.c_void_p)
        a.mosaic, a.mosaic_f32 = ptr(mosaic), ptr(fl)
        a.marks, a.regions, a.regions_host = ptr(ws["marks"]), ptr(ws["regions"]), ptr(ws["regions_host"])
        a.block_owner, a.interior = ptr(ws["bown"]), ptr(ws["interior"])
        a.classes = ptr(ws["classes"])
        a.records_host, a.table, a.cap_records = ptr(ws["records_host"]), ptr(ws["table"]), ws["cap"]
        a.n, a.H, a.W = plan.n, H, W
        a.xs0, a.xs1, a.own0, a.own1 = strip[0], strip[1], ext[0], ext[1]
        a.n_levels, a.radius, a.shortcut = n_levels, radius, 1 if shortcut else 0
        a.warp_need = {True: 1, False: 0}.get(self.warp_need, -1)
        a.max_spans, a.min_gap = max_spans, 2 * radius + 2
        sig = (id(plan), strip, ext, n_levels, bool(shortcut), fl is not None, luts is None,
               tuple(sorted(have)), tuple(id(self._arenas.get(k)) for k in ("planes", "blurred", "scratch")),
               id(ws["tiles"]))
        kept = self._trusted
        repeat = (self.trust_layout and kept is not None and kept[0] == sig and kept[1] is plan)
        a.trust_layout = (3 if self.keep_geometry else 1) if repeat else 0
        if repeat and self.keep_geometry:
            owner, valid = kept[3], kept[4]
        else:
            owner = torch.empty((H, W), dtype=torch.int16, device=self.device)
            valid = torch.empty((H, W), dtype=torch.uint8, device=self.device)
        a.owner, a.valid = ptr(owner), ptr(valid)
        resume = 0
        a.layout.missing = a.layout.n_records = 0
        while True:
            arenas = [self._arenas.get(k) for k in ("planes", "blurred", "scratch")]
            for k, t in zip(("planes", "blurred", "scratch"), arenas):
                setattr(a, k, ptr(t))
                setattr(a, k + "_floats", t.numel() - 64 if t is not None else 0)
            a.tile_flags, a.need, a.cap_tiles = ptr(ws["tiles"]), ptr(ws["need"]), ws["cap_tiles"]
            status = self.lib.pano_stitch_multiband(self.ctx(), C.byref(a), resume)
            if status != _lib.EGROW:
                break
            lay = a.layout
            self.arena("planes", int(lay.planes_floats) + 64)
            self.arena("blurred", int(lay.blurred_floats) + 64)
            self.arena("scratch", int(lay.scratch_floats) + 64)
            if lay.n_tiles > ws["cap_tiles"]:
                ws["cap_tiles"] = int(lay.n_tiles * 1.25) + 64
                ws["tiles"] = torch.empty(ws["cap_tiles"], dtype=torch.uint8, device=self.device)
                ws["need"] = torch.empty(ws["cap_tiles"], dtype=torch.uint8, device=self.device)
            resume = 1
        if status != 0:
            if status == _lib.EINVAL and a.layout.missing:
                rec = ws["records_host"].numpy().view(PATCH_DTYPE)[:a.layout.n_records]
                missing = sorted({int(i) for i in rec["index"] if not resident[int(i)]})
                raise _lib.PanoError(f"frames {missing} are needed for columns [{strip[0]}, "
                                     f"{strip[1]}) but are not resident on this device")
            _lib.check(status, "pano_stitch_multiband")
        lay = a.layout
        if a.trust_layout in (2, 4):
            patches = kept[2]
            if self.keep_geometry:
                self._trusted = kept[:3] + (owner, valid)
            self.last_kept_geometry = a.trust_layout == 4
        else:
            rec = ws["records_host"].numpy().view(PATCH_DTYPE)[:lay.n_records].copy()
            patches = FusedPatches.from_records(
                rec, lay, ws["table"][:lay.n_records * PATCH_DTYPE.itemsize],
                tuple(self._arenas.get(k) for k in ("planes", "blurred", "scratch")))
            sig = sig[:-2] + (tuple(id(self._arenas.get(k)) for k in ("planes", "blurred", "scratch")),
                              id(ws["tiles"]))
            self._trusted = ((sig, plan, patches) + ((owner, valid) if self.keep_geometry else (None, None))
                             if self.trust_layout else None)
            self.last_kept_geometry = False
        if n_blur:
            self.last_tiles = (patches.table, ws["tiles"] if shortcut else None)
        self.last_classes = (ws["classes"] if shortcut and n_blur
                             and self.get_option(_lib.OPT_LEVEL_CLASSES) else None)
        self.last_interior = ws["interior"] if shortcut and n_blur else None
        return mosaic, fl, valid, patches

    def trust_layouts(self, on=True, keep_geometry=False):
        self.trust_layout = bool(on)
        self.keep_geometry = bool(on and keep_geometry)
        self._trusted = None
        self.set_option(_lib.OPT_STITCH_ASYNC, 1 if on else 0)
        return self

    def verify_trusted(self):
        _lib.check(self.lib.pano_stitch_verify(self._ctx), "pano_stitch_verify")

    def blend_fused(self, frames, plan, linear, frame_ids=None, strip=None, luts=None):
        torch = _torch()
        H, W = plan.shape
        c0, c1 = strip if strip is not None else (0, W)
        ids = list(range(plan.n)) if frame_ids is None else list(frame_ids)
        have = dict(zip(ids, frames))
        missing = [i for i, (_, _, x0, x1) in enumerate(plan.rects)
                   if x0 < c1 and x1 > c0 and i not in have]
        if missing:
            raise _lib.PanoError(f"frames {missing} are needed for columns [{c0}, {c1}) "
                                 "but are not resident on this device")
        cams = self.camera_table(plan, have)
        mosaic = torch.empty((H, W, 3), dtype=torch.uint8, device=self.device)
        valid = torch.empty((H, W), dtype=torch.uint8, device=self.device)
        _lib.check(self.lib.pano_blend_cameras(
            self.ctx(), _ptr(cams), plan.n, H, W, c0, c1, 1 if linear else 0, _ptr(plan.dev[0]),
            _ptr(plan.dev[1]), _ptr(plan.dev[2]), *self._lut_args(luts), _ptr(mosaic),
            _ptr(valid)), "pano_blend_cameras")
        return mosaic, valid

    def crop_rect(self, valid):
        torch = _torch()
        H, W = valid.shape
        heights = torch.empty((H, W), dtype=torch.int32, device=self.device)
        result = torch.zeros(6, dtype=torch.int64, device=self.device)
        _lib.check(self.lib.pano_crop_rect(
            self.ctx(), _ptr(valid), H, W, _ptr(heights), _ptr(result)), "pano_crop_rect")
        res = result.cpu().numpy()
        if not res[0]:
            return None
        return tuple(int(v) for v in res[1:5])

    def plane_taps(self, ksize, sigma):
        key = ("plane", int(ksize), float(sigma))
        if key not in self._taps:
            self._taps[key] = np.ascontiguousarray(padded_taps(gaussian_taps(ksize, sigma)))
        return self._taps[key]

    def blur_plane(self, plane, ksize, sigma, out=None):
        torch = _torch()
        h, w = plane.shape
        pitch = (w + 3) & ~3
        if pitch == w and plane.is_contiguous():
            src = plane
        else:
            src = torch.zeros((h, pitch), dtype=torch.float32, device=self.device)
            src[:, :w] = plane
        dst = out if out is not None and pitch == w else torch.empty_like(src)
        tmp = torch.empty_like(src)
        _lib.check(self.lib.pano_blur_plane(
            self.ctx(), _ptr(src), _ptr(dst), _ptr(tmp), h, w, pitch,
            self.plane_taps(ksize, sigma).ctypes.data, ksize), "pano_blur_plane")
        return dst[:, :w]

    def pyr_down(self, plane):
        torch = _torch()
        plane = plane.contiguous()
        h, w = plane.shape
        out = torch.empty(((h + 1) // 2, (w + 1) // 2), dtype=torch.float32,
                          device=self.device)
        _lib.check(self.lib.pano_pyr_down(self.ctx(), _ptr(plane), h, w, _ptr(out)),
                   "pano_pyr_down")
        return out

    def stitch(self, frames, plan, blend="multiband", n_levels=5, want_float=False,
               fused=True, shortcut=True, luts=None):
        if not hasattr(plan, "dev"):
            self.upload_plan(plan)
        if blend == "multiband" and fused:
            return self.multiband_fused(frames, plan, n_levels, want_float, shortcut=shortcut,
                                        luts=luts)
        if fused:
            mosaic, valid = self.blend_fused(frames, plan, blend == "linear", luts=luts)
            return mosaic, None, valid, []
        n_blur = n_levels - 1 if blend == "multiband" else 0
        patches, _ = self.warp_all(frames, plan, n_blur, luts=luts)
        table = patch_table(patches, self)
        if blend == "multiband":
            mosaic, fl, _, valid = self.multiband(patches, plan.shape, n_levels, want_float,
                                                  table)
            return mosaic, fl, valid, patches
        mosaic = self.simple_blend(patches, plan.shape, blend == "linear", table)
        return mosaic, None, None, patches


_engine = None


def engine():
    global _engine
    if _engine is None:
        _engine = Engine()
    return _engine
```

Measured before the change: 203,600 MP/s.

## Shade interior mosaic pixels inside warp kernel; compose only seam pixels

Adds a warp variant that writes interior (single-owner) mosaic pixels straight to the output while warping, so the compose kernel skips those pixels and handles only seam regions. The stream sync is also reordered: the main stream waits on the side stream's interior map before warping rather than before blur. This avoids a second pass over interior pixels in compose. The cost is an earlier cross-stream dependency and warp-kernel work that now depends on the interior map and block owners.

```diff
diff --git a/include/pano360.h b/include/pano360.h
--- a/include/pano360.h
+++ b/include/pano360.h
@@ -113,6 +113,13 @@
                       const double *cos_t, const double *tan_p, const float *lut,
                       int lut_stride, const uint8_t *need);
 
+int pano_warp_windows_mosaic(pano_ctx *ctx, const pano_camera *cams, const pano_patch *patches,
+                             int n, int max_vw, int max_vh, const double *sin_t,
+                             const double *cos_t, const double *tan_p, const float *lut,
+                             int lut_stride, const uint8_t *need, const uint8_t *interior,
+                             const int16_t *block_owner, int H, int W, int xs0, int xs1,
+                             uint8_t *mosaic, float *mosaic_f32);
+
 int pano_ownership(pano_ctx *ctx, const pano_patch *patches, int n, int H, int W,
                    int16_t *owner, uint8_t *valid);
 
@@ -161,6 +168,13 @@
                            const double *sin_t, const double *cos_t, const double *tan_p,
                            const float *lut, int lut_stride, uint8_t *mosaic,
                            float *mosaic_f32);
+int pano_multiband_compose_seams(pano_ctx *ctx, const pano_patch *patches, int n, int H, int W,
+                                 int xs0, int xs1, int n_levels, const int16_t *owner,
+                                 const uint8_t *valid, const uint8_t *interior,
+                                 const uint8_t *classes, const pano_camera *cams,
+                                 const double *sin_t, const double *cos_t, const double *tan_p,
+                                 const float *lut, int lut_stride, uint8_t *mosaic,
+                                 float *mosaic_f32);
 
 int pano_blend_cameras(pano_ctx *ctx, const pano_camera *cams, int n, int H, int W,
                        int xs0, int xs1, int linear, const double *sin_t,
diff --git a/pano360_amd/_lib.py b/pano360_amd/_lib.py
--- a/pano360_amd/_lib.py
+++ b/pano360_amd/_lib.py
@@ -106,6 +106,8 @@
     "pano_warp_spherical": (_i, [_vp, _vp, _i, _i, _vp, _vp, _vp, _vp, _vp, _vp, _vp, _i, _i, _i,
                                  _i, _vp, _vp, _vp, _vp]),
     "pano_warp_windows": (_i, [_vp, _vp, _vp, _i, _i, _i, _vp, _vp, _vp, _vp, _i, _vp]),
+    "pano_warp_windows_mosaic": (_i, [_vp, _vp, _vp, _i, _i, _i, _vp, _vp, _vp, _vp, _i, _vp, _vp, _vp,
+                                      _i, _i, _i, _i, _vp, _vp]),
     "pano_blur_tiles": (_i, [_vp, _vp, _i, _i, _i, _i, _i, _vp, _vp, _vp]),
     "pano_ownership": (_i, [_vp, _vp, _i, _i, _i, _vp, _vp]),
     "pano_ownership_cameras": (_i, [_vp, _vp, _i, _i, _i, _i, _i, _vp, _vp, _vp, _vp, _vp]),
@@ -121,6 +123,8 @@
     "pano_interior_classes": (_i, [_vp, _vp, _i, _i, _i, _i, _vp, _i, _vp, _vp, _vp]),
     "pano_multiband_compose": (_i, [_vp, _vp, _i, _i, _i, _i, _i, _i, _vp, _vp, _vp, _vp, _vp, _vp,
                                     _vp, _vp, _vp, _i, _vp, _vp]),
+    "pano_multiband_compose_seams": (_i, [_vp, _vp, _i, _i, _i, _i, _i, _i, _vp, _vp, _vp, _vp, _vp,
+                                          _vp, _vp, _vp, _vp, _i, _vp, _vp]),
     "pano_blend_cameras": (_i, [_vp, _vp, _i, _i, _i, _i, _i, _i, _vp, _vp, _vp, _vp, _i, _vp,
                                 _vp]),
     "pano_blur_tile_grid": (_i, [_vp]),
diff --git a/pano360_amd/csrc/api.hip b/pano360_amd/csrc/api.hip
--- a/pano360_amd/csrc/api.hip
+++ b/pano360_amd/csrc/api.hip
@@ -116,6 +116,7 @@
     if (ctx->ev_regions) (void)hipEventDestroy(ctx->ev_regions);
     if (ctx->ev_upload) (void)hipEventDestroy(ctx->ev_upload);
     if (ctx->ev_copy) (void)hipEventDestroy(ctx->ev_copy);
+    if (ctx->ev_interior) (void)hipEventDestroy(ctx->ev_interior);
     delete ctx;
     return PANO_OK;
 }
@@ -126,6 +127,7 @@
     if (!ctx->ev_fork) PANO_HIP(hipEventCreateWithFlags(&ctx->ev_fork, hipEventDisableTiming));
     if (!ctx->ev_join) PANO_HIP(hipEventCreateWithFlags(&ctx->ev_join, hipEventDisableTiming));
     if (!ctx->ev_copy) PANO_HIP(hipEventCreateWithFlags(&ctx->ev_copy, hipEventDisableTiming));
+    if (!ctx->ev_interior) PANO_HIP(hipEventCreateWithFlags(&ctx->ev_interior, hipEventDisableTiming));
     if (!ctx->side) PANO_HIP(hipStreamCreateWithFlags(&ctx->side, hipStreamNonBlocking));
     return PANO_OK;
 }
diff --git a/pano360_amd/csrc/blend.hip b/pano360_amd/csrc/blend.hip
--- a/pano360_amd/csrc/blend.hip
+++ b/pano360_amd/csrc/blend.hip
@@ -710,13 +710,13 @@
 }
 
 #define COMPOSE_MASKS 4
-template <int L, bool PERCAM, bool CLS>
+template <int L, bool PERCAM, bool CLS, bool INTERIOR_DONE>
 __global__ __launch_bounds__(256) void multiband_compose_kernel(
     const pano_patch *__restrict__ patches, int n, int H, int W, int xs0, int xs1,
     const int16_t *__restrict__ owner, const uint8_t *__restrict__ valid,
     uint8_t *__restrict__ mosaic, float *__restrict__ mosaic_f32, InteriorArgs ia) {
     __shared__ float s_lut[256];
-    if (ia.interior && !PERCAM) {
+    if (!INTERIOR_DONE && ia.interior && !PERCAM) {
         s_lut[threadIdx.y * 64 + threadIdx.x] = ia.lut[threadIdx.y * 64 + threadIdx.x];
         __syncthreads();
     }
@@ -741,6 +741,7 @@
     }
     if (!inside) return;
     if (is_interior) {
+        if (INTERIOR_DONE) return;
         const int own = owner[(size_t)y * W + x];
         if (PERCAM)
             shade_interior_of<LUT_GLOBAL>(own, ia.lut, 256, ia, x, y, W, mosaic, mosaic_f32);
@@ -1133,6 +1134,57 @@
                                classes, "pano_interior_classes");
 }
 
+static int compose_launch(pano_ctx *ctx, const char *who, bool done, const pano_patch *patches, int n,
+                          int H, int W, int xs0, int xs1, int n_levels, const int16_t *owner,
+                          const uint8_t *valid, const uint8_t *interior, const uint8_t *classes,
+                          const pano_camera *cams, const double *sin_t, const double *cos_t,
+                          const double *tan_p, const float *lut, int lut_stride, uint8_t *mosaic,
+                          float *mosaic_f32) {
+    void *const stream = (void *)ctx->stream;
+    if (int rc = check_table(patches, n, H, W, who)) return rc;
+    PANO_REQUIRE(H > 0 && W > 0, "%s: bad mosaic shape %dx%d", who, H, W);
+    PANO_REQUIRE(owner && mosaic && valid, "%s: null pointer", who);
+    PANO_REQUIRE(n_levels >= 1 && n_levels <= PANO_MAX_LEVELS, "%s: n_levels %d outside [1, %d]", who,
+                 n_levels, PANO_MAX_LEVELS);
+    PANO_REQUIRE(xs0 >= 0 && xs1 <= W && xs0 <= xs1, "%s: bad strip [%d, %d)", who, xs0, xs1);
+    PANO_REQUIRE(!interior || (cams && sin_t && cos_t && tan_p && lut),
+                 "%s: the interior map needs cameras, tables and LUT", who);
+    PANO_REQUIRE(lut_stride == 0 || lut_stride == 256,
+                 "%s: lut_stride %d (0 = shared table, 256 = per camera)", who, lut_stride);
+    PANO_REQUIRE(!done || (interior && n_levels > 1),
+                 "%s: needs the interior map (and so more than one level)", who);
+    if (xs0 == xs1) return PANO_OK;
+    PANO_REQUIRE(!classes || interior, "%s: level classes without the interior map", who);
+    InteriorArgs ia = {interior, ceil_div(W, IB), cams, sin_t, cos_t, tan_p, lut,
+                       ctx->opt[PANO_OPT_LEVEL_CLASSES] ? classes : nullptr};
+    const bool percam = interior && lut_stride != 0;
+    dim3 block(64, 4), grid(ceil_div(xs1 - xs0, 64), ceil_div(H, 4));
+    hipStream_t s = (hipStream_t)stream;
+#define COMPOSE_AS(L, PC, CL, DN)                                                        \
+    PANO_TIMED(PK_COMPOSE, s,                                                           \
+               hipLaunchKernelGGL((multiband_compose_kernel<L, PC, CL, DN>), grid, block, 0, s, \
+                                  patches, n, H, W, xs0, xs1, owner, valid, mosaic,     \
+                                  mosaic_f32, ia))
+#define COMPOSE(L)                                                                      \
+    case L:                                                                             \
+        if (done && L > 1) {                                                            \
+            if (ia.classes) COMPOSE_AS(L, false, true, (L > 1));                        \
+            else COMPOSE_AS(L, false, false, (L > 1));                                  \
+        } else if (ia.classes && L > 1) {                                               \
+            if (percam) COMPOSE_AS(L, true, true, false); else COMPOSE_AS(L, false, true, false); \
+        } else {                                                                        \
+            if (percam) COMPOSE_AS(L, true, false, false); else COMPOSE_AS(L, false, false, false); \
+        }                                                                               \
+        break;
+    switch (n_levels) {
+        COMPOSE(1) COMPOSE(2) COMPOSE(3) COMPOSE(4) COMPOSE(5) COMPOSE(6) COMPOSE(7) COMPOSE(8)
+    }
+#undef COMPOSE_AS
+#undef COMPOSE
+    PANO_LAUNCH_CHECK("multiband_compose_kernel");
+    return PANO_OK;
+}
+
 extern "C" int pano_multiband_compose(pano_ctx *ctx, const pano_patch *patches, int n, int H,
                                       int W, int xs0, int xs1, int n_levels, const int16_t *owner,
                                       const uint8_t *valid, const uint8_t *interior,
@@ -1141,45 +1193,23 @@
                                       const double *cos_t, const double *tan_p, const float *lut,
                                       int lut_stride, uint8_t *mosaic, float *mosaic_f32) {
     PANO_ENTER(ctx, "pano_multiband_compose");
-    if (int rc = check_table(patches, n, H, W, "pano_multiband_compose")) return rc;
-    PANO_REQUIRE(H > 0 && W > 0, "pano_multiband_compose: bad mosaic shape %dx%d", H, W);
-    PANO_REQUIRE(owner && mosaic && valid, "pano_multiband_compose: null pointer");
-    PANO_REQUIRE(n_levels >= 1 && n_levels <= PANO_MAX_LEVELS,
-                 "pano_multiband_compose: n_levels %d outside [1, %d]", n_levels, PANO_MAX_LEVELS);
-    PANO_REQUIRE(xs0 >= 0 && xs1 <= W && xs0 <= xs1,
-                 "pano_multiband_compose: bad strip [%d, %d)", xs0, xs1);
-    PANO_REQUIRE(!interior || (cams && sin_t && cos_t && tan_p && lut),
-                 "pano_multiband_compose: the interior map needs cameras, tables and LUT");
-    PANO_REQUIRE(lut_stride == 0 || lut_stride == 256,
-                 "pano_multiband_compose: lut_stride %d (0 = shared table, 256 = per camera)",
-                 lut_stride);
-    if (xs0 == xs1) return PANO_OK;
-    PANO_REQUIRE(!classes || interior, "pano_multiband_compose: level classes without the interior map");
-    InteriorArgs ia = {interior, ceil_div(W, IB), cams, sin_t, cos_t, tan_p, lut,
-                       ctx->opt[PANO_OPT_LEVEL_CLASSES] ? classes : nullptr};
-    const bool percam = interior && lut_stride != 0;
-    dim3 block(64, 4), grid(ceil_div(xs1 - xs0, 64), ceil_div(H, 4));
-    hipStream_t s = (hipStream_t)stream;
-#define COMPOSE_AS(L, PC, CL)                                                            \
-    PANO_TIMED(PK_COMPOSE, s,                                                           \
-               hipLaunchKernelGGL((multiband_compose_kernel<L, PC, CL>), grid, block, 0, s, \
-                                  patches, n, H, W, xs0, xs1, owner, valid, mosaic,     \
-                                  mosaic_f32, ia))
-#define COMPOSE(L)                                                                      \
-    case L:                                                                             \
-        if (ia.classes && L > 1) {                                                      \
-            if (percam) COMPOSE_AS(L, true, true); else COMPOSE_AS(L, false, true);     \
-        } else {                                                                        \
-            if (percam) COMPOSE_AS(L, true, false); else COMPOSE_AS(L, false, false);   \
-        }                                                                               \
-        break;
-    switch (n_levels) {
-        COMPOSE(1) COMPOSE(2) COMPOSE(3) COMPOSE(4) COMPOSE(5) COMPOSE(6) COMPOSE(7) COMPOSE(8)
-    }
-#undef COMPOSE_AS
-#undef COMPOSE
-    PANO_LAUNCH_CHECK("multiband_compose_kernel");
-    return PANO_OK;
+    return compose_launch(ctx, "pano_multiband_compose", false, patches, n, H, W, xs0, xs1, n_levels,
+                          owner, valid, interior, classes, cams, sin_t, cos_t, tan_p, lut, lut_stride,
+                          mosaic, mosaic_f32);
+}
+
+extern "C" int pano_multiband_compose_seams(pano_ctx *ctx, const pano_patch *patches, int n, int H,
+                                            int W, int xs0, int xs1, int n_levels,
+                                            const int16_t *owner, const uint8_t *valid,
+                                            const uint8_t *interior, const uint8_t *classes,
+                                            const pano_camera *cams, const double *sin_t,
+                                            const double *cos_t, const double *tan_p,
+                                            const float *lut, int lut_stride, uint8_t *mosaic,
+                                            float *mosaic_f32) {
+    PANO_ENTER(ctx, "pano_multiband_compose_seams");
+    return compose_launch(ctx, "pano_multiband_compose_seams", true, patches, n, H, W, xs0, xs1,
+                          n_levels, owner, valid, interior, classes, cams, sin_t, cos_t, tan_p, lut,
+                          lut_stride, mosaic, mosaic_f32);
 }
 
 extern "C" int pano_linear_blend(pano_ctx *ctx, const pano_patch *patches, int n, int H, int W,
diff --git a/pano360_amd/csrc/common.h b/pano360_amd/csrc/common.h
--- a/pano360_amd/csrc/common.h
+++ b/pano360_amd/csrc/common.h
@@ -104,7 +104,7 @@
     uint64_t used;
 };
 
-#define GEOM_BUFS 11
+#define GEOM_BUFS 12
 #define STITCH_SIG 13
 struct pano_ctx {
     int device;
@@ -123,6 +123,7 @@
     std::vector<PanoTapSet> tap_sets;
     uint64_t tick;
     hipEvent_t ev_regions, ev_upload, ev_fork, ev_join, ev_copy;
+    hipEvent_t ev_interior;
     hipStream_t side;
     bool upload_pending;
     LayoutSummary *lay_sum_host;
diff --git a/pano360_amd/csrc/stitch.hip b/pano360_amd/csrc/stitch.hip
--- a/pano360_amd/csrc/stitch.hip
+++ b/pano360_amd/csrc/stitch.hip
@@ -228,6 +228,10 @@
             ctx->upload_pending = true;
         }
     }
+    if (two_streams && interior && !kept) {
+        PANO_HIP(hipEventRecord(ctx->ev_interior, ctx->side));
+        PANO_HIP(hipStreamWaitEvent(s, ctx->ev_interior, 0));
+    }
     a->used_need = 0;
     if (kept) {
         a->used_need = need_choice == 1;
@@ -240,10 +244,6 @@
             on = sum / nr >= 768.0;
         }
         if (on) {
-            if (two_streams) {
-                PANO_HIP(hipEventRecord(ctx->ev_join, ctx->side));
-                PANO_HIP(hipStreamWaitEvent(s, ctx->ev_join, 0));
-            }
             if (int rc = pano_blur_tiles(ctx, a->table, nr, lay.max_aw, lay.max_ah, a->W, a->radius,
                                          a->interior, a->tile_flags, a->need))
                 return rc;
@@ -260,14 +260,20 @@
         ON_SIDE(ctx, pano_multiband_blur_prepare(ctx, a->table, nr, lay.max_aw, lay.max_ah, a->W,
                                                  a->interior, a->tile_flags));
         PANO_HIP(hipEventRecord(ctx->ev_join, ctx->side));
-    } else if (two_streams && interior) {
-        PANO_HIP(hipEventRecord(ctx->ev_join, ctx->side));
-    }
-    if (int rc = pano_warp_windows(ctx, a->cams, a->table, nr, lay.max_vw, lay.max_vh, a->sin_t,
-                                   a->cos_t, a->tan_p, a->lut, a->lut_stride,
-                                   a->used_need ? a->need : nullptr))
+    }
+    if (interior) {
+        if (int rc = pano_warp_windows_mosaic(ctx, a->cams, a->table, nr, lay.max_vw, lay.max_vh,
+                                              a->sin_t, a->cos_t, a->tan_p, a->lut, a->lut_stride,
+                                              a->used_need ? a->need : nullptr, a->interior,
+                                              a->block_owner, a->H, a->W, a->xs0, a->xs1, a->mosaic,
+                                              a->mosaic_f32))
+            return rc;
+    } else if (int rc = pano_warp_windows(ctx, a->cams, a->table, nr, lay.max_vw, lay.max_vh, a->sin_t,
+                                          a->cos_t, a->tan_p, a->lut, a->lut_stride,
+                                          a->used_need ? a->need : nullptr)) {
         return rc;
-    if (two_streams && interior) PANO_HIP(hipStreamWaitEvent(s, ctx->ev_join, 0));
+    }
+    if (fork2) PANO_HIP(hipStreamWaitEvent(s, ctx->ev_join, 0));
     if (kept && use_blur) {
         ctx->prepared_table = a->table;
         ctx->prepared_n = nr;
@@ -278,17 +284,21 @@
                                          interior ? a->interior : nullptr,
                                          interior ? a->tile_flags : nullptr))
             return rc;
+    if (interior)
+        return pano_multiband_compose_seams(ctx, a->table, nr, a->H, a->W, a->xs0, a->xs1, a->n_levels,
+                                            a->owner, a->valid, a->interior,
+                                            stitch_has_classes(ctx, a, n_blur) ? a->classes : nullptr,
+                                            a->cams, a->sin_t, a->cos_t, a->tan_p, a->lut,
+                                            a->lut_stride, a->mosaic, a->mosaic_f32);
     return pano_multiband_compose(ctx, a->table, nr, a->H, a->W, a->xs0, a->xs1, a->n_levels,
-                                  a->owner, a->valid, interior ? a->interior : nullptr,
-                                  interior && stitch_has_classes(ctx, a, n_blur) ? a->classes : nullptr,
-                                  interior ? a->cams : nullptr, interior ? a->sin_t : nullptr,
-                                  interior ? a->cos_t : nullptr, interior ? a->tan_p : nullptr,
-                                  a->lut, a->lut_stride, a->mosaic, a->mosaic_f32);
+                                  a->owner, a->valid, nullptr, nullptr, nullptr, nullptr, nullptr,
+                                  nullptr, a->lut, a->lut_stride, a->mosaic, a->mosaic_f32);
 }
 
 static void geometry_buffers(const pano_stitch_args *a, const void *out[GEOM_BUFS]) {
     const void *v[GEOM_BUFS] = {a->owner, a->valid, a->table, a->interior, a->tile_flags, a->need,
-                                a->planes, a->blurred, a->scratch, a->sin_t, a->classes};
+                                a->planes, a->blurred, a->scratch, a->sin_t, a->classes,
+                                a->block_owner};
     for (int k = 0; k < GEOM_BUFS; ++k) out[k] = v[k];
 }
 static void geometry_left(pano_ctx *ctx, const pano_stitch_args *a) {
diff --git a/pano360_amd/csrc/warp.hip b/pano360_amd/csrc/warp.hip
--- a/pano360_amd/csrc/warp.hip
+++ b/pano360_amd/csrc/warp.hip
@@ -48,15 +48,28 @@
 }
 
 #define WARP_ROWS 4
+
+struct WarpMosaic {
+    const uint8_t *interior;
+    const int16_t *block_owner;
+    int W8, H, W, xs0, xs1;
+    uint8_t *mosaic;
+    float *mosaic_f32;
+};
+
+template <bool SHADE>
 __global__ __launch_bounds__(256) void warp_windows_kernel(
     const pano_camera *__restrict__ cams, const pano_patch *__restrict__ patches,
     const double *__restrict__ sin_t, const double *__restrict__ cos_t,
     const double *__restrict__ tan_p, const float *__restrict__ lut, int lut_stride,
-    const uint8_t *__restrict__ need) {
+    const uint8_t *__restrict__ need, WarpMosaic mo) {
     __shared__ float s_lut[256];
     const pano_patch p = patches[blockIdx.z];
     constexpr int BH = 4 * WARP_ROWS;
     if ((int)blockIdx.x * 64 >= p.vw || (int)blockIdx.y * BH >= p.vh) return;
+    const pano_camera *cam = cams + p.index;
+    if (SHADE && !cam->frame) return;
+    bool planes_needed = true;
     if (need) {
         const int ntx = ((p.ax0 + p.aw - 1) >> 5) - (p.ax0 >> 5) + 1;
         const int nty = ((p.ay0 + p.ah - 1) >> 5) - (p.ay0 >> 5) + 1;
@@ -68,7 +81,10 @@
         bool any = false;
         for (int ty = ty0; ty <= ty1; ++ty)
             for (int tx = tx0; tx <= tx1; ++tx) any |= need[p.tiles_off + ty * ntx + tx] != 0;
-        if (!any) return;
+        if (!any) {
+            if (!SHADE) return;
+            planes_needed = false;
+        }
     }
     s_lut[threadIdx.y * 64 + threadIdx.x] =
         lut[(size_t)p.index * lut_stride + threadIdx.y * 64 + threadIdx.x];
@@ -77,9 +93,32 @@
     const int x = blockIdx.x * 64 + threadIdx.x;
     const int y0 = blockIdx.y * BH + threadIdx.y;
     if (x >= p.vw || y0 >= p.vh) return;
-    const pano_camera *cam = cams + p.index;
     const int sw = cam->sw, sh = cam->sh;
     const int gx = p.x0 + p.vx0 + x;
+    bool shade[WARP_ROWS];
+    int wy = 0;
+    if (SHADE) {
+        wy = __builtin_amdgcn_readfirstlane((int)threadIdx.y);
+        const bool col = gx >= mo.xs0 && gx < mo.xs1;
+#pragma unroll
+        for (int j = 0; j < WARP_ROWS; ++j) {
+            const int y = (int)blockIdx.y * BH + wy + 4 * j, gy = p.y0 + p.vy0 + y;
+            shade[j] = false;
+            if (col && y < p.vh && (unsigned)gy < (unsigned)mo.H) {
+                const size_t row = (size_t)(gy / PANO_INTERIOR_BLOCK) * mo.W8;
+                const uint32_t b = (uint32_t)gx / PANO_INTERIOR_BLOCK;
+                const uint8_t in = mo.interior[row + b];
+                const int16_t own = mo.block_owner[row + b];
+                shade[j] = (in != 0) & (own == (int16_t)p.index);
+            }
+        }
+        if (!planes_needed) {
+            bool some = false;
+#pragma unroll
+            for (int j = 0; j < WARP_ROWS; ++j) some |= shade[j];
+            if (__ballot(some) == 0ull) return;
+        }
+    }
     const double s = table_f64(sin_t, gx), c = table_f64(cos_t, gx);
     double t[WARP_ROWS];
 #pragma unroll
@@ -115,10 +154,28 @@
         const int y = y0 + 4 * j;
         if (y >= p.vh) break;
         const uint32_t o = ((uint32_t)y * (uint32_t)p.vpitch + (uint32_t)x) * 4u;
-#pragma unroll
-        for (int k = 0; k < 3; ++k) {
-            *(plane_ptr)(out[k] + o) = lerp4(lut_at(s_lut, tb[j].v[0][k]), lut_at(s_lut, tb[j].v[1][k]),
-                                             lut_at(s_lut, tb[j].v[2][k]), lut_at(s_lut, tb[j].v[3][k]), tp[j]);
+        float v[3];
+#pragma unroll
+        for (int k = 0; k < 3; ++k)
+            v[k] = lerp4(lut_at(s_lut, tb[j].v[0][k]), lut_at(s_lut, tb[j].v[1][k]),
+                         lut_at(s_lut, tb[j].v[2][k]), lut_at(s_lut, tb[j].v[3][k]), tp[j]);
+        if (!SHADE || planes_needed) {
+#pragma unroll
+            for (int k = 0; k < 3; ++k) *(plane_ptr)(out[k] + o) = v[k];
+        }
+        if (SHADE && shade[j]) {
+            const int gy = p.y0 + p.vy0 + (int)blockIdx.y * BH + wy + 4 * j;
+            const size_t g0 = ((size_t)gy * mo.W + (p.x0 + p.vx0 + (int)blockIdx.x * 64)) * 3;
+            const uint32_t l = (uint32_t)threadIdx.x * 3u;
+            const byte_ptr m8 = (byte_ptr)mo.mosaic + g0;
+            const byte_ptr m32 = (byte_ptr)mo.mosaic_f32 + g0 * 4;
+#pragma unroll
+            for (int k = 0; k < 3; ++k) {
+                float q = v[k];
+                q = q < 0.0f ? 0.0f : (q > 1.0f ? 1.0f : q);
+                if (mo.mosaic_f32) *(plane_ptr)(m32 + (l + k) * 4u) = q;
+                *(__attribute__((address_space(1))) uint8_t *)(m8 + l + k) = (uint8_t)(int)(255.0f * q);
+            }
         }
     }
 }
@@ -184,20 +241,54 @@
     return PANO_OK;
 }
 
+static int warp_windows_check(const char *who, const pano_camera *cams, const pano_patch *patches,
+                              int n, int max_vw, int max_vh, const double *sin_t, const double *cos_t,
+                              const double *tan_p, const float *lut, int lut_stride) {
+    PANO_REQUIRE(cams && patches && sin_t && cos_t && tan_p && lut && lut_stride >= 0,
+                 "%s: null pointer", who);
+    PANO_REQUIRE(n >= 0 && n <= 65535 && max_vw >= 0 && max_vh >= 0, "%s: bad argument", who);
+    return PANO_OK;
+}
+
 extern "C" int pano_warp_windows(pano_ctx *ctx, const pano_camera *cams, const pano_patch *patches,
                                  int n, int max_vw, int max_vh, const double *sin_t,
                                  const double *cos_t, const double *tan_p, const float *lut,
                                  int lut_stride, const uint8_t *need) {
     PANO_ENTER(ctx, "pano_warp_windows");
-    PANO_REQUIRE(cams && patches && sin_t && cos_t && tan_p && lut && lut_stride >= 0,
-                 "pano_warp_windows: null pointer");
-    PANO_REQUIRE(n >= 0 && n <= 65535 && max_vw >= 0 && max_vh >= 0,
-                 "pano_warp_windows: bad argument");
+    if (int rc = warp_windows_check("pano_warp_windows", cams, patches, n, max_vw, max_vh, sin_t,
+                                    cos_t, tan_p, lut, lut_stride))
+        return rc;
     if (n == 0 || max_vw == 0 || max_vh == 0) return PANO_OK;
     dim3 block(64, 4), grid(ceil_div(max_vw, 64), ceil_div(max_vh, 4 * WARP_ROWS), n);
     PANO_TIMED(PK_WARP_WINDOWS, (hipStream_t)stream,
-               hipLaunchKernelGGL(warp_windows_kernel, grid, block, 0, (hipStream_t)stream,
-                                  cams, patches, sin_t, cos_t, tan_p, lut, lut_stride, need));
+               hipLaunchKernelGGL(warp_windows_kernel<false>, grid, block, 0, (hipStream_t)stream,
+                                  cams, patches, sin_t, cos_t, tan_p, lut, lut_stride, need,
+                                  WarpMosaic{}));
     PANO_LAUNCH_CHECK("warp_windows_kernel");
     return PANO_OK;
 }
+
+extern "C" int pano_warp_windows_mosaic(pano_ctx *ctx, const pano_camera *cams,
+                                        const pano_patch *patches, int n, int max_vw, int max_vh,
+                                        const double *sin_t, const double *cos_t,
+                                        const double *tan_p, const float *lut, int lut_stride,
+                                        const uint8_t *need, const uint8_t *interior,
+                                        const int16_t *block_owner, int H, int W, int xs0, int xs1,
+                                        uint8_t *mosaic, float *mosaic_f32) {
+    PANO_ENTER(ctx, "pano_warp_windows_mosaic");
+    if (int rc = warp_windows_check("pano_warp_windows_mosaic", cams, patches, n, max_vw, max_vh,
+                                    sin_t, cos_t, tan_p, lut, lut_stride))
+        return rc;
+    PANO_REQUIRE(interior && block_owner && mosaic, "pano_warp_windows_mosaic: null pointer");
+    PANO_REQUIRE(H > 0 && W > 0 && xs0 >= 0 && xs1 <= W && xs0 <= xs1,
+                 "pano_warp_windows_mosaic: bad mosaic %dx%d or strip [%d, %d)", H, W, xs0, xs1);
+    if (n == 0 || max_vw == 0 || max_vh == 0) return PANO_OK;
+    const WarpMosaic mo = {interior, block_owner, ceil_div(W, PANO_INTERIOR_BLOCK), H, W, xs0, xs1,
+                           mosaic, mosaic_f32};
+    dim3 block(64, 4), grid(ceil_div(max_vw, 64), ceil_div(max_vh, 4 * WARP_ROWS), n);
+    PANO_TIMED(PK_WARP_WINDOWS, (hipStream_t)stream,
+               hipLaunchKernelGGL(warp_windows_kernel<true>, grid, block, 0, (hipStream_t)stream,
+                                  cams, patches, sin_t, cos_t, tan_p, lut, lut_stride, need, mo));
+    PANO_LAUNCH_CHECK("warp_windows_kernel");
+    return PANO_OK;
+}
diff --git a/pano360_amd/engine.py b/pano360_amd/engine.py
--- a/pano360_amd/engine.py
+++ b/pano360_amd/engine.py
@@ -714,7 +714,7 @@
         mosaic, fl = self.blur_and_compose(table, owner, valid, shape, n_levels, want_float)
         return mosaic, fl, owner, valid
 
-    def interior_map(self, owner, radius, strip=None):
+    def interior_map(self, owner, radius, strip=None, with_owners=False):
         torch = _torch()
         H, W = owner.shape
         c0, c1 = strip if strip is not None else (0, W)
@@ -724,9 +724,9 @@
         interior = torch.empty(shape8, dtype=torch.uint8, device=self.device)
         _lib.check(self.lib.pano_interior_map(self.ctx(), _ptr(owner), H, W, c0, c1, radius,
                                               _ptr(bown), _ptr(interior)), "pano_interior_map")
-        return interior
-
-    def interior_classes(self, owner, radii, strip=None):
+        return (interior, bown) if with_owners else interior
+
+    def interior_classes(self, owner, radii, strip=None, with_owners=False):
         torch = _torch()
         H, W = owner.shape
         c0, c1 = strip if strip is not None else (0, W)
@@ -739,7 +739,7 @@
         _lib.check(self.lib.pano_interior_classes(self.ctx(), _ptr(owner), H, W, c0, c1, arr,
                                                   len(radii), _ptr(bown), _ptr(interior),
                                                   _ptr(classes)), "pano_interior_classes")
-        return interior, classes
+        return (interior, classes, bown) if with_owners else (interior, classes)
 
     def level_radii(self, n_levels):
         return [gaussian_ksize(s) // 2 for s in level_sigmas(n_levels)]
@@ -822,7 +822,7 @@
 
     def blur_and_compose(self, table, owner, valid, shape, n_levels, want_float=False,
                          strip=None, interior=None, cams=None, plan=None, luts=None, flags=None,
-                         mosaic_out=None, classes=None):
+                         mosaic_out=None, classes=None, float_out=None, interior_done=False):
         torch = _torch()
         H, W = shape
         c0, c1 = strip if strip is not None else (0, W)
@@ -837,15 +837,19 @@
             self.last_tiles = (table, flags)
         mosaic = (mosaic_out if mosaic_out is not None else
                   torch.empty((H, W, 3), dtype=torch.uint8, device=self.device))
-        fl = (torch.empty((H, W, 3), dtype=torch.float32, device=self.device)
-              if want_float else None)
+        fl = float_out
+        if fl is None and want_float:
+            fl = torch.empty((H, W, 3), dtype=torch.float32, device=self.device)
         tabs = plan.dev if interior is not None else (None, None, None)
-        _lib.check(self.lib.pano_multiband_compose(
+        if interior_done and (interior is None or mosaic_out is None or (want_float and float_out is None)):
+            raise ValueError("interior_done: needs the interior map and the buffers the warp wrote")
+        compose = self.lib.pano_multiband_compose_seams if interior_done else self.lib.pano_multiband_compose
+        _lib.check(compose(
             self.ctx(), table.ptr, table.n, H, W, c0, c1, n_levels, _ptr(owner), _ptr(valid),
             _ptr(interior), _ptr(classes) if interior is not None else None,
             _ptr(cams) if interior is not None else None, _ptr(tabs[0]),
             _ptr(tabs[1]), _ptr(tabs[2]), *self._lut_args(luts), _ptr(mosaic), _ptr(fl)),
-            "pano_multiband_compose")
+            "pano_multiband_compose_seams" if interior_done else "pano_multiband_compose")
         return mosaic, fl
 
     def simple_blend(self, patches, shape, linear, table=None):
@@ -995,7 +999,7 @@
         return self.owned_regions(owner, n, strip)[0]
 
     def multiband_fused(self, frames, plan, n_levels, want_float=False, frame_ids=None,
-                        strip=None, shortcut=True, luts=None, mosaic_out=None):
+                        strip=None, shortcut=True, luts=None, mosaic_out=None, float_out=None):
         H, W = plan.shape
         c0, c1 = strip if strip is not None else (0, W)
         taps, ntaps, n_blur, radius = self.blur_tables(n_levels)
@@ -1008,15 +1012,16 @@
         cams = self.camera_table(plan, have)
         if self.native_stitch:
             return self._stitch_native(plan, cams, have, n_levels, want_float, (c0, c1), ext,
-                                       shortcut, luts, mosaic_out)
+                                       shortcut, luts, mosaic_out, float_out)
         owner, valid = self.ownership_cameras(plan, strip=ext, cams=cams)
         regions = self.owned_regions_async(owner, plan.n, ext, 2 * radius + 2)
-        interior = classes = None
+        interior = classes = bown = None
         if shortcut and n_blur:
             if self.get_option(_lib.OPT_LEVEL_CLASSES):
-                interior, classes = self.interior_classes(owner, self.level_radii(n_levels), ext)
+                interior, classes, bown = self.interior_classes(owner, self.level_radii(n_levels), ext,
+                                                                with_owners=True)
             else:
-                interior = self.interior_map(owner, radius, ext)
+                interior, bown = self.interior_map(owner, radius, ext, with_owners=True)
         resident = np.zeros(plan.n, np.uint8)
         resident[[i for i in have if 0 <= i < plan.n]] = 1
         rects32 = np.ascontiguousarray(plan.rects, np.int32)
@@ -1035,13 +1040,27 @@
             _lib.check(self.lib.pano_blur_tiles(
                 self.ctx(), table.ptr, table.n, table.max_aw, table.max_ah, plan.shape[1], radius,
                 _ptr(interior), _ptr(flags), _ptr(need)), "pano_blur_tiles")
-        _lib.check(self.lib.pano_warp_windows(
-            self.ctx(), _ptr(cams), table.ptr, table.n, table.max_vw, table.max_vh,
-            _ptr(plan.dev[0]),
-            _ptr(plan.dev[1]), _ptr(plan.dev[2]), *self._lut_args(luts), _ptr(need)), "pano_warp_windows")
+        fl = float_out if want_float else None
+        if interior is not None:
+            torch = _torch()
+            if mosaic_out is None:
+                mosaic_out = torch.empty((H, W, 3), dtype=torch.uint8, device=self.device)
+            if want_float and fl is None:
+                fl = torch.empty((H, W, 3), dtype=torch.float32, device=self.device)
+            _lib.check(self.lib.pano_warp_windows_mosaic(
+                self.ctx(), _ptr(cams), table.ptr, table.n, table.max_vw, table.max_vh,
+                _ptr(plan.dev[0]), _ptr(plan.dev[1]), _ptr(plan.dev[2]), *self._lut_args(luts),
+                _ptr(need), _ptr(interior), _ptr(bown), H, W, c0, c1, _ptr(mosaic_out), _ptr(fl)),
+                "pano_warp_windows_mosaic")
+        else:
+            _lib.check(self.lib.pano_warp_windows(
+                self.ctx(), _ptr(cams), table.ptr, table.n, table.max_vw, table.max_vh,
+                _ptr(plan.dev[0]),
+                _ptr(plan.dev[1]), _ptr(plan.dev[2]), *self._lut_args(luts), _ptr(need)), "pano_warp_windows")
         mosaic, fl = self.blur_and_compose(table, owner, valid, plan.shape, n_levels,
                                            want_float, (c0, c1), interior, cams, plan, luts,
-                                           flags=flags, mosaic_out=mosaic_out, classes=classes)
+                                           flags=flags, mosaic_out=mosaic_out, classes=classes,
+                                           float_out=fl, interior_done=interior is not None)
         self.last_classes, self.last_interior = classes, interior
         return mosaic, fl, valid, patches
 
@@ -1072,7 +1091,7 @@
         return ws
 
     def _stitch_native(self, plan, cams, have, n_levels, want_float, strip, ext, shortcut, luts,
-                       mosaic_out):
+                       mosaic_out, float_out=None):
         torch = _torch()
         H, W = plan.shape
         taps, ntaps, n_blur, radius = self.blur_tables(n_levels)
@@ -1081,8 +1100,9 @@
         a = ws["args"]
         mosaic = (mosaic_out if mosaic_out is not None else
                   torch.empty((H, W, 3), dtype=torch.uint8, device=self.device))
-        fl = (torch.empty((H, W, 3), dtype=torch.float32, device=self.device)
-              if want_float else None)
+        fl = float_out if want_float else None
+        if fl is None and want_float:
+            fl = torch.empty((H, W, 3), dtype=torch.float32, device=self.device)
         resident = ws["have"]
         resident[:] = 0
         resident[[i for i in have if 0 <= i < plan.n]] = 1
```

Result: faster. 211,000 MP/s (median of 6 runs) (+3.7%).
